# OpenPPL/ppq

Measured on AMD Instinct MI355X. Metric: calibration samples/sec (RuntimeCalibrationPass, KL 2048-bin, ResNet-50 INT8), higher is better.
Workload: dtype f32; 1 GPU; ResNet-50 topology (53 Conv + 1 Gemm, BN folded, seeded He init), RuntimeCalibrationPass kl 2048 bins, per-tensor INT8 activations, per-channel INT8 weights, 279 batches x 32 x 3x224x224 per GPU; samples=8928, batch=32, observed_tensors=72, rccl_ranks=1, async_observe=False, cache_params=False, channels_last=False, fuse_params=True, batch_observations=True, reuse_activations=False, replayed_batches=0, hip_graph=auto, graph_replays=0, miopen_find=False

## Files before the change

include/ppq_hip.h:

```cpp
#ifndef PPQ_HIP_H_
#define PPQ_HIP_H_

#include <stdint.h>

#ifdef __cplusplus
extern "C" {
#endif

typedef enum {
    PPQHIP_OK = 0,
    PPQHIP_ERR_INVALID_VALUE = -1,
    PPQHIP_ERR_UNSUPPORTED = -2,
    PPQHIP_ERR_HIP = -3
} ppqhip_status;

#define PPQHIP_ABI_VERSION 4

const char* ppqhip_last_error(void);
int ppqhip_version(void);
int ppqhip_device_arch(char* buf, int n);

int ppqhip_fq_linear_t(const float* x, const float* scale, const float* offset, float* out,
                       int64_t n, int clip_min, int clip_max, int rounding, void* stream);

// ... 85 lines not shown

int ppqhip_fq_float_c_bwd(const float* x, const float* scale, const float* offset,
                          const float* grad_y, float* grad_x, float* grad_s, int64_t n,
                          int64_t num_channel, int64_t elem_per_channel,
                          int exponent, int mantissa, float clip_min, float clip_max,
                          int rounding, void* stream);

int64_t ppqhip_hist_workspace_bytes(int64_t n, int64_t num_bins);
int ppqhip_hist_sym_t(const float* x, int64_t n, float hist_scale, int clip_outliers,
                      int32_t* hist, int64_t num_bins, void* workspace, void* stream);

int ppqhip_hist_asym_t(const float* x, int64_t n, float min_value, float max_value,
                       int clip_outliers, int32_t* hist, int64_t num_bins, void* workspace,
                       void* stream);

int ppqhip_hist_sym_c(const float* x, int64_t n, int64_t num_channel, int64_t elem_per_channel,
                      float hist_scale, int clip_outliers, int32_t* hist, int64_t num_bins,
                      void* stream);

int ppqhip_hist_sym_c_scales(const float* x, int64_t n, int64_t num_channel, int64_t elem_per_channel,
                             const float* hist_scales, int clip_outliers, int32_t* hist,
                             int64_t num_bins, void* stream);
int ppqhip_hist_asym_c_ranges(const float* x, int64_t n, int64_t num_channel, int64_t elem_per_channel,
                              const float* mins, const float* maxs, int clip_outliers, int32_t* hist,
                              int64_t num_bins, void* stream);

int64_t ppqhip_quantile_workspace_bytes(int64_t n);
int ppqhip_quantile_t(const float* x, int64_t n, float q, float* dest, uint32_t* hint, void* workspace,
                      void* stream);

typedef struct ppqhip_quantile_job {
    const float* x;
    float* dest;
    uint32_t* hint;
    int64_t n;
} ppqhip_quantile_job;
int64_t ppqhip_quantile_multi_workspace_bytes(int num_jobs, int64_t total_elems);
int ppqhip_quantile_t_multi(const ppqhip_quantile_job* jobs, int num_jobs, float q, void* workspace,
                            void* stream);
void ppqhip_quantile_debug_layout(int64_t* out);
void ppqhip_quantile_hot_layout(int64_t* out);

int ppqhip_isotone_t(const float* x, int64_t n, float* dest, void* workspace, void* stream);

int64_t ppqhip_minmax_workspace_bytes(int64_t n);
int ppqhip_minmax_t(const float* x, int64_t n, float* minmax, void* workspace, void* stream);

int ppqhip_minmax_c(const float* x, int64_t n, int64_t num_channel, int64_t elem_per_channel,
                    float* mins, float* maxs, void* stream);

typedef struct ppqhip_minmax_c_job {
    const float* x;
    float* mins;
    float* maxs;
    int64_t n, num_channel, elem_per_channel;
    int32_t fresh, reserved;
} ppqhip_minmax_c_job;
int ppqhip_minmax_c_multi(const ppqhip_minmax_c_job* jobs, int num_jobs, void* stream);

int ppqhip_channel_sum(const float* x, int64_t n, int64_t num_channel, int64_t elem_per_channel,
                       double* sums, void* stream);

int64_t ppqhip_hist_rows(void);
int ppqhip_hist_sym_t_rows(const float* x, int64_t n, float hist_scale, int clip_outliers,
                           int32_t* rows, int64_t num_bins, void* stream);
int ppqhip_hist_asym_t_rows(const float* x, int64_t n, float min_value, float max_value,
                            int clip_outliers, int32_t* rows, int64_t num_bins, void* stream);
typedef struct ppqhip_minmax_job {
    const float* x;
    float* slots;
    int64_t n;
} ppqhip_minmax_job;
int ppqhip_minmax_t_slots_multi(const ppqhip_minmax_job* jobs, int num_jobs, void* stream);

typedef struct ppqhip_hist_job {
    const float* x;
    int32_t* rows;
    int64_t n;
    float p0, p1;
} ppqhip_hist_job;
int ppqhip_hist_t_rows_multi(const ppqhip_hist_job* jobs, int num_jobs, int asymmetric,
                             int clip_outliers, int64_t num_bins, void* stream);
int ppqhip_hist_rows_finish(const int32_t* rows, int64_t num_bins, int32_t* hist, void* stream);
int ppqhip_check_bin_rule(const float* x, int64_t n, float min_value, float hist_scale, int asymmetric, uint64_t* out, void* stream);
int64_t ppqhip_minmax_slots(void);
int ppqhip_minmax_t_slots(const float* x, int64_t n, float* slots, void* stream);
int ppqhip_minmax_slots_finish(const float* slots, float* minmax, void* stream);

float ppqhip_mse_loss_host(const int64_t* hist, int64_t num_bins, int start, int step, int end);

int64_t ppqhip_mse_search_workspace_bytes(int64_t num_hist);
int ppqhip_mse_search(const int32_t* hist, int64_t num_hist, int64_t num_bins,
                      const double* hist_scale, const double* min_value,
                      int quant_min, int quant_max, int symmetrical, int32_t* best,
                      void* workspace, void* stream);

int64_t ppqhip_kl_num_candidates(int64_t num_bins, int num_of_bits);
int ppqhip_kl_losses(const int32_t* hist, int64_t num_hist, int64_t num_bins, int num_of_bits,
                     double* losses, void* stream);

int ppqhip_tensor_clip_t(const float* value, const float* reference, const float* limit,
                         float* out, int64_t n, void* stream);
int ppqhip_tensor_clip_c(const float* value, const float* reference, const float* limit,
                         float* out, int64_t n, int64_t num_channel, int64_t elem_per_channel,
                         void* stream);
int ppqhip_rounding_loss(const float* x, const float* scale, const float* offset, float* out,
                         int64_t n, int64_t num_channel, int64_t elem_per_channel,
                         int clip_min, int clip_max, int rounding, void* stream);
int ppqhip_rounding_loss_bwd(const float* x, const float* dy, const float* scale,
                             const float* offset, float* dx, int64_t n, int64_t num_channel,
                             int64_t elem_per_channel, int clip_min, int clip_max, int rounding,
                             void* stream);

int ppqhip_bias_act(float* y, const float* bias, int64_t n, int64_t num_channel, int64_t elem_per_channel,
                    int relu, void* stream);
int ppqhip_bias_add_act(float* a, const float* bias_a, float* b, const float* bias_b, float* out,
                        int64_t n, int64_t num_channel, int64_t elem_per_channel, int relu, void* stream);

#define PPQHIP_NOT_FUSED 1
int ppqhip_bias_act_stats(float* y, const float* bias, int64_t n, int64_t num_channel, int64_t elem_per_channel,
                          int relu, float* slots_y, void* stream);
int ppqhip_bias_add_act_stats(float* a, const float* bias_a, float* b, const float* bias_b, float* out,
                              int64_t n, int64_t num_channel, int64_t elem_per_channel, int relu,
                              float* slots_a, float* slots_b, float* slots_out, void* stream);

#define PPQHIP_ELIDE_A 1
#define PPQHIP_ELIDE_B 2
int ppqhip_bias_add_act_stats2(float* a, const float* bias_a, float* b, const float* bias_b, float* out,
                               int64_t n, int64_t num_channel, int64_t elem_per_channel, int relu,
                               float* slots_a, float* slots_b, float* slots_out, int elide, void* stream);

int ppqhip_bias_act_hist(float* y, const float* bias, int64_t n, int64_t num_channel, int64_t elem_per_channel,
                         int relu, int32_t* rows_y, float p0_y, float p1_y, int64_t num_bins, int asymmetric,
                         int clip_outliers, void* stream);
int ppqhip_bias_add_act_hist(float* a, const float* bias_a, float* b, const float* bias_b, float* out,
                             int64_t n, int64_t num_channel, int64_t elem_per_channel, int relu,
                             int32_t* rows_a, float p0_a, float p1_a, int32_t* rows_b, float p0_b, float p1_b,
                             int32_t* rows_out, float p0_out, float p1_out, int64_t num_bins, int asymmetric,
                             int clip_outliers, int elide, void* stream);

typedef struct ppqhip_adaround_job {
    const float* w;
    const float* v;
    const float* scale;
    const float* offset;
    float* out;
    const float* dy;
    int64_t n, num_channel, elem_per_channel;
    int32_t qmin, qmax;
} ppqhip_adaround_job;
int ppqhip_adaround_fwd_multi(const ppqhip_adaround_job* jobs, int num_jobs, void* stream);
int ppqhip_adaround_bwd_multi(const ppqhip_adaround_job* jobs, int num_jobs, const float* reg, void* stream);

typedef struct ppqhip_roundtune_job {
    const float* w;
    const float* r;
    const float* scale;
    const float* offset;
    float* out;
    int64_t n, num_channel, elem_per_channel;
    int32_t qmin, qmax;
} ppqhip_roundtune_job;
int ppqhip_roundtune_fwd_multi(const ppqhip_roundtune_job* jobs, int num_jobs, void* stream);

typedef struct ppqhip_fetch_rows_job {
    const float* x;
    const int32_t* index;
    float* out;
    int64_t rows, row_len, count;
} ppqhip_fetch_rows_job;
int ppqhip_fetch_rows_multi(const ppqhip_fetch_rows_job* jobs, int num_jobs, void* stream);
typedef struct ppqhip_measure_rows_job {
    const float* p;
    const float* r;
    const int32_t* index;
    double* sums;
    int64_t rows, row_len, count;
} ppqhip_measure_rows_job;
int ppqhip_measure_rows_multi(const ppqhip_measure_rows_job* jobs, int num_jobs, void* stream);
enum { PPQHIP_MEASURE_SNR = 0, PPQHIP_MEASURE_MSE = 1, PPQHIP_MEASURE_COSINE = 2 };
enum { PPQHIP_REDUCE_MEAN = 0, PPQHIP_REDUCE_MAX = 1 };
typedef struct ppqhip_measure_finish_job {
    const double* sums;
    double* acc;
    float* row_out;
    int64_t rows, count;
    int32_t method, reduce;
} ppqhip_measure_finish_job;
int ppqhip_measure_finish_multi(const ppqhip_measure_finish_job* jobs, int num_jobs, void* stream);

typedef struct ppqhip_equalize_segment {
    const float* base;
    int64_t extent;
    int64_t div, a, b;
    int64_t outer, stride, run;
    float multiplier;
    int32_t downstream;
} ppqhip_equalize_segment;
typedef struct ppqhip_equalize_scale_job {
    const ppqhip_equalize_segment* segments;
    float* scale;
    int32_t num_segments, num_channel;
    float value_threshold;
    int32_t reserved;
} ppqhip_equalize_scale_job;
int ppqhip_equalize_scale_multi(const ppqhip_equalize_scale_job* jobs, int num_jobs, void* stream);
typedef struct ppqhip_equalize_apply_job {
    float* x;
    const float* scale;
    int64_t n, run, inner, group_out;
    int64_t num_scale;
    int32_t divide, reserved;
} ppqhip_equalize_apply_job;
int ppqhip_equalize_apply_multi(const ppqhip_equalize_apply_job* jobs, int num_jobs, void* stream);

typedef struct ppqhip_split_plan_job {
    const ppqhip_equalize_segment* segments;
    int32_t* src_of;
    int32_t* count;
    int32_t num_segments, num_channel;
    float value_threshold;
    int32_t reserved;
// ... 119 lines not shown
```

ppq_amd/_lib.py:

```python
import ctypes
import os

_HERE = os.path.dirname(os.path.abspath(__file__))
LIB_PATH = os.path.join(_HERE, 'libppq_hip.so')

c_f32p = ctypes.c_void_p
c_i32p = ctypes.c_void_p
c_f64p = ctypes.c_void_p
c_i64 = ctypes.c_int64
c_int = ctypes.c_int
c_flt = ctypes.c_float
c_vp = ctypes.c_void_p

ABI_VERSION = 4


NOT_FUSED = 1


class ProfEntry(ctypes.Structure):
    _fields_ = [('name', ctypes.c_char * 48), ('launches', ctypes.c_int64),
                ('total_ms', ctypes.c_double), ('total_bytes', ctypes.c_double)]


PROTOTYPES = {
    'ppqhip_last_error': (ctypes.c_char_p, []),
    'ppqhip_version': (c_int, []),
    'ppqhip_device_arch': (c_int, [ctypes.c_char_p, c_int]),
    'ppqhip_fq_linear_t': (c_int, [c_f32p, c_f32p, c_f32p, c_f32p, c_i64, c_int, c_int, c_int, c_vp]),
    'ppqhip_fq_linear_c': (c_int, [c_f32p, c_f32p, c_f32p, c_f32p, c_i64, c_i64, c_i64, c_int, c_int, c_int, c_vp]),
    'ppqhip_to_int_t': (c_int, [c_f32p, c_f32p, c_f32p, c_vp, c_i64, c_int, c_int, c_int, c_int, c_vp]),
    'ppqhip_to_int_c': (c_int, [c_f32p, c_f32p, c_f32p, c_vp, c_i64, c_i64, c_i64, c_int, c_int, c_int, c_int, c_vp]),
    'ppqhip_fq_linear_t_bwd': (c_int, [c_f32p, c_f32p, c_f32p, c_f32p, c_f32p, c_f32p, c_i64, c_int, c_int, c_int,
                                       c_vp]),
    'ppqhip_fq_linear_c_bwd': (c_int, [c_f32p, c_f32p, c_f32p, c_f32p, c_f32p, c_f32p, c_i64, c_i64, c_i64, c_int,
                                       c_int, c_int, c_vp]),
    'ppqhip_fq_linear_c_bwd_multi': (c_int, [c_vp, c_int, c_int, c_vp]),
    'ppqhip_fq_linear_t_bwd_partials': (c_i64, [c_i64]),
    'ppqhip_fq_linear_t_bwd_main': (c_int, [c_f32p, c_f32p, c_f32p, c_f32p, c_f32p, c_f32p, c_i64, c_int, c_int, c_int, c_vp]),
    'ppqhip_lsq_finish_multi': (c_int, [c_vp, c_int, c_vp]),
    'ppqhip_bias_act': (c_int, [c_f32p, c_f32p, c_i64, c_i64, c_i64, c_int, c_vp]),
    'ppqhip_bias_add_act': (c_int, [c_f32p, c_f32p, c_f32p, c_f32p, c_f32p, c_i64, c_i64, c_i64, c_int, c_vp]),
    'ppqhip_bias_act_stats': (c_int, [c_f32p, c_f32p, c_i64, c_i64, c_i64, c_int, c_f32p, c_vp]),
    'ppqhip_bias_add_act_stats': (c_int, [c_f32p, c_f32p, c_f32p, c_f32p, c_f32p, c_i64, c_i64, c_i64, c_int, c_f32p, c_f32p,
                                          c_f32p, c_vp]),
    'ppqhip_bias_add_act_stats2': (c_int, [c_f32p, c_f32p, c_f32p, c_f32p, c_f32p, c_i64, c_i64, c_i64, c_int, c_f32p, c_f32p,
                                           c_f32p, c_int, c_vp]),
    'ppqhip_bias_act_hist': (c_int, [c_f32p, c_f32p, c_i64, c_i64, c_i64, c_int, c_i32p, c_flt, c_flt, c_i64, c_int, c_int, c_vp]),
    'ppqhip_bias_add_act_hist': (c_int, [c_f32p, c_f32p, c_f32p, c_f32p, c_f32p, c_i64, c_i64, c_i64, c_int,
                                         c_i32p, c_flt, c_flt, c_i32p, c_flt, c_flt, c_i32p, c_flt, c_flt, c_i64, c_int, c_int,
                                         c_int, c_vp]),
    'ppqhip_fq_float_t': (c_int, [c_f32p, c_f32p, c_f32p, c_f32p, c_i64, c_int, c_int, c_flt, c_flt, c_int, c_vp]),
    'ppqhip_fq_float_c': (c_int, [c_f32p, c_f32p, c_f32p, c_f32p, c_i64, c_i64, c_i64, c_int, c_int, c_flt, c_flt,
                                  c_int, c_vp]),
    'ppqhip_fq_float_c_bwd': (c_int, [c_f32p, c_f32p, c_f32p, c_f32p, c_f32p, c_f32p, c_i64, c_i64, c_i64, c_int,
                                      c_int, c_flt, c_flt, c_int, c_vp]),
    'ppqhip_hist_workspace_bytes': (c_i64, [c_i64, c_i64]),
    'ppqhip_hist_sym_t': (c_int, [c_f32p, c_i64, c_flt, c_int, c_i32p, c_i64, c_vp, c_vp]),
    'ppqhip_hist_asym_t': (c_int, [c_f32p, c_i64, c_flt, c_flt, c_int, c_i32p, c_i64, c_vp, c_vp]),
    'ppqhip_hist_sym_c': (c_int, [c_f32p, c_i64, c_i64, c_i64, c_flt, c_int, c_i32p, c_i64, c_vp]),
    'ppqhip_hist_sym_c_scales': (c_int, [c_f32p, c_i64, c_i64, c_i64, c_f32p, c_int, c_i32p, c_i64, c_vp]),
    'ppqhip_hist_asym_c_ranges': (c_int, [c_f32p, c_i64, c_i64, c_i64, c_f32p, c_f32p, c_int, c_i32p, c_i64, c_vp]),
    'ppqhip_quantile_workspace_bytes': (c_i64, [c_i64]),
    'ppqhip_quantile_t': (c_int, [c_f32p, c_i64, c_flt, c_f32p, c_vp, c_vp, c_vp]),
    'ppqhip_isotone_t': (c_int, [c_f32p, c_i64, c_f32p, c_vp, c_vp]),
    'ppqhip_minmax_workspace_bytes': (c_i64, [c_i64]),
    'ppqhip_minmax_t': (c_int, [c_f32p, c_i64, c_f32p, c_vp, c_vp]),
    'ppqhip_minmax_c': (c_int, [c_f32p, c_i64, c_i64, c_i64, c_f32p, c_f32p, c_vp]),
    'ppqhip_minmax_c_multi': (c_int, [c_vp, c_int, c_vp]),
    'ppqhip_fq_linear_multi_table_bytes': (c_i64, [c_int]),
    'ppqhip_fq_linear_multi': (c_int, [c_vp, c_int, c_int, c_vp, c_int, c_vp]),
    'ppqhip_float_scale_search_table_bytes': (c_i64, [c_int]),
    'ppqhip_float_scale_search': (c_int, [c_vp, c_int, c_vp, c_int, c_int, c_vp, c_vp, c_vp]),
    'ppqhip_fq_float_multi_table_bytes': (c_i64, [c_int]),
    'ppqhip_fq_float_multi': (c_int, [c_vp, c_int, c_int, c_vp, c_int, c_vp]),
    'ppqhip_quantile_multi_workspace_bytes': (c_i64, [c_int, c_i64]),
    'ppqhip_quantile_t_multi': (c_int, [c_vp, c_int, c_flt, c_vp, c_vp]),
    'ppqhip_quantile_debug_layout': (None, [c_vp]),
    'ppqhip_quantile_hot_layout': (None, [c_vp]),
    'ppqhip_minmax_t_slots_multi': (c_int, [c_vp, c_int, c_vp]),
    'ppqhip_hist_t_rows_multi': (c_int, [c_vp, c_int, c_int, c_int, c_i64, c_vp]),
    'ppqhip_channel_sum': (c_int, [c_f32p, c_i64, c_i64, c_i64, c_f64p, c_vp]),
    'ppqhip_hist_rows': (c_i64, []),
    'ppqhip_hist_sym_t_rows': (c_int, [c_f32p, c_i64, c_flt, c_int, c_i32p, c_i64, c_vp]),
    'ppqhip_hist_asym_t_rows': (c_int, [c_f32p, c_i64, c_flt, c_flt, c_int, c_i32p, c_i64, c_vp]),
    'ppqhip_hist_rows_finish': (c_int, [c_i32p, c_i64, c_i32p, c_vp]),
    'ppqhip_check_bin_rule': (c_int, [c_f32p, c_i64, c_flt, c_flt, c_int, c_vp, c_vp]),
    'ppqhip_minmax_slots': (c_i64, []),
    'ppqhip_minmax_t_slots': (c_int, [c_f32p, c_i64, c_f32p, c_vp]),
    'ppqhip_minmax_slots_finish': (c_int, [c_f32p, c_f32p, c_vp]),
    'ppqhip_mse_loss_host': (c_flt, [ctypes.POINTER(ctypes.c_int64), c_i64, c_int, c_int, c_int]),
    'ppqhip_mse_search_workspace_bytes': (c_i64, [c_i64]),
    'ppqhip_mse_search': (c_int, [c_i32p, c_i64, c_i64, c_f64p, c_f64p, c_int, c_int, c_int, c_i32p, c_vp, c_vp]),
    'ppqhip_kl_num_candidates': (c_i64, [c_i64, c_int]),
    'ppqhip_kl_losses': (c_int, [c_i32p, c_i64, c_i64, c_int, c_f64p, c_vp]),
    'ppqhip_tensor_clip_t': (c_int, [c_f32p, c_f32p, c_f32p, c_f32p, c_i64, c_vp]),
    'ppqhip_tensor_clip_c': (c_int, [c_f32p, c_f32p, c_f32p, c_f32p, c_i64, c_i64, c_i64, c_vp]),
    'ppqhip_rounding_loss': (c_int, [c_f32p, c_f32p, c_f32p, c_f32p, c_i64, c_i64, c_i64, c_int, c_int, c_int, c_vp]),
    'ppqhip_rounding_loss_bwd': (c_int, [c_f32p, c_f32p, c_f32p, c_f32p, c_f32p, c_i64, c_i64, c_i64, c_int, c_int,
                                         c_int, c_vp]),
    'ppqhip_adaround_fwd_multi': (c_int, [c_vp, c_int, c_vp]),
    'ppqhip_adaround_bwd_multi': (c_int, [c_vp, c_int, c_f32p, c_vp]),
    'ppqhip_roundtune_fwd_multi': (c_int, [c_vp, c_int, c_vp]),
    'ppqhip_equalize_scale_multi': (c_int, [c_vp, c_int, c_vp]),
    'ppqhip_equalize_apply_multi': (c_int, [c_vp, c_int, c_vp]),
    'ppqhip_split_plan_multi': (c_int, [c_vp, c_int, c_vp]),
    'ppqhip_split_apply_multi': (c_int, [c_vp, c_int, c_vp]),
    'ppqhip_ssd_scales_multi': (c_int, [c_vp, c_int, c_vp]),
    'ppqhip_ssd_apply_multi': (c_int, [c_vp, c_int, c_vp]),
    'ppqhip_fq_measure_rows_multi': (c_int, [c_vp, c_int, c_vp]),
    'ppqhip_fetch_rows_multi': (c_int, [c_vp, c_int, c_vp]),
    'ppqhip_measure_rows_multi': (c_int, [c_vp, c_int, c_vp]),
    'ppqhip_measure_finish_multi': (c_int, [c_vp, c_int, c_vp]),
    'ppqhip_stat_moments_multi': (c_int, [c_vp, c_int, c_vp]),
    'ppqhip_stat_shape_multi': (c_int, [c_vp, c_int, c_vp]),
    'ppqhip_mx_fq': (c_int, [c_f32p, c_f32p, c_vp, c_i64, c_i64, c_i64, c_int, c_vp]),
    'ppqhip_mx_fq_multi': (c_int, [c_vp, c_int, c_vp]),
    'ppqhip_mx_pack': (c_int, [c_f32p, c_vp, c_vp, c_i64, c_i64, c_i64, c_int, c_vp]),
    'ppqhip_mx_pack_multi': (c_int, [c_vp, c_int, c_vp]),
    'ppqhip_mx_unpack': (c_int, [c_vp, c_vp, c_f32p, c_i64, c_i64, c_i64, c_int, c_vp]),
    'ppqhip_mx_unpack_multi': (c_int, [c_vp, c_int, c_vp]),
    'ppqhip_mx_gemm': (c_int, [c_vp, c_vp, c_int, c_vp, c_vp, c_int, c_f32p, c_f32p, c_i64, c_i64, c_i64, c_vp]),
    'ppqhip_prof_enable': (c_int, [c_int]),
    'ppqhip_mx_conv2d': (c_int, [c_vp, c_vp, c_int, c_vp, c_vp, c_int, c_f32p, c_f32p] + [c_i64] * 13 + [c_vp]),
    'ppqhip_mx_gemm_fused': (c_int, [c_vp, c_vp, c_int, c_vp, c_vp, c_int, c_f32p, c_f32p, c_int, c_f32p, c_vp, c_vp, c_int, c_i64, c_i64, c_i64, c_vp]),
    'ppqhip_mx_conv2d_fused': (c_int, [c_vp, c_vp, c_int, c_vp, c_vp, c_int, c_f32p, c_f32p, c_int, c_f32p, c_vp, c_vp, c_int] + [c_i64] * 13 + [c_vp]),
    'ppqhip_prof_collect': (c_int, [ctypes.POINTER(ProfEntry), c_int]),
    'ppqhip_prof_event_overhead_us': (ctypes.c_double, [c_vp, c_int]),
}

if not os.path.exists(LIB_PATH):
    raise ImportError(
        f'{LIB_PATH} is missing: the HIP kernel library has not been built.  Run '
        '`python -c "import __graft_entry__ as g; g.build()"` or `make -C ppq_amd/csrc` (needs hipcc, '
        'targets gfx950).  ppq_amd has no CPU / PyTorch fallback by design.')

import torch

_torch_hip = os.path.join(os.path.dirname(torch.__file__), 'lib', 'libamdhip64.so')
if os.path.exists(_torch_hip):
    ctypes.CDLL(_torch_hip, mode=ctypes.RTLD_GLOBAL)

try:
    lib = ctypes.CDLL(LIB_PATH)
except OSError as e:
    raise ImportError(f'cannot load {LIB_PATH}: {e}') from e

for _name, (_res, _args) in PROTOTYPES.items():
    _fn = getattr(lib, _name)
    _fn.restype = _res
    _fn.argtypes = _args


if lib.ppqhip_version() != ABI_VERSION:
    raise ImportError(f'{LIB_PATH} has ABI version {lib.ppqhip_version()}, this package needs {ABI_VERSION}: rebuild it '
                      '(`make -C ppq_amd/csrc` or `python -c "import __graft_entry__ as g; g.build()"`)')


def last_error() -> str:
    msg = lib.ppqhip_last_error()
    return msg.decode('utf-8', 'replace') if msg else ''
```

ppq_amd/csrc/epilogue.hip:

```cpp
#include "channel_axis.hpp"
#include "common.hpp"
#include "hist_bin.hpp"
#include "minmax_fold.hpp"

namespace ppqhip {
namespace {

constexpr int kEpTileU = 2;
constexpr int kEpSmallU = 1;
constexpr long long kEpSmallElems = 1ll << 20;

struct EpArgs {
    float* a;
    const float* bias_a;
    float* b;
    const float* bias_b;
    float* out;
    uint32_t nvec;
    uint32_t tail;
    int ntail;
    FastDiv epc;
    FastDiv nc;
    uint32_t elide;
};

__device__ __forceinline__ float act(float v, bool relu) {
    return (relu && !__builtin_isnan(v)) ? __builtin_fmaxf(v, 0.f) : v;
}

__device__ __forceinline__ float4 add4(const float4& x, const float4& y) {
    return make_float4(x.x + y.x, x.y + y.y, x.z + y.z, x.w + y.w);
}

template <bool RELU>
__device__ __forceinline__ float4 act4(const float4& v) {
    return make_float4(act(v.x, RELU), act(v.y, RELU), act(v.z, RELU), act(v.w, RELU));
}

template <bool PLANE>
__device__ __forceinline__ float4 bias4(const float* __restrict__ bias, uint32_t v, const FastDiv& epc, const FastDiv& nc) {
    if (PLANE) {
        const float t = bias[channel_of(v, epc, nc)];
        return make_float4(t, t, t, t);
    }
    const uint32_t i = v * 4u;
    return make_float4(bias[channel_of(i, epc, nc)], bias[channel_of(i + 1, epc, nc)], bias[channel_of(i + 2, epc, nc)],
                       bias[channel_of(i + 3, epc, nc)]);
}

template <typename T>
struct EpStored { T a, b, out; };

constexpr uint32_t kElideA = 1u, kElideB = 2u;

template <bool RESID, bool BIAS_B, bool RELU>
__device__ __forceinline__ EpStored<float> epilogue_elem(const EpArgs& p, uint32_t i, const FastDiv& epc, uint32_t elide = 0) {
    EpStored<float> s{};
    const uint32_t c = channel_of(i, epc, p.nc);
    const float x = p.a[i] + p.bias_a[c];
    if (!RESID) { p.a[i] = s.a = act(x, RELU); return s; }
    s.a = x;
    if (!(elide & kElideA)) p.a[i] = x;
    float y = p.b[i];
    if (BIAS_B) {
        y = y + p.bias_b[c];
        s.b = y;
        if (!(elide & kElideB)) p.b[i] = y;
    }
    p.out[i] = s.out = act(x + y, RELU);
    return s;
}

template <bool RESID, bool BIAS_B, bool RELU>
__device__ __forceinline__ EpStored<float4> epilogue_vec(float4* a4, float4* b4, float4* o4, uint32_t vv, const float4& a,
                                                         const float4& ba, const float4& b, const float4& bb,
                                                         uint32_t elide = 0) {
    EpStored<float4> s{};
    const float4 x = add4(a, ba);
    if (!RESID) { a4[vv] = s.a = act4<RELU>(x); return s; }
    s.a = x;
    if (!(elide & kElideA)) a4[vv] = x;
    float4 y = b;
    if (BIAS_B) {
        y = add4(y, bb);
        s.b = y;
        if (!(elide & kElideB)) b4[vv] = y;
    }
    o4[vv] = s.out = act4<RELU>(add4(x, y));
    return s;
}

template <int U, bool RESID, bool BIAS_B, bool RELU, bool PLANE>
__global__ __launch_bounds__(kBlock) void epilogue_kernel(EpArgs p) {
    const uint32_t base = blockIdx.x * (kBlock * U) + threadIdx.x;
    float4* a4 = reinterpret_cast<float4*>(p.a);
    float4* b4 = reinterpret_cast<float4*>(p.b);
    float4* o4 = reinterpret_cast<float4*>(p.out);
    float4 a[U], ba[U], b[U]{}, bb[U]{};
#pragma unroll
    for (int k = 0; k < U; k++) {
        const uint32_t vv = min(base + k * kBlock, p.nvec - 1);
        a[k] = a4[vv];
        ba[k] = bias4<PLANE>(p.bias_a, vv, p.epc, p.nc);
        if (RESID) b[k] = b4[vv];
        if (BIAS_B) bb[k] = bias4<PLANE>(p.bias_b, vv, p.epc, p.nc);
    }
#pragma unroll
    for (int k = 0; k < U; k++) {
        const uint32_t vv = base + k * kBlock;
        if (vv >= p.nvec) continue;
        epilogue_vec<RESID, BIAS_B, RELU>(a4, b4, o4, vv, a[k], ba[k], b[k], bb[k]);
    }
    if (!PLANE && blockIdx.x == 0 && (int)threadIdx.x < p.ntail)
        epilogue_elem<RESID, BIAS_B, RELU>(p, p.tail + threadIdx.x, p.epc);
}

template <bool RESID, bool BIAS_B, bool RELU>
__global__ __launch_bounds__(kBlock) void epilogue_scalar_kernel(EpArgs p) {
    const uint32_t stride = gridDim.x * kBlock;
    for (uint32_t i = blockIdx.x * kBlock + threadIdx.x; i < (uint32_t)p.ntail; i += stride)
        epilogue_elem<RESID, BIAS_B, RELU>(p, i, p.epc);
}

bool fill_vector_geometry(EpArgs& p, int64_t n, int64_t C, int64_t epc) {
    const ChannelAxisMap g = pack_channel_axis(true, n, C, epc);
    p.nc = g.nc; p.epc = g.epc;
    p.nvec = g.nvec;
    p.tail = g.nvec * 4u;
    p.ntail = (int)(n & 3);
    return g.plane != 0;
}

template <bool RESID, bool BIAS_B, bool RELU>
void launch_epilogue(EpArgs p, int64_t n, int64_t C, int64_t epc, bool aligned, hipStream_t st) {
    if (!aligned || n < 4) {
        p.nvec = 0; p.tail = 0; p.ntail = (int)n;
        p.epc = make_fastdiv((uint32_t)epc); p.nc = make_fastdiv((uint32_t)C);
        hipLaunchKernelGGL((epilogue_scalar_kernel<RESID, BIAS_B, RELU>), dim3(stream_grid(n, kBlock)), dim3(kBlock), 0, st, p);
        return;
    }
    const bool plane = fill_vector_geometry(p, n, C, epc);
#define PPQ_LAUNCH_EP(U, PLANE)                                                                                          \
    hipLaunchKernelGGL((epilogue_kernel<U, RESID, BIAS_B, RELU, PLANE>), dim3((p.nvec + kBlock * U - 1) / (kBlock * U)),   \
                       dim3(kBlock), 0, st, p)
    if (n <= kEpSmallElems) {
        if (plane) PPQ_LAUNCH_EP(kEpSmallU, true); else PPQ_LAUNCH_EP(kEpSmallU, false);
    } else {
        if (plane) PPQ_LAUNCH_EP(kEpTileU, true); else PPQ_LAUNCH_EP(kEpTileU, false);
    }
#undef PPQ_LAUNCH_EP
}

constexpr int kEpStatBlock = 512;
constexpr int kEpStatWgPerCu = 2;

struct EpMinMaxSinks { float* slots[3]; };
template <bool RESID, bool BIAS_B>
struct EpMinMaxSet {
    using Args = EpMinMaxSinks;
    static constexpr int NS = RESID ? 3 : 1;
    bool live[NS];
    float mn[NS], mx[NS];
// ... 61 lines not shown
    __device__ __forceinline__ void begin() {
#pragma unroll
        for (int k = 0; k < NS; k++) {
#pragma unroll
            for (int r = 0; r < kRowRegs; r++) {
                const int b = (int)threadIdx.x + r * kEpStatBlock;
                old[k][r] = (early && live[k] && b <= acc[k].last) ? row[k][b] : 0;
            }
        }
        for (uint32_t i = threadIdx.x; i < lds_ints; i += kEpStatBlock) lds[i] = 0;
        asm volatile("s_waitcnt lgkmcnt(0)\n\ts_barrier" ::: "memory");
    }
    template <bool FULL>
    __device__ __forceinline__ void bin4(Binner<ASYM, CLIP, true>& a, const float4& v, bool in, bool elect) {
        int b[4];
        a.bins4(v, b);
        if (elect) a.elect(b[0], FULL || in);
        if (FULL && CLIP) a.commit4_exec(b);
        else {
            a.template commit<FULL>(b[0], in); a.template commit<FULL>(b[1], in);
            a.template commit<FULL>(b[2], in); a.template commit<FULL>(b[3], in);
        }
    }
    template <bool FULL>
    __device__ __forceinline__ void feed4(const EpStored<float4>& s, bool in, bool elect) {
        if (live[0]) bin4<FULL>(acc[0], s.a, in, elect);
        if (RESID) {
            if (BIAS_B && live[1]) bin4<FULL>(acc[1], s.b, in, elect);
            if (live[NS - 1]) bin4<FULL>(acc[NS - 1], s.out, in, elect);
        }
    }
    __device__ __forceinline__ void bin1(Binner<ASYM, CLIP, true>& a, float v, bool in) {
        const int b = a.bin1(v);
        a.elect(b, in);
        a.template commit<false>(b, in);
    }
    __device__ __forceinline__ void feed1(const EpStored<float>& s, bool in) {
        if (live[0]) bin1(acc[0], s.a, in);
        if (RESID) {
            if (BIAS_B && live[1]) bin1(acc[1], s.b, in);
            if (live[NS - 1]) bin1(acc[NS - 1], s.out, in);
        }
    }
    __device__ __forceinline__ void finish(const Args& sk, uint32_t g, int*) {
#pragma unroll
        for (int k = 0; k < NS; k++)
            if (live[k]) acc[k].flush_hot();
        asm volatile("s_waitcnt lgkmcnt(0)" ::: "memory");
        __syncthreads();
#pragma unroll
        for (int k = 0; k < NS; k++) {
            if (!live[k]) continue;
            const int* h = acc[k].h;
            if (early) {
#pragma unroll
                for (int r = 0; r < kRowRegs; r++) {
                    const int b = (int)threadIdx.x + r * kEpStatBlock;
                    if (b >= sk.bins) break;
                    const int c = h[b];
                    if (c) row[k][b] = old[k][r] + c;
                }
            } else {
                for (int b = threadIdx.x; b < sk.bins; b += kEpStatBlock) {
                    const int c = h[b];
                    if (c) row[k][b] += c;
                }
            }
        }
    }
};

template <int U, bool RESID, bool BIAS_B, bool RELU, bool PLANE, class SINKS>
__global__ __launch_bounds__(kEpStatBlock, (kEpStatBlock * kEpStatWgPerCu + 255) / 256)
void epilogue_stats_kernel(EpArgs p, typename SINKS::Args sk) {
    extern __shared__ int lds[];
    constexpr uint32_t kTile = (uint32_t)kEpStatBlock * U;
    const uint32_t G = gridDim.x, g = blockIdx.x;
    const uint32_t full = p.nvec / kTile, tiles = full + (p.nvec > full * kTile ? 1u : 0u);
    uint32_t t, t_end;
    even_split(tiles, G, g, t, t_end);
    float4* a4 = reinterpret_cast<float4*>(p.a);
    float4* b4 = reinterpret_cast<float4*>(p.b);
    float4* o4 = reinterpret_cast<float4*>(p.out);
    const uint32_t elide = p.elide;
    SINKS sinks;
    sinks.init(sk, lds);

    struct Tile { float4 a[U], ba[U], b[U], bb[U]; };
    auto fetch = [&](Tile& T, uint32_t tile) {
        const uint32_t base = tile * kTile + threadIdx.x;
#pragma unroll
        for (int u = 0; u < U; u++) {
            const uint32_t vv = base + u * kEpStatBlock;
            T.a[u] = a4[vv];
            T.ba[u] = bias4<PLANE>(p.bias_a, vv, p.epc, p.nc);
            if (RESID) T.b[u] = b4[vv];
            if (BIAS_B) T.bb[u] = bias4<PLANE>(p.bias_b, vv, p.epc, p.nc);
        }
    };
    auto consume = [&](const Tile& T, uint32_t tile) {
        const uint32_t base = tile * kTile + threadIdx.x;
        EpStored<float4> s[U];
#pragma unroll
        for (int u = 0; u < U; u++)
            s[u] = epilogue_vec<RESID, BIAS_B, RELU>(a4, b4, o4, base + u * kEpStatBlock, T.a[u], T.ba[u], T.b[u], T.bb[u], elide);
#pragma unroll
        for (int u = 0; u < U; u++) sinks.template feed4<true>(s[u], true, u == 0);
    };
    const uint32_t tf = min(t_end, full);
    Tile ta{}, tb{};
    if (t < tf) fetch(ta, t);
    sinks.begin();
    if (t < tf) {
        for (;;) {
            fetch(tb, min(t + 1, tf - 1));
            consume(ta, t);
            if (++t >= tf) break;
            fetch(ta, min(t + 1, tf - 1));
            consume(tb, t);
            if (++t >= tf) break;
        }
    }
    if (t < t_end) {
        const uint32_t base = t * kTile + threadIdx.x;
#pragma unroll
        for (int u = 0; u < U; u++) {
            const uint32_t vv = base + u * kEpStatBlock;
            const uint32_t vc = min(vv, p.nvec - 1);
            const float4 a = a4[vc], ba = bias4<PLANE>(p.bias_a, vc, p.epc, p.nc);
            float4 b{}, bb{};
            if (RESID) b = b4[vc];
            if (BIAS_B) bb = bias4<PLANE>(p.bias_b, vc, p.epc, p.nc);
            const bool in = vv < p.nvec;
            EpStored<float4> s{};
            if (in) s = epilogue_vec<RESID, BIAS_B, RELU>(a4, b4, o4, vv, a, ba, b, bb, elide);
            sinks.template feed4<false>(s, in, true);
        }
    }
    if (!PLANE && g == G - 1 && p.ntail > 0) {
        const bool in = (int)threadIdx.x < p.ntail;
        EpStored<float> s{};
        if (in) s = epilogue_elem<RESID, BIAS_B, RELU>(p, p.tail + threadIdx.x, p.epc, elide);
        sinks.feed1(s, in);
    }
    sinks.finish(sk, g, lds);
}

template <bool RESID, bool BIAS_B>
int launch_epilogue_stats(EpArgs p, int64_t n, int64_t C, int64_t epc, int relu, bool aligned, EpMinMaxSinks sk, const char* what,
                          hipStream_t st) {
    if ((!sk.slots[0] && !sk.slots[1] && !sk.slots[2]) || !aligned || n < 4) return PPQHIP_NOT_FUSED;
    const bool plane = fill_vector_geometry(p, n, C, epc);
    const bool small = n <= kEpSmallElems;
    const uint32_t tile = (uint32_t)kEpStatBlock * (small ? kEpSmallU : kEpTileU), tiles = (p.nvec + tile - 1) / tile;
    const uint32_t cap = (uint32_t)(num_cu() * kEpStatWgPerCu);
    const uint32_t grid = tiles < cap ? tiles : cap;
    using Set = EpMinMaxSet<RESID, BIAS_B>;
#define PPQ_LAUNCH_EPS(U, RELU, PLANE)                                                                                    \
    hipLaunchKernelGGL((epilogue_stats_kernel<U, RESID, BIAS_B, RELU, PLANE, Set>), dim3(grid), dim3(kEpStatBlock),         \
                       32 * sizeof(float), st, p, sk)
    switch ((small ? 0 : 4) | (relu ? 2 : 0) | (plane ? 1 : 0)) {
        case 0: PPQ_LAUNCH_EPS(kEpSmallU, false, false); break;
        case 1: PPQ_LAUNCH_EPS(kEpSmallU, false, true); break;
        case 2: PPQ_LAUNCH_EPS(kEpSmallU, true, false); break;
        case 3: PPQ_LAUNCH_EPS(kEpSmallU, true, true); break;
        case 4: PPQ_LAUNCH_EPS(kEpTileU, false, false); break;
        case 5: PPQ_LAUNCH_EPS(kEpTileU, false, true); break;
        case 6: PPQ_LAUNCH_EPS(kEpTileU, true, false); break;
        default: PPQ_LAUNCH_EPS(kEpTileU, true, true); break;
    }
#undef PPQ_LAUNCH_EPS
    return finish_launch(what);
}

constexpr uint32_t kEpHistLdsInts = 3 * 2048;
constexpr uint32_t kEpHistMinTiles = 2;
struct EpHistRule { int bins, asym, clip; };

template <bool RESID, bool BIAS_B>
int launch_epilogue_hist(EpArgs p, int64_t n, int64_t C, int64_t epc, int relu, bool aligned, EpHistSinks sk, EpHistRule r,
                         const char* what, hipStream_t st) {
    uint32_t ints = 0;
    for (int k = 0; k < 3; k++) {
        sk.lds_off[k] = ints;
        if (sk.rows[k]) ints += (uint32_t)r.bins;
    }
    sk.lds_ints = ints; sk.bins = r.bins;
    if (ints == 0 || ints > kEpHistLdsInts || !aligned || n <= kEpSmallElems || !relu) return PPQHIP_NOT_FUSED;
    const bool plane = fill_vector_geometry(p, n, C, epc);
    const uint32_t tile = (uint32_t)kEpStatBlock * kEpTileU, tiles = (p.nvec + tile - 1) / tile;
    const uint32_t cap = (uint32_t)(num_cu() * kEpStatWgPerCu);
    uint32_t grid = tiles / kEpHistMinTiles;
    if (grid > cap) grid = cap;
#define PPQ_LAUNCH_EPH(PLANE, ASYM, CLIP)                                                                                 \
    hipLaunchKernelGGL((epilogue_stats_kernel<kEpTileU, RESID, BIAS_B, true, PLANE, EpHistSet<RESID, BIAS_B, ASYM, CLIP>>),  \
                       dim3(grid), dim3(kEpStatBlock), ints * sizeof(int), st, p, sk)
    switch ((plane ? 4 : 0) | (r.asym ? 2 : 0) | (r.clip ? 1 : 0)) {
        case 0: PPQ_LAUNCH_EPH(false, false, false); break;
        case 1: PPQ_LAUNCH_EPH(false, false, true); break;
        case 2: PPQ_LAUNCH_EPH(false, true, false); break;
        case 3: PPQ_LAUNCH_EPH(false, true, true); break;
        case 4: PPQ_LAUNCH_EPH(true, false, false); break;
        case 5: PPQ_LAUNCH_EPH(true, false, true); break;
        case 6: PPQ_LAUNCH_EPH(true, true, false); break;
        default: PPQ_LAUNCH_EPH(true, true, true); break;
    }
#undef PPQ_LAUNCH_EPH
    return finish_launch(what);
}

void set_hist_rule(EpHistSinks& sk, int k, int32_t* rows, float p0, float p1, const EpHistRule& r) {
    sk.rows[k] = rows;
    if (r.asym) { sk.a0[k] = p0; sk.hs[k] = (p1 - p0) / (float)r.bins; }
    else { sk.a0[k] = 0.f; sk.hs[k] = p0; }
}

int validate_elide(const char* what, int elide, bool sink_a, bool sink_b, bool has_bias_b) {
    if (elide & ~(int)(kElideA | kElideB)) { set_error("%s: elide has unknown bits", what); return PPQHIP_ERR_INVALID_VALUE; }
    if (((elide & (int)kElideA) && !sink_a) || ((elide & (int)kElideB) && !(sink_b && has_bias_b))) {
        set_error("%s: a tensor that is not stored needs a sink", what); return PPQHIP_ERR_INVALID_VALUE;
    }
    return PPQHIP_OK;
}

}
}

using namespace ppqhip;

extern "C" {

int ppqhip_bias_act(float* y, const float* bias, int64_t n, int64_t num_channel, int64_t elem_per_channel, int relu,
                    void* stream) {
    if (int st = validate_channel_axis("bias_act", n, num_channel, elem_per_channel)) return st;
    if (!y || !bias) { set_error("bias_act: null pointer"); return PPQHIP_ERR_INVALID_VALUE; }
    hipStream_t s = (hipStream_t)stream;
    EpArgs p{};
    p.a = y; p.bias_a = bias;
    const bool aligned = aligned16(y);
    if (relu) launch_epilogue<false, false, true>(p, n, num_channel, elem_per_channel, aligned, s);
    else launch_epilogue<false, false, false>(p, n, num_channel, elem_per_channel, aligned, s);
    return finish_launch("bias_act");
}

int ppqhip_bias_add_act(float* a, const float* bias_a, float* b, const float* bias_b, float* out, int64_t n,
                        int64_t num_channel, int64_t elem_per_channel, int relu, void* stream) {
    if (int st = validate_channel_axis("bias_add_act", n, num_channel, elem_per_channel)) return st;
    if (!a || !bias_a || !b || !out) { set_error("bias_add_act: null pointer"); return PPQHIP_ERR_INVALID_VALUE; }
    hipStream_t s = (hipStream_t)stream;
    EpArgs p{};
    p.a = a; p.bias_a = bias_a; p.b = b; p.bias_b = bias_b; p.out = out;
    const bool aligned = aligned16(a) && aligned16(b) && aligned16(out);
    if (bias_b) {
        if (relu) launch_epilogue<true, true, true>(p, n, num_channel, elem_per_channel, aligned, s);
        else launch_epilogue<true, true, false>(p, n, num_channel, elem_per_channel, aligned, s);
    } else {
        if (relu) launch_epilogue<true, false, true>(p, n, num_channel, elem_per_channel, aligned, s);
        else launch_epilogue<true, false, false>(p, n, num_channel, elem_per_channel, aligned, s);
    }
    return finish_launch("bias_add_act");
}

int ppqhip_bias_act_stats(float* y, const float* bias, int64_t n, int64_t num_channel, int64_t elem_per_channel, int relu,
                          float* slots_y, void* stream) {
    if (int st = validate_channel_axis("bias_act_stats", n, num_channel, elem_per_channel)) return st;
    if (!y || !bias) { set_error("bias_act_stats: null pointer"); return PPQHIP_ERR_INVALID_VALUE; }
    EpArgs p{};
    p.a = y; p.bias_a = bias;
    return launch_epilogue_stats<false, false>(p, n, num_channel, elem_per_channel, relu, aligned16(y), EpMinMaxSinks{{slots_y, nullptr, nullptr}},
                                               "bias_act_stats", (hipStream_t)stream);
}

static int bias_add_act_stats_impl(const char* what, float* a, const float* bias_a, float* b, const float* bias_b, float* out,
                                   int64_t n, int64_t num_channel, int64_t elem_per_channel, int relu, float* slots_a,
                                   float* slots_b, float* slots_out, int elide, void* stream) {
    if (int st = validate_channel_axis(what, n, num_channel, elem_per_channel)) return st;
    if (!a || !bias_a || !b || !out) { set_error("%s: null pointer", what); return PPQHIP_ERR_INVALID_VALUE; }
    if (!bias_b && slots_b) { set_error("%s: without bias_b, b is only read: it has no sink", what); return PPQHIP_ERR_INVALID_VALUE; }
    if (int st = validate_elide(what, elide, slots_a != nullptr, slots_b != nullptr, bias_b != nullptr)) return st;
    EpArgs p{};
    p.a = a; p.bias_a = bias_a; p.b = b; p.bias_b = bias_b; p.out = out; p.elide = (uint32_t)elide;
    const bool aligned = aligned16(a) && aligned16(b) && aligned16(out);
    const EpMinMaxSinks sk{{slots_a, slots_b, slots_out}};
    hipStream_t s = (hipStream_t)stream;
    if (bias_b) return launch_epilogue_stats<true, true>(p, n, num_channel, elem_per_channel, relu, aligned, sk, what, s);
    return launch_epilogue_stats<true, false>(p, n, num_channel, elem_per_channel, relu, aligned, sk, what, s);
}

int ppqhip_bias_add_act_stats(float* a, const float* bias_a, float* b, const float* bias_b, float* out, int64_t n,
                              int64_t num_channel, int64_t elem_per_channel, int relu, float* slots_a, float* slots_b,
                              float* slots_out, void* stream) {
    return bias_add_act_stats_impl("bias_add_act_stats", a, bias_a, b, bias_b, out, n, num_channel, elem_per_channel, relu,
                                   slots_a, slots_b, slots_out, 0, stream);
}

int ppqhip_bias_add_act_stats2(float* a, const float* bias_a, float* b, const float* bias_b, float* out, int64_t n,
                               int64_t num_channel, int64_t elem_per_channel, int relu, float* slots_a, float* slots_b,
                               float* slots_out, int elide, void* stream) {
    return bias_add_act_stats_impl("bias_add_act_stats2", a, bias_a, b, bias_b, out, n, num_channel, elem_per_channel, relu,
                                   slots_a, slots_b, slots_out, elide, stream);
}

static int validate_hist_rule(const char* what, int64_t bins) {
    if (bins <= 0 || bins > 0x7fffffffLL) { set_error("%s: histogram is empty or too large", what); return PPQHIP_ERR_INVALID_VALUE; }
    return PPQHIP_OK;
}

int ppqhip_bias_act_hist(float* y, const float* bias, int64_t n, int64_t num_channel, int64_t elem_per_channel, int relu,
                         int32_t* rows_y, float p0_y, float p1_y, int64_t num_bins, int asymmetric, int clip_outliers,
                         void* stream) {
    if (int st = validate_channel_axis("bias_act_hist", n, num_channel, elem_per_channel)) return st;
    if (!y || !bias) { set_error("bias_act_hist: null pointer"); return PPQHIP_ERR_INVALID_VALUE; }
    if (int st = validate_hist_rule("bias_act_hist", num_bins)) return st;
    if (num_bins > (int64_t)kEpHistLdsInts) return PPQHIP_NOT_FUSED;
    const EpHistRule r{(int)num_bins, asymmetric ? 1 : 0, clip_outliers ? 1 : 0};
    EpHistSinks sk{};
    set_hist_rule(sk, 0, rows_y, p0_y, p1_y, r);
    EpArgs p{};
    p.a = y; p.bias_a = bias;
    return launch_epilogue_hist<false, false>(p, n, num_channel, elem_per_channel, relu, aligned16(y), sk, r, "bias_act_hist",
                                              (hipStream_t)stream);
}

int ppqhip_bias_add_act_hist(float* a, const float* bias_a, float* b, const float* bias_b, float* out, int64_t n,
                             int64_t num_channel, int64_t elem_per_channel, int relu, int32_t* rows_a, float p0_a, float p1_a,
                             int32_t* rows_b, float p0_b, float p1_b, int32_t* rows_out, float p0_out, float p1_out,
                             int64_t num_bins, int asymmetric, int clip_outliers, int elide, void* stream) {
    const char* what = "bias_add_act_hist";
    if (int st = validate_channel_axis(what, n, num_channel, elem_per_channel)) return st;
    if (!a || !bias_a || !b || !out) { set_error("%s: null pointer", what); return PPQHIP_ERR_INVALID_VALUE; }
    if (!bias_b && rows_b) { set_error("%s: without bias_b, b is only read: it has no sink", what); return PPQHIP_ERR_INVALID_VALUE; }
    if (int st = validate_hist_rule(what, num_bins)) return st;
    if (int st = validate_elide(what, elide, rows_a != nullptr, rows_b != nullptr, bias_b != nullptr)) return st;
    if ((rows_a && (rows_a == rows_b || rows_a == rows_out)) || (rows_b && rows_b == rows_out)) {
        set_error("%s: two sinks share one rows accumulator", what); return PPQHIP_ERR_INVALID_VALUE;
    }
    if (num_bins > (int64_t)kEpHistLdsInts) return PPQHIP_NOT_FUSED;
    const EpHistRule r{(int)num_bins, asymmetric ? 1 : 0, clip_outliers ? 1 : 0};
    EpHistSinks sk{};
    set_hist_rule(sk, 0, rows_a, p0_a, p1_a, r);
    set_hist_rule(sk, 1, rows_b, p0_b, p1_b, r);
    set_hist_rule(sk, 2, rows_out, p0_out, p1_out, r);
    EpArgs p{};
    p.a = a; p.bias_a = bias_a; p.b = b; p.bias_b = bias_b; p.out = out; p.elide = (uint32_t)elide;
    const bool aligned = aligned16(a) && aligned16(b) && aligned16(out);
    hipStream_t s = (hipStream_t)stream;
    if (bias_b) return launch_epilogue_hist<true, true>(p, n, num_channel, elem_per_channel, relu, aligned, sk, r, what, s);
    return launch_epilogue_hist<true, false>(p, n, num_channel, elem_per_channel, relu, aligned, sk, r, what, s);
}

}
```

ppq_amd/csrc/hist.hip:

```cpp
#include "common.hpp"
#include "hist_bin.hpp"

namespace ppqhip {

constexpr int kMaxLdsBins = 16384;
constexpr int kLdsBudgetInts = 2048;
constexpr int kHistBlock = 512;
constexpr int kHistWgPerCu = 2;
constexpr int kHistU = 2;
constexpr int kHistMinTiles = 2;
constexpr int kHistAtomicMaxWg = 128;
constexpr long long kHistNtElems = 48ll << 20;
constexpr int kHistRows = kNumCU * kHistWgPerCu;
constexpr uint32_t kTileVec = (uint32_t)kHistBlock * kHistU;
constexpr uint32_t kTileElems = kTileVec * 4;
static_assert(kHistBlock % 64 == 0 && kHistBlock >= 64 && kHistBlock <= 1024, "histogram workgroup: whole waves");

struct BinRule {
    float a;
    float hs;
    float rcp;
    int bins;
    int clip;
    int asym;
};
static BinRule make_rule(float a, float hs, int bins, int clip, int asym) {
    BinRule r; r.a = a; r.hs = hs; r.rcp = 1.0f / hs; r.bins = bins; r.clip = clip; r.asym = asym;
    return r;
}

constexpr int kReduceBins = 32, kReduceSlices = 32, kReduceBlock = kReduceBins * kReduceSlices;
__global__ __launch_bounds__(kReduceBlock) void hist_reduce_kernel(const int* __restrict__ partial, int count, int bins,
                                                                   int* __restrict__ hist) {
    __shared__ int lds[kReduceSlices][kReduceBins];
    const int lane_bin = threadIdx.x % kReduceBins, slice = threadIdx.x / kReduceBins;
    const int b = blockIdx.x * kReduceBins + lane_bin;
    int total = 0;
    if (b < bins) {
        int i = slice;
        for (; i + 15 * kReduceSlices < count; i += 16 * kReduceSlices) {
            int v[16];
#pragma unroll
            for (int k = 0; k < 16; k++) v[k] = partial[(size_t)(i + k * kReduceSlices) * bins + b];
#pragma unroll
            for (int k = 0; k < 16; k++) total += v[k];
        }
        for (; i < count; i += kReduceSlices) total += partial[(size_t)i * bins + b];
    }
    lds[slice][lane_bin] = total;
    __syncthreads();
    if (slice == 0 && b < bins) {
        int t = 0;
#pragma unroll
        for (int k = 0; k < kReduceSlices; k++) t += lds[k][lane_bin];
        if (t) hist[b] += t;
    }
}

constexpr int kMultiMax = 96;
enum FlushMode : int {
    FLUSH_ROWS_ADD = 0,
    FLUSH_ROWS_STORE = 1,
    FLUSH_ATOMIC = 2
};
struct HistJob {
    const float* x;
    int* rows;
    uint32_t n;
    float a, hs;
    uint32_t first_tile;
};
struct HistJobs {
    HistJob job[kMultiMax];
    uint32_t count;
    uint32_t total_tiles;
    int bins, copies, mode;
};
__host__ __device__ inline uint32_t job_tiles(uint32_t n, bool vec_ok) {
    if (!vec_ok) return (n + kTileElems - 1) / kTileElems;
    const uint32_t full = (n >> 2) / kTileVec;
    return full + (n > full * kTileElems ? 1u : 0u);
}

__device__ __forceinline__ void lds_hist_flush(int* lds, int bins, int copies, int* __restrict__ dst, int mode) {
    asm volatile("s_waitcnt lgkmcnt(0)" ::: "memory");
    __syncthreads();
    for (int b = threadIdx.x; b < bins; b += kHistBlock) {
        int s = 0;
        for (int c = 0; c < copies; c++) { s += lds[c * bins + b]; lds[c * bins + b] = 0; }
        if (mode == FLUSH_ROWS_STORE) dst[b] = s;
        else if (s) {
            if (mode == FLUSH_ROWS_ADD) dst[b] += s;
            else atomicAdd(&dst[b], s);
        }
    }
    __syncthreads();
}

template <bool ASYM, bool CLIP, bool HOT, bool NT>
__global__ __launch_bounds__(kHistBlock, (kHistBlock * kHistWgPerCu + 255) / 256)
void hist_persistent_kernel(const HistJobs jobs) {
    extern __shared__ int lds[];
    const uint32_t G = gridDim.x, g = blockIdx.x;
    uint32_t t, t_end;
    even_split(jobs.total_tiles, G, g, t, t_end);
    const int bins = jobs.bins, copies = jobs.copies;
    bool zeroed = false;
    auto zero_lds = [&]() {
        if (zeroed) return;
        for (int i = threadIdx.x; i < copies * bins; i += kHistBlock) lds[i] = 0;
        asm volatile("s_waitcnt lgkmcnt(0)\n\ts_barrier" ::: "memory");
        zeroed = true;
    };
    if (t >= t_end) {
        if (jobs.mode == FLUSH_ROWS_STORE) for (int b = threadIdx.x; b < bins; b += kHistBlock) jobs.job[0].rows[(size_t)g * bins + b] = 0;
        return;
    }
    uint32_t lo = 0, hi = jobs.count;
    while (hi - lo > 1) {
        const uint32_t mid = (lo + hi) >> 1;
        if (jobs.job[mid].first_tile <= t) lo = mid; else hi = mid;
    }
    Binner<ASYM, CLIP, HOT> acc;
    acc.init(lds + ((threadIdx.x >> 6) % copies) * bins, bins);

    for (uint32_t j = lo; t < t_end; j++) {
        const HistJob& job = jobs.job[j];
        const uint32_t j_end = (j + 1 < jobs.count) ? jobs.job[j + 1].first_tile : jobs.total_tiles;
        uint32_t k = t - job.first_tile;
        const uint32_t k1 = min(t_end, j_end) - job.first_tile;
        t = min(t_end, j_end);
        acc.set_rule(job.a, job.hs);
        const float* __restrict__ x = job.x;
        const uint32_t n = job.n;
        const bool vec_ok = (reinterpret_cast<uintptr_t>(x) & 15u) == 0;
        const uint32_t full = vec_ok ? (n >> 2) / kTileVec : 0u;
        const uint32_t kf = min(k1, full);
        if (k < kf) {
            const float4* xv = reinterpret_cast<const float4*>(x) + threadIdx.x;
// ... 534 lines not shown
    LaunchScope scope(K_HIST_SYM_T, 4.0 * (double)n, s);
    BinRule rule = make_rule(0.f, hist_scale, (int)num_bins, clip_outliers ? 1 : 0, 0);
    if (int st = launch_hist_t(x, n, rule, hist, workspace, s)) return st;
    return finish_launch("hist_sym_t");
}

int ppqhip_hist_asym_t(const float* x, int64_t n, float min_value, float max_value, int clip_outliers,
                       int32_t* hist, int64_t num_bins, void* workspace, void* stream) {
    if (int st = validate(n, num_bins, "hist_asym_t")) return st;
    hipStream_t s = (hipStream_t)stream;
    LaunchScope scope(K_HIST_ASYM_T, 4.0 * (double)n, s);
    const float hs = (max_value - min_value) / (float)num_bins;
    BinRule rule = make_rule(min_value, hs, (int)num_bins, clip_outliers ? 1 : 0, 1);
    if (int st = launch_hist_t(x, n, rule, hist, workspace, s)) return st;
    return finish_launch("hist_asym_t");
}

int64_t ppqhip_hist_rows(void) { return (int64_t)kHistRows; }

int ppqhip_hist_sym_t_rows(const float* x, int64_t n, float hist_scale, int clip_outliers, int32_t* rows,
                           int64_t num_bins, void* stream) {
    if (int st = validate(n, num_bins, "hist_sym_t_rows")) return st;
    if (num_bins > kMaxLdsBins) { set_error("hist_sym_t_rows: at most %d bins", kMaxLdsBins); return PPQHIP_ERR_UNSUPPORTED; }
    hipStream_t s = (hipStream_t)stream;
    LaunchScope scope(K_HIST_SYM_T, 4.0 * (double)n, s);
    BinRule rule = make_rule(0.f, hist_scale, (int)num_bins, clip_outliers ? 1 : 0, 0);
    if (int st = launch_hist_t(x, n, rule, nullptr, nullptr, s, rows)) return st;
    return finish_launch("hist_sym_t_rows");
}

int ppqhip_hist_asym_t_rows(const float* x, int64_t n, float min_value, float max_value, int clip_outliers,
                            int32_t* rows, int64_t num_bins, void* stream) {
    if (int st = validate(n, num_bins, "hist_asym_t_rows")) return st;
    if (num_bins > kMaxLdsBins) { set_error("hist_asym_t_rows: at most %d bins", kMaxLdsBins); return PPQHIP_ERR_UNSUPPORTED; }
    hipStream_t s = (hipStream_t)stream;
    LaunchScope scope(K_HIST_ASYM_T, 4.0 * (double)n, s);
    const float hs = (max_value - min_value) / (float)num_bins;
    BinRule rule = make_rule(min_value, hs, (int)num_bins, clip_outliers ? 1 : 0, 1);
    if (int st = launch_hist_t(x, n, rule, nullptr, nullptr, s, rows)) return st;
    return finish_launch("hist_asym_t_rows");
}

int ppqhip_hist_t_rows_multi(const ppqhip_hist_job* jobs, int num_jobs, int asymmetric, int clip_outliers,
                             int64_t num_bins, void* stream) {
    if (num_jobs <= 0) return PPQHIP_OK;
    if (jobs == nullptr) { set_error("hist_t_rows_multi: jobs is null"); return PPQHIP_ERR_INVALID_VALUE; }
    if (num_bins <= 0 || num_bins > kMaxLdsBins) {
        set_error("hist_t_rows_multi: 1..%d bins", kMaxLdsBins); return PPQHIP_ERR_UNSUPPORTED;
    }
    double bytes = 0.0;
    for (int k = 0; k < num_jobs; k++) {
        if (int st = validate(jobs[k].n, num_bins, "hist_t_rows_multi")) return st;
        if (jobs[k].x == nullptr || jobs[k].rows == nullptr) {
            set_error("hist_t_rows_multi: job %d has a null pointer", k); return PPQHIP_ERR_INVALID_VALUE;
        }
        bytes += 4.0 * (double)jobs[k].n;
    }
    hipStream_t s = (hipStream_t)stream;
    LaunchScope scope(asymmetric ? K_HIST_ASYM_T : K_HIST_SYM_T, bytes, s);
    if (int st = launch_hist_multi(jobs, num_jobs, (int)num_bins, clip_outliers ? 1 : 0, asymmetric ? 1 : 0, s)) return st;
    return finish_launch("hist_t_rows_multi");
}

int ppqhip_check_bin_rule(const float* x, int64_t n, float min_value, float hist_scale, int asymmetric, uint64_t* out, void* stream) {
    if (n <= 0 || n > 0x7fffffffLL || (n & 3) || !aligned16(x) || out == nullptr) {
        set_error("check_bin_rule: n must be a positive multiple of 4 below 2^31, x 16-B aligned, out non-null"); return PPQHIP_ERR_INVALID_VALUE;
    }
    hipStream_t s = (hipStream_t)stream;
    const uint32_t nvec = (uint32_t)(n >> 2);
    if (asymmetric) hipLaunchKernelGGL((check_bin_rule_kernel<true>), dim3(stream_grid(nvec, kBlock)), dim3(kBlock), 0, s, (const float4*)x, nvec,
                                       min_value, hist_scale, (unsigned long long*)out);
    else hipLaunchKernelGGL((check_bin_rule_kernel<false>), dim3(stream_grid(nvec, kBlock)), dim3(kBlock), 0, s, (const float4*)x, nvec,
                            0.f, hist_scale, (unsigned long long*)out);
    return finish_launch("check_bin_rule");
}

int ppqhip_hist_rows_finish(const int32_t* rows, int64_t num_bins, int32_t* hist, void* stream) {
    if (num_bins <= 0 || num_bins > kMaxLdsBins) { set_error("hist_rows_finish: bad bins"); return PPQHIP_ERR_INVALID_VALUE; }
    hipStream_t s = (hipStream_t)stream;
    launch_reduce((const int*)rows, (int)ppqhip_hist_rows(), (int)num_bins, hist, s);
    return finish_launch("hist_rows_finish");
}

static int hist_c_impl(const float* x, int64_t n, int64_t num_channel, int64_t elem_per_channel,
                       float hist_scale, const float* scales, const float* mins, const float* maxs, int clip_outliers,
                       int32_t* hist, int64_t num_bins, void* stream, const char* what) {
    if (int st = validate(n, num_bins, what)) return st;
    if (num_channel <= 0 || elem_per_channel <= 0 || n % (num_channel * elem_per_channel) != 0) {
        set_error("%s: Kernel Failure, Histogram shape is invalid.", what); return PPQHIP_ERR_INVALID_VALUE;
    }
    hipStream_t s = (hipStream_t)stream;
    const int asym = mins != nullptr;
    LaunchScope scope(K_HIST_SYM_C, 4.0 * (double)n, s);
    BinRule rule = make_rule(0.f, hist_scale, (int)num_bins, clip_outliers ? 1 : 0, asym);
    const FastDiv nc = make_fastdiv((uint32_t)num_channel);
    if (elem_per_channel % 4 == 0 && elem_per_channel >= 64 && aligned16(x) && num_bins <= kMaxLdsBins) {
        const uint32_t C = (uint32_t)num_channel, outer = (uint32_t)(n / (num_channel * elem_per_channel));
        const uint32_t want_wgs = (uint32_t)num_cu() * kHistCWgPerCu;
        uint32_t splits = C >= want_wgs ? 1u : (want_wgs + C - 1) / C;
        const uint64_t tiles_per_channel = ((uint64_t)outer * (uint64_t)(elem_per_channel / 4)) / kTileVec;
        if (splits > tiles_per_channel) splits = tiles_per_channel > 0 ? (uint32_t)tiles_per_channel : 1u;
        const int copies = pick_copies(rule.bins, kHistBlock);
        const int flush_mode = (splits == 1 && n > kHistSmallElems) ? FLUSH_ROWS_ADD : FLUSH_ATOMIC;
        const bool nt = n >= kHistNtElems;
#define PPQ_LAUNCH_HIST_CC(A, CL)                                                                                     \
        do {                                                                                                          \
            if (nt) hipLaunchKernelGGL((hist_c_channel_kernel<A, CL, true>), dim3(C * splits), dim3(kHistBlock), lds_bytes(rule.bins, copies), s, x, \
                           make_fastdiv((uint32_t)(elem_per_channel / 4)), C, outer, splits, rule, copies, hist, scales, mins, maxs, \
                           flush_mode);                                                                               \
            else hipLaunchKernelGGL((hist_c_channel_kernel<A, CL, false>), dim3(C * splits), dim3(kHistBlock), lds_bytes(rule.bins, copies), s, x, \
                           make_fastdiv((uint32_t)(elem_per_channel / 4)), C, outer, splits, rule, copies, hist, scales, mins, maxs, \
                           flush_mode);                                                                               \
        } while (0)
        switch ((asym ? 2 : 0) | (rule.clip ? 1 : 0)) {
            case 0: PPQ_LAUNCH_HIST_CC(false, false); break;
            case 1: PPQ_LAUNCH_HIST_CC(false, true); break;
            case 2: PPQ_LAUNCH_HIST_CC(true, false); break;
            default: PPQ_LAUNCH_HIST_CC(true, true); break;
        }
#undef PPQ_LAUNCH_HIST_CC
    } else if (n / num_channel >= 256 && num_bins <= kMaxLdsBins) {
        const uint32_t C = (uint32_t)num_channel, outer = (uint32_t)(n / (num_channel * elem_per_channel));
        const uint32_t want_wgs = (uint32_t)num_cu() * kHistCWgPerCu;
        uint32_t splits = C >= want_wgs ? 1u : (want_wgs + C - 1) / C;
        const uint64_t trips_per_channel = ((uint64_t)outer * (uint64_t)elem_per_channel) / (kHistBlock * 8);
        if (splits > trips_per_channel) splits = trips_per_channel > 0 ? (uint32_t)trips_per_channel : 1u;
        const int copies = pick_copies(rule.bins, kHistBlock);
#define PPQ_LAUNCH_HIST_CS(A, CL)                                                                                     \
        hipLaunchKernelGGL((hist_c_channel_scalar_kernel<A, CL>), dim3(C * splits), dim3(kHistBlock), lds_bytes(rule.bins, copies), s, \
                           x, make_fastdiv((uint32_t)elem_per_channel), C, outer, splits, rule, copies, hist, scales, mins, maxs)
        switch ((asym ? 2 : 0) | (rule.clip ? 1 : 0)) {
            case 0: PPQ_LAUNCH_HIST_CS(false, false); break;
            case 1: PPQ_LAUNCH_HIST_CS(false, true); break;
            case 2: PPQ_LAUNCH_HIST_CS(true, false); break;
            default: PPQ_LAUNCH_HIST_CS(true, true); break;
        }
#undef PPQ_LAUNCH_HIST_CS
    } else {
        hipLaunchKernelGGL(hist_c_global_kernel, dim3(stream_grid(n, kBlock * 4)), dim3(kBlock), 0, s, x, (uint32_t)n,
                           make_fastdiv((uint32_t)elem_per_channel), nc, rule, hist, scales, mins, maxs);
    }
    return finish_launch(what);
}

int ppqhip_hist_sym_c(const float* x, int64_t n, int64_t num_channel, int64_t elem_per_channel,
                      float hist_scale, int clip_outliers, int32_t* hist, int64_t num_bins, void* stream) {
    return hist_c_impl(x, n, num_channel, elem_per_channel, hist_scale, nullptr, nullptr, nullptr, clip_outliers, hist,
                       num_bins, stream, "hist_sym_c");
}

int ppqhip_hist_sym_c_scales(const float* x, int64_t n, int64_t num_channel, int64_t elem_per_channel,
                             const float* hist_scales, int clip_outliers, int32_t* hist, int64_t num_bins,
                             void* stream) {
    if (hist_scales == nullptr) { set_error("hist_sym_c_scales: hist_scales is null"); return PPQHIP_ERR_INVALID_VALUE; }
    return hist_c_impl(x, n, num_channel, elem_per_channel, 1.0f, hist_scales, nullptr, nullptr, clip_outliers, hist,
                       num_bins, stream, "hist_sym_c_scales");
}

int ppqhip_hist_asym_c_ranges(const float* x, int64_t n, int64_t num_channel, int64_t elem_per_channel,
                              const float* mins, const float* maxs, int clip_outliers, int32_t* hist,
                              int64_t num_bins, void* stream) {
    if (mins == nullptr || maxs == nullptr) { set_error("hist_asym_c_ranges: mins / maxs is null"); return PPQHIP_ERR_INVALID_VALUE; }
    return hist_c_impl(x, n, num_channel, elem_per_channel, 1.0f, nullptr, mins, maxs, clip_outliers, hist, num_bins,
                       stream, "hist_asym_c_ranges");
}

// ... 2 lines not shown
```

ppq_amd/csrc/reduce.hip:

```cpp
#include <cmath>
#include <cstdlib>
#include <vector>

#include "common.hpp"
#include "minmax_fold.hpp"

namespace ppqhip {

__device__ __forceinline__ void block_minmax_commit(float mn, float mx, float* gmin, float* gmax, float* lds) {
    mn = wave_min(mn);
    mx = wave_max(mx);
    const int wid = threadIdx.x >> 6, lane = threadIdx.x & 63, nw = blockDim.x >> 6;
    if (lane == 0) { lds[wid] = mn; lds[8 + wid] = mx; }
    __syncthreads();
    if (threadIdx.x == 0) {
        for (int w = 1; w < nw; w++) { mn = fminf(mn, lds[w]); mx = fmaxf(mx, lds[8 + w]); }
        if (mn <= mx) {
            atomic_min_f32(gmin, mn);
            atomic_max_f32(gmax, mx);
        }
    }
}

template <int U, bool NT>
__global__ __launch_bounds__(kBlock) void minmax_t_kernel(const float* __restrict__ x, uint32_t n, int vec_ok,
                                                          float* __restrict__ minmax, float* __restrict__ partial,
                                                          int accumulate) {
    __shared__ float lds[32];
    float mn = INFINITY, mx = -INFINITY;
    stream_elems<U, NT>(x, n, vec_ok != 0, [&](float a) { minmax_fold1(mn, mx, a); });
    if (partial == nullptr) { block_minmax_commit(mn, mx, &minmax[0], &minmax[1], lds); return; }
    minmax_block_fold(mn, mx, lds);
    if (threadIdx.x == 0) {
        if (accumulate) {
            mn = fminf(mn, partial[2 * blockIdx.x]);
            mx = fmaxf(mx, partial[2 * blockIdx.x + 1]);
        }
        partial[2 * blockIdx.x] = mn;
        partial[2 * blockIdx.x + 1] = mx;
    }
}

constexpr int kMinMaxMultiMax = 96;
constexpr int kMMBlock = 256, kMMU = 2;
constexpr int kMMWgPerCu = 8;
constexpr int kMMGrid = kNumCU * kMMWgPerCu;
constexpr uint32_t kMMTileVec = (uint32_t)kMMBlock * kMMU, kMMTileElems = kMMTileVec * 4;
static_assert(kMMGrid <= kNumCU * 8, "one slot per workgroup");
struct MinMaxJob {
    const float* x;
    float* slots;
    uint32_t n;
    uint32_t first_tile;
};
struct MinMaxJobs {
    MinMaxJob job[kMinMaxMultiMax];
    uint32_t count;
    uint32_t total_tiles;
};
__host__ __device__ inline uint32_t mm_job_tiles(uint32_t n, bool vec_ok) {
    if (!vec_ok) return (n + kMMTileElems - 1) / kMMTileElems;
    const uint32_t full = (n >> 2) / kMMTileVec;
    return full + (n > full * kMMTileElems ? 1u : 0u);
}

template <bool NT>
__global__ __launch_bounds__(kMMBlock) void minmax_persistent_kernel(const MinMaxJobs jobs) {
    __shared__ float lds[32];
    const uint32_t G = gridDim.x, g = blockIdx.x;
    uint32_t t, t_end;
    even_split(jobs.total_tiles, G, g, t, t_end);
    if (t >= t_end) return;
    uint32_t lo = 0, hi = jobs.count;
    while (hi - lo > 1) {
        const uint32_t mid = (lo + hi) >> 1;
        if (jobs.job[mid].first_tile <= t) lo = mid; else hi = mid;
    }
    for (uint32_t j = lo; t < t_end; j++) {
        const MinMaxJob& job = jobs.job[j];
        const uint32_t j_end = (j + 1 < jobs.count) ? jobs.job[j + 1].first_tile : jobs.total_tiles;
        uint32_t k = t - job.first_tile;
        const uint32_t k1 = min(t_end, j_end) - job.first_tile;
        t = min(t_end, j_end);
        const float* __restrict__ x = job.x;
        const uint32_t n = job.n;
        const bool vec_ok = (reinterpret_cast<uintptr_t>(x) & 15u) == 0;
        const uint32_t full = vec_ok ? (n >> 2) / kMMTileVec : 0u;
// ... 7 lines not shown
#pragma unroll
                for (int u = 0; u < kMMU; u++) buf[u] = load4<NT>(p + u * kMMBlock);
            };
            auto consume = [&](const float4 (&buf)[kMMU]) {
#pragma unroll
                for (int u = 0; u < kMMU; u++) minmax_fold4(mn, mx, buf[u]);
            };
            fetch(bufa, k);
            for (;;) {
                fetch(bufb, min(k + 1, kf - 1));
                consume(bufa);
                if (++k >= kf) break;
                fetch(bufa, min(k + 1, kf - 1));
                consume(bufb);
                if (++k >= kf) break;
            }
        }
        for (; k < k1; k++) {
            const uint32_t e0 = k * kMMTileElems + threadIdx.x;
#pragma unroll 4
            for (int r = 0; r < 4 * kMMU; r++) {
                const uint32_t i = e0 + r * kMMBlock;
                if (i < n) minmax_fold1(mn, mx, x[i]);
            }
        }
        minmax_block_fold(mn, mx, lds);
        if (threadIdx.x == 0) minmax_slot_fold(job.slots + 2 * g, mn, mx);
        __syncthreads();
    }
}

template <int K, bool PING = false, bool NT = false>
__global__ __launch_bounds__(kMMBlock) void minmax_small_kernel(const float* __restrict__ x, uint32_t n, float* __restrict__ slots) {
    __shared__ float lds[32];
    const uint32_t G = gridDim.x, g = blockIdx.x;
    float s_mn = INFINITY, s_mx = -INFINITY;
    if (threadIdx.x == 0) { s_mn = slots[2 * g]; s_mx = slots[2 * g + 1]; }
    const uint32_t nvec = n >> 2, full_rows = nvec / kMMBlock;
    uint32_t r0, r1;
    even_split(full_rows, G, g, r0, r1);
    const float4* xv = reinterpret_cast<const float4*>(x) + threadIdx.x;
    float mn = INFINITY, mx = -INFINITY;
    auto fetch = [&](float4 (&buf)[K], uint32_t r) {
#pragma unroll
        for (int k = 0; k < K; k++) buf[k] = load4<NT>(xv + (size_t)min(r + (uint32_t)k, r1 - 1) * kMMBlock);
    };
    auto fold = [&](const float4 (&buf)[K]) {
#pragma unroll
        for (int k = 0; k < K; k++) minmax_fold4(mn, mx, buf[k]);
    };
    if (PING) {
        if (r0 < r1) {
            float4 bufa[K], bufb[K];
            uint32_t r = r0;
            fetch(bufa, r);
            for (;;) {
                fetch(bufb, r + K);
                fold(bufa);
                r += K;
                if (r >= r1) break;
                fetch(bufa, r + K);
                fold(bufb);
                r += K;
                if (r >= r1) break;
            }
        }
    } else {
        for (uint32_t r = r0; r < r1; r += K) {
            float4 buf[K];
            fetch(buf, r);
            fold(buf);
        }
    }
    if (g == G - 1) {
        for (uint32_t i = full_rows * kMMBlock * 4 + threadIdx.x; i < n; i += kMMBlock) minmax_fold1(mn, mx, x[i]);
    }
    minmax_block_fold(mn, mx, lds);
    if (threadIdx.x == 0) {
        slots[2 * g] = fminf(mn, s_mn);
        slots[2 * g + 1] = fmaxf(mx, s_mx);
    }
}

__global__ __launch_bounds__(kBlock) void minmax_finish_kernel(const float* __restrict__ partial, uint32_t count,
                                                               float* __restrict__ minmax) {
    __shared__ float lds[32];
    float mn = INFINITY, mx = -INFINITY;
    for (uint32_t i = threadIdx.x; i < count; i += kBlock) {
        mn = fminf(mn, partial[2 * i]);
        mx = fmaxf(mx, partial[2 * i + 1]);
    }
    minmax_block_fold(mn, mx, lds);
    if (threadIdx.x == 0) minmax_slot_fold(minmax, mn, mx);
}

constexpr int kMMCU = 16;
constexpr int kMMCWavesPerCu = 16;
constexpr uint32_t kMMCChunk = 8192;
__global__ __launch_bounds__(kBlock) void minmax_c_wave_kernel(const float* __restrict__ x, uint32_t epc, int vec_ok, uint32_t C,
                                                               uint32_t outer, uint32_t K, uint32_t chunks, uint32_t items,
                                                               float* __restrict__ mins, float* __restrict__ maxs) {
    const uint32_t item = blockIdx.x * (kBlock / kWave) + (threadIdx.x >> 6);
    if (item >= items) return;
    const uint32_t lane = threadIdx.x & 63;
    const uint32_t rc = item / chunks, chunk = item - rc * chunks;
    const uint32_t g = rc / C, c = rc - g * C;
    const uint32_t n0 = g * K, n1 = min(n0 + K, outer);
    const uint32_t lo = chunk * kMMCChunk, hi = min(lo + kMMCChunk, epc);
    float mn = INFINITY, mx = -INFINITY;
    for (uint32_t n = n0; n < n1; n++) {
        const float* xr = x + ((size_t)n * C + c) * epc;
        if (vec_ok) {
            const float4* xv = reinterpret_cast<const float4*>(xr);
            const uint32_t v1 = hi >> 2;
            for (uint32_t v0 = (lo >> 2) + lane; v0 < v1; v0 += 64 * kMMCU) {
                float4 a[kMMCU];
#pragma unroll
                for (int u = 0; u < kMMCU; u++) a[u] = xv[min(v0 + 64 * u, v1 - 1)];
#pragma unroll
                for (int u = 0; u < kMMCU; u++) {
                    mn = fminf(fminf(mn, a[u].x), fminf(a[u].y, fminf(a[u].z, a[u].w)));
                    mx = fmaxf(fmaxf(mx, a[u].x), fmaxf(a[u].y, fmaxf(a[u].z, a[u].w)));
                }
            }
        } else {
            for (uint32_t j = lo + lane; j < hi; j += 64) { const float a = xr[j]; mn = fminf(mn, a); mx = fmaxf(mx, a); }
        }
    }
    mn = wave_min(mn);
    mx = wave_max(mx);
    if (lane == 0 && mn <= mx) { atomic_min_f32(&mins[c], mn); atomic_max_f32(&maxs[c], mx); }
}

__global__ __launch_bounds__(kBlock) void minmax_c_generic_kernel(const float* __restrict__ x, uint32_t n,
                                                                  FastDiv elem_per_channel, FastDiv num_channel,
                                                                  int use_lds, float* __restrict__ mins,
                                                                  float* __restrict__ maxs) {
    extern __shared__ float mm[];
    const uint32_t C = num_channel.d;
    if (use_lds) {
        for (uint32_t c = threadIdx.x; c < C; c += kBlock) { mm[c] = INFINITY; mm[C + c] = -INFINITY; }
        __syncthreads();
    }
    const uint32_t stride = gridDim.x * kBlock;
    for (uint32_t i = blockIdx.x * kBlock + threadIdx.x; i < n; i += stride) {
        const float a = x[i];
        if (a != a) continue;
        const uint32_t row = fdiv(i, elem_per_channel);
        const uint32_t c = row - fdiv(row, num_channel) * C;
        if (use_lds) { atomic_min_f32(&mm[c], a); atomic_max_f32(&mm[C + c], a); }
        else { atomic_min_f32(&mins[c], a); atomic_max_f32(&maxs[c], a); }
    }
    if (use_lds) {
        __syncthreads();
        for (uint32_t c = threadIdx.x; c < C; c += kBlock) {
            if (mm[c] <= mm[C + c]) { atomic_min_f32(&mins[c], mm[c]); atomic_max_f32(&maxs[c], mm[C + c]); }
        }
    }
}

__device__ __forceinline__ double wave_sum_f64(double v) {
#pragma unroll
    for (int m = 32; m > 0; m >>= 1) v += __shfl_xor(v, m, 64);
    return v;
}

__global__ __launch_bounds__(kBlock) void channel_sum_row_kernel(const float* __restrict__ x, uint32_t rows_per_channel,
                                                                 uint32_t C, uint32_t epc, int vec_ok,
                                                                 double* __restrict__ partial) {
    __shared__ double lds[kBlock / kWave];
    const uint32_t c = blockIdx.x, s = blockIdx.y, S = gridDim.y;
    double acc = 0.0;
    for (uint32_t n = s; n < rows_per_channel; n += S) {
        const float* xr = x + ((size_t)n * C + c) * epc;
        if (vec_ok) {
            const float4* xv = reinterpret_cast<const float4*>(xr);
// ... 234 lines not shown
int64_t ppqhip_minmax_slots(void) { return (int64_t)kNumCU * 8; }

static void launch_minmax_persistent(const MinMaxJobs& args, int64_t elems, hipStream_t s) {
    uint32_t grid = args.total_tiles / 2;
    if (grid < 1) grid = 1;
    const uint32_t mm_cap = (uint32_t)(num_cu() * kMMWgPerCu);
    if (grid > mm_cap) grid = mm_cap;
    if (elems >= (48ll << 20)) hipLaunchKernelGGL((minmax_persistent_kernel<true>), dim3(grid), dim3(kMMBlock), 0, s, args);
    else hipLaunchKernelGGL((minmax_persistent_kernel<false>), dim3(grid), dim3(kMMBlock), 0, s, args);
}

int ppqhip_minmax_t_slots(const float* x, int64_t n, float* slots, void* stream) {
    if (slots == nullptr) { set_error("minmax_t_slots: slots is null"); return PPQHIP_ERR_INVALID_VALUE; }
    if (int st = validate(n, "minmax_t_slots")) return st;
    hipStream_t s = (hipStream_t)stream;
    LaunchScope scope(K_MINMAX_T, 4.0 * (double)n, s);
    if (n <= (4ll << 20) && aligned16(x)) {
        const uint32_t full_rows = (uint32_t)((n >> 2) / kMMBlock);
        uint32_t grid = (full_rows + 1) / 2;
        const uint32_t cap = (uint32_t)(num_cu() * kMMWgPerCu);
        if (grid > cap) grid = cap;
        if (grid < 1) grid = 1;
        const uint32_t share = (full_rows + grid - 1) / grid;
        if (share <= 2) hipLaunchKernelGGL((minmax_small_kernel<2>), dim3(grid), dim3(kMMBlock), 0, s, x, (uint32_t)n, slots);
        else if (share <= 4) hipLaunchKernelGGL((minmax_small_kernel<4>), dim3(grid), dim3(kMMBlock), 0, s, x, (uint32_t)n, slots);
        else hipLaunchKernelGGL((minmax_small_kernel<8>), dim3(grid), dim3(kMMBlock), 0, s, x, (uint32_t)n, slots);
        return finish_launch("minmax_t_slots");
    }
    if (aligned16(x)) {
        const uint32_t full_rows = (uint32_t)((n >> 2) / kMMBlock);
        uint32_t grid = full_rows / 8;
        const uint32_t cap = (uint32_t)(num_cu() * kMMWgPerCu);
        if (grid > cap) grid = cap;
        if (grid < 1) grid = 1;
        if (n >= (48ll << 20)) hipLaunchKernelGGL((minmax_small_kernel<2, true, true>), dim3(grid), dim3(kMMBlock), 0, s, x, (uint32_t)n, slots);
        else hipLaunchKernelGGL((minmax_small_kernel<2, true, false>), dim3(grid), dim3(kMMBlock), 0, s, x, (uint32_t)n, slots);
        return finish_launch("minmax_t_slots");
    }
    MinMaxJobs args;
    args.count = 1;
    args.job[0].x = x; args.job[0].slots = slots; args.job[0].n = (uint32_t)n; args.job[0].first_tile = 0;
    args.total_tiles = mm_job_tiles((uint32_t)n, aligned16(x));
    launch_minmax_persistent(args, n, s);
    return finish_launch("minmax_t_slots");
}

int ppqhip_minmax_t_slots_multi(const ppqhip_minmax_job* jobs, int num_jobs, void* stream) {
    if (num_jobs <= 0) return PPQHIP_OK;
    if (jobs == nullptr) { set_error("minmax_t_slots_multi: jobs is null"); return PPQHIP_ERR_INVALID_VALUE; }
    double bytes = 0.0;
    for (int k = 0; k < num_jobs; k++) {
        if (int st = validate(jobs[k].n, "minmax_t_slots_multi")) return st;
        if (jobs[k].x == nullptr || jobs[k].slots == nullptr) {
            set_error("minmax_t_slots_multi: job %d has a null pointer", k); return PPQHIP_ERR_INVALID_VALUE;
        }
        bytes += 4.0 * (double)jobs[k].n;
    }
    hipStream_t s = (hipStream_t)stream;
    LaunchScope scope(K_MINMAX_T, bytes, s);
    for (int base = 0; base < num_jobs; base += kMinMaxMultiMax) {
        MinMaxJobs args;
        args.count = (uint32_t)((num_jobs - base) < kMinMaxMultiMax ? (num_jobs - base) : kMinMaxMultiMax);
        uint32_t tiles = 0;
        int64_t elems = 0;
        for (uint32_t k = 0; k < args.count; k++) {
            const ppqhip_minmax_job& src = jobs[base + k];
            args.job[k].x = src.x; args.job[k].slots = src.slots; args.job[k].n = (uint32_t)src.n;
            args.job[k].first_tile = tiles;
            tiles += mm_job_tiles((uint32_t)src.n, aligned16(src.x));
            elems += src.n;
        }
        args.total_tiles = tiles;
        launch_minmax_persistent(args, elems, s);
    }
    return finish_launch("minmax_t_slots_multi");
}

int ppqhip_minmax_slots_finish(const float* slots, float* minmax, void* stream) {
    hipStream_t s = (hipStream_t)stream;
    hipLaunchKernelGGL(minmax_finish_kernel, dim3(1), dim3(kBlock), 0, s, slots, (uint32_t)ppqhip_minmax_slots(), minmax);
    return finish_launch("minmax_slots_finish");
}

int ppqhip_minmax_c(const float* x, int64_t n, int64_t num_channel, int64_t elem_per_channel, float* mins,
                    float* maxs, void* stream) {
    if (int st = validate(n, "minmax_c")) return st;
    if (num_channel <= 0 || elem_per_channel <= 0 || n % (num_channel * elem_per_channel) != 0) {
        set_error("minmax_c: bad channel geometry"); return PPQHIP_ERR_INVALID_VALUE;
    }
    hipStream_t s = (hipStream_t)stream;
    LaunchScope scope(K_MINMAX_C, 4.0 * (double)n, s);
    const FastDiv nc = make_fastdiv((uint32_t)num_channel);
    if (elem_per_channel >= 64) {
        const int64_t rows = n / elem_per_channel;
        const int vec_ok = (aligned16(x) && elem_per_channel % 4 == 0) ? 1 : 0;
        const uint32_t C = (uint32_t)num_channel, outer = (uint32_t)(rows / num_channel);
        const uint32_t chunks = (uint32_t)((elem_per_channel + kMMCChunk - 1) / kMMCChunk);
        uint32_t K = 1;
        if (chunks == 1) {
            K = (uint32_t)(rows / (num_cu() * kMMCWavesPerCu));
            const uint32_t k_bytes = (uint32_t)(65536 / (elem_per_channel * 4));
            if (K > k_bytes) K = k_bytes;
            if (K > outer) K = outer;
            if (K < 1) K = 1;
        }
        const uint32_t groups = (outer + K - 1) / K;
        const uint32_t items = groups * C * chunks;
        hipLaunchKernelGGL(minmax_c_wave_kernel, dim3((items + kBlock / kWave - 1) / (kBlock / kWave)), dim3(kBlock), 0, s, x,
                           (uint32_t)elem_per_channel, vec_ok, C, outer, K, chunks, items, mins, maxs);
    } else {
        const int use_lds = num_channel <= 4096;
        const size_t lds = use_lds ? 2 * sizeof(float) * (size_t)num_channel : 0;
        hipLaunchKernelGGL(minmax_c_generic_kernel, dim3(stream_grid(n, kBlock * 16, num_cu() * 2)), dim3(kBlock), lds,
                           s, x, (uint32_t)n, make_fastdiv((uint32_t)elem_per_channel), nc, use_lds, mins, maxs);
    }
    return finish_launch("minmax_c");
}

int ppqhip_channel_sum(const float* x, int64_t n, int64_t num_channel, int64_t elem_per_channel, double* sums,
                       void* stream) {
    if (int st = validate(n, "channel_sum")) return st;
    if (num_channel <= 0 || elem_per_channel <= 0 || n % (num_channel * elem_per_channel) != 0) {
        set_error("channel_sum: bad channel geometry"); return PPQHIP_ERR_INVALID_VALUE;
    }
    hipStream_t s = (hipStream_t)stream;
    LaunchScope scope(K_CHANNEL_SUM, 4.0 * (double)n, s);
    const uint32_t C = (uint32_t)num_channel, epc = (uint32_t)elem_per_channel;
    const uint32_t outer = (uint32_t)(n / (num_channel * elem_per_channel));
    if (epc >= 64 && epc % 4 == 0 && aligned16(x) && C >= 2u * (uint32_t)num_cu()) {
        hipLaunchKernelGGL(channel_sum_single_kernel, dim3(C), dim3(kBlock), 0, s, x, outer, C, epc, sums);
    } else if (epc >= 64) {
        uint32_t S = (4 * (uint32_t)num_cu() + C - 1) / C;
        if (S > outer) S = outer;
        if (S < 1) S = 1;
        double* partial = (double*)scratch(s, sizeof(double) * (size_t)S * C);
        if (partial == nullptr) return PPQHIP_ERR_HIP;
        const int vec_ok = (aligned16(x) && epc % 4 == 0) ? 1 : 0;
        hipLaunchKernelGGL(channel_sum_row_kernel, dim3(C, S), dim3(kBlock), 0, s, x, outer, C, epc, vec_ok, partial);
        hipLaunchKernelGGL(channel_sum_finish_kernel, dim3((C + kBlock - 1) / kBlock), dim3(kBlock), 0, s, partial, S,
                           C, sums);
    } else {
        hipLaunchKernelGGL(channel_sum_generic_kernel, dim3((C + kBlock - 1) / kBlock), dim3(kBlock), 0, s, x, outer,
                           C, epc, sums);
    }
    return finish_launch("channel_sum");
}

int ppqhip_isotone_t(const float* x, int64_t n, float* dest, void* workspace, void* stream) {
    if (int st = validate(n, "isotone_t")) return st;
    if (workspace == nullptr) { set_error("isotone_t: workspace is null"); return PPQHIP_ERR_INVALID_VALUE; }
    hipStream_t s = (hipStream_t)stream;
    LaunchScope scope(K_ISOTONE, 4.0 * (double)n, s);
    Top2* partial = (Top2*)workspace;
    const int grid = stream_grid(n, kBlock * 8, kIsotoneBlocks);
    hipLaunchKernelGGL(isotone_kernel, dim3(grid), dim3(kBlock), 0, s, x, (uint32_t)n, (const Top2*)nullptr, 0u,
                       partial, (float*)nullptr, (uint32_t)n);
    hipLaunchKernelGGL(isotone_kernel, dim3(1), dim3(kBlock), 0, s, (const float*)nullptr, 0u, (const Top2*)partial,
                       (uint32_t)grid, (Top2*)nullptr, dest, (uint32_t)n);
    return finish_launch("isotone_t");
}

int ppqhip_minmax_c_multi(const ppqhip_minmax_c_job* jobs, int num_jobs, void* stream) {
    if (num_jobs <= 0) return PPQHIP_OK;
    if (jobs == nullptr) { set_error("minmax_c_multi: jobs is null"); return PPQHIP_ERR_INVALID_VALUE; }
    hipStream_t s = (hipStream_t)stream;
    double bytes = 0.0;
// ... 49 lines not shown
```

ppq_amd/ffi.py:

```python
import math
import threading
import weakref
from typing import List

import numpy as np
import torch

from . import _lib
from ._lib import lib

_KERNEL_FAILURE = 'Kernel Failure, '


_raw_stream = torch._C._cuda_getCurrentRawStream
_get_device = torch._C._cuda_getDevice


def _stream() -> int:
    return _raw_stream(_get_device())


def _check(t: torch.Tensor, dtype: torch.dtype, name: str) -> None:
    if not isinstance(t, torch.Tensor):
        raise TypeError(f'{name}: expected a torch.Tensor, got {type(t)}')
# ... 40 lines not shown
    return int(shape[channel_axis]), epc


class _DeviceOf:
    __slots__ = ('idx', 'prev')

    def __init__(self, t: torch.Tensor):
        self.idx = t.device.index
        self.prev = None

    def __enter__(self):
        if self.idx is not None and self.idx != _get_device():
            self.prev = _get_device()
            torch.cuda.set_device(self.idx)

    def __exit__(self, *a):
        if self.prev is not None:
            torch.cuda.set_device(self.prev)


_workspaces = {}
_MAX_WORKSPACES = 16


def _workspace(device: torch.device, nbytes: int) -> torch.Tensor:
    key = (device.index, _stream())
    ws = _workspaces.pop(key, None)
    if ws is None or ws.numel() < nbytes:
        ws = torch.empty(max(nbytes, 1 << 16), dtype=torch.uint8, device=device)
    _workspaces[key] = ws
    while len(_workspaces) > _MAX_WORKSPACES:
        _workspaces.pop(next(iter(_workspaces)))
    return ws


_MINMAX_JOB = np.dtype([('x', '<u8'), ('slots', '<u8'), ('n', '<i8')])
_FQ_JOB = np.dtype([('x', '<u8'), ('scale', '<u8'), ('offset', '<u8'), ('out', '<u8'), ('n', '<i8'),
                    ('num_channel', '<i8'), ('elem_per_channel', '<i8'), ('clip_min', '<i4'), ('clip_max', '<i4')])
_FQ_FLOAT_JOB = np.dtype([('x', '<u8'), ('scale', '<u8'), ('offset', '<u8'), ('out', '<u8'), ('n', '<i8'),
                          ('num_channel', '<i8'), ('elem_per_channel', '<i8'), ('exponent', '<i4'), ('mantissa', '<i4'),
                          ('clip_min', '<f4'), ('clip_max', '<f4')])
_FLOAT_SEARCH_JOB = np.dtype([('x', '<u8'), ('rows', '<i8'), ('row_len', '<i8'), ('exponent', '<i4'), ('mantissa', '<i4'),
                              ('clip_min', '<f4'), ('clip_max', '<f4')])
_LSQ_JOB = np.dtype([('x', '<u8'), ('scale', '<u8'), ('offset', '<u8'), ('grad_y', '<u8'), ('grad_x', '<u8'), ('grad_s', '<u8'),
                     ('n', '<i8'), ('num_channel', '<i8'), ('elem_per_channel', '<i8'), ('clip_min', '<i4'), ('clip_max', '<i4')])
_LSQ_FINISH_JOB = np.dtype([('partial', '<u8'), ('grad_s', '<u8'), ('n', '<i8'), ('clip_min', '<i4'), ('clip_max', '<i4')])
_MINMAX_C_JOB = np.dtype([('x', '<u8'), ('mins', '<u8'), ('maxs', '<u8'), ('n', '<i8'), ('num_channel', '<i8'),
                          ('elem_per_channel', '<i8'), ('fresh', '<i4'), ('reserved', '<i4')])
_QUANTILE_JOB = np.dtype([('x', '<u8'), ('dest', '<u8'), ('hint', '<u8'), ('n', '<i8')])

_owner_hints = weakref.WeakKeyDictionary()
_hint_owner = threading.local()


def quantile_hint(device: torch.device) -> torch.Tensor:
    return torch.zeros(8, dtype=torch.int32, device=device)


class quantile_hint_owner:
    __slots__ = ('owner', 'prev')

    def __init__(self, owner):
        self.owner, self.prev = owner, None

    def __enter__(self):
        self.prev = getattr(_hint_owner, 'current', None)
        _hint_owner.current = self.owner
        return self

    def __exit__(self, *a):
        _hint_owner.current = self.prev


def _owner_quantile_hint(device: torch.device, numel: int, q: float):
    owner = getattr(_hint_owner, 'current', None)
    if owner is None: return None
    try: per = _owner_hints.setdefault(owner, {})
    except TypeError: return None
    key = (device.index, int(numel), float(q))
    h = per.get(key)
    if h is None: h = per[key] = quantile_hint(device)
    return h


_HIST_JOB = np.dtype([('x', '<u8'), ('rows', '<u8'), ('n', '<i8'), ('p0', '<f4'), ('p1', '<f4')])


def _epilogue_geometry(ts, bias_list):
    t0 = ts[0]
    if not isinstance(t0, torch.Tensor) or t0.dtype is not _F32 or not t0.is_cuda or t0.dim() != 4 or t0.numel() == 0:
        return None
    shape, strides, dev = t0.shape, t0.stride(), t0.device
    for t in ts[1:]:
        if not isinstance(t, torch.Tensor) or t.dtype is not _F32 or t.device != dev or t.shape != shape or t.stride() != strides:
            return None
    C = int(shape[1])
    for bias in bias_list:
        if (not isinstance(bias, torch.Tensor) or bias.dtype is not _F32 or bias.device != dev or bias.dim() != 1
                or bias.numel() != C or not bias.is_contiguous()):
            return None
    if t0.is_contiguous(): return C, int(shape[2]) * int(shape[3])
    if t0.is_contiguous(memory_format=torch.channels_last): return C, 1
    return None


def bias_act_(y: torch.Tensor, bias: torch.Tensor, relu: bool) -> bool:
    geo = _epilogue_geometry([y], [bias])
    if geo is None: return False
    with _DeviceOf(y):
        _raise(lib.ppqhip_bias_act(y.data_ptr(), bias.data_ptr(), y.numel(), geo[0], geo[1], 1 if relu else 0, _stream()))
    return True


def bias_add_act(a: torch.Tensor, bias_a: torch.Tensor, b: torch.Tensor, bias_b, relu: bool):
    geo = _epilogue_geometry([a, b], [bias_a] if bias_b is None else [bias_a, bias_b])
    if geo is None or a.data_ptr() == b.data_ptr(): return None
    out = torch.empty_like(a)
    with _DeviceOf(a):
        _raise(lib.ppqhip_bias_add_act(a.data_ptr(), bias_a.data_ptr(), b.data_ptr(), 0 if bias_b is None else bias_b.data_ptr(),
                                       out.data_ptr(), a.numel(), geo[0], geo[1], 1 if relu else 0, _stream()))
    return out


def _sink_slots(job, dev) -> int:
    if job is None: return 0
    slots = job[1]
    if (job[0] != 'minmax' or slots.dtype is not _F32 or slots.device != dev or not slots.is_contiguous()
            or slots.numel() != 2 * lib.ppqhip_minmax_slots()): raise ValueError('no sink for this job')
    return slots.data_ptr()


def _fused_or_raise(status: int) -> bool:
    if status == _lib.NOT_FUSED: return False
    _raise(status)
    return True


def bias_act_stats_(y: torch.Tensor, bias: torch.Tensor, relu: bool, job) -> bool:
    geo = _epilogue_geometry([y], [bias])
    if geo is None or job is None: return False
    try: slots = _sink_slots(job, y.device)
    except ValueError: return False
    with _DeviceOf(y):
        return _fused_or_raise(lib.ppqhip_bias_act_stats(y.data_ptr(), bias.data_ptr(), y.numel(), geo[0], geo[1],
                                                         1 if relu else 0, slots, _stream()))


ELIDE_A, ELIDE_B = 1, 2


def bias_add_act_stats(a: torch.Tensor, bias_a: torch.Tensor, b: torch.Tensor, bias_b, relu: bool, job_a, job_b, job_out,
                       elide: int = 0):
    geo = _epilogue_geometry([a, b], [bias_a] if bias_b is None else [bias_a, bias_b])
    if geo is None or a.data_ptr() == b.data_ptr(): return None
    if bias_b is None and job_b is not None: return None
    try: slots = [_sink_slots(j, a.device) for j in (job_a, job_b, job_out)]
    except ValueError: return None
    if not any(slots): return None
    out = torch.empty_like(a)
    args = (a.data_ptr(), bias_a.data_ptr(), b.data_ptr(), 0 if bias_b is None else bias_b.data_ptr(), out.data_ptr(),
            a.numel(), geo[0], geo[1], 1 if relu else 0, slots[0], slots[1], slots[2])
    with _DeviceOf(a):
        if elide: ok = _fused_or_raise(lib.ppqhip_bias_add_act_stats2(*args, int(elide), _stream()))
        else: ok = _fused_or_raise(lib.ppqhip_bias_add_act_stats(*args, _stream()))
    return out if ok else None


def _sink_rows(job, dev) -> tuple:
    if job is None: return 0, 0.0, 0.0
    if job[0] != 'hist_rows': raise ValueError('no sink for this job')
    rows = job[1]
    if (rows.dtype is not torch.int32 or rows.device != dev or rows.dim() != 2 or not rows.is_contiguous()
            or rows.shape[0] != lib.ppqhip_hist_rows()): raise ValueError('no sink for this job')
    return rows.data_ptr(), float(job[3]), float(job[4])


def _hist_rule(jobs):
    rules = {(int(j[1].shape[1]), bool(j[2]), bool(j[5])) for j in jobs if j is not None}
    return next(iter(rules)) if len(rules) == 1 else None


def bias_act_hist_(y: torch.Tensor, bias: torch.Tensor, relu: bool, job) -> bool:
    geo = _epilogue_geometry([y], [bias])
    if geo is None or job is None: return False
    try: rows, p0, p1 = _sink_rows(job, y.device)
    except ValueError: return False
    bins, asym, clip = _hist_rule([job])
    with _DeviceOf(y):
        return _fused_or_raise(lib.ppqhip_bias_act_hist(y.data_ptr(), bias.data_ptr(), y.numel(), geo[0], geo[1],
                                                        1 if relu else 0, rows, p0, p1, bins, int(asym), int(clip), _stream()))


def bias_add_act_hist(a: torch.Tensor, bias_a: torch.Tensor, b: torch.Tensor, bias_b, relu: bool, job_a, job_b, job_out,
                      elide: int = 0):
    geo = _epilogue_geometry([a, b], [bias_a] if bias_b is None else [bias_a, bias_b])
    if geo is None or a.data_ptr() == b.data_ptr(): return None
    if bias_b is None and job_b is not None: return None
    try: sinks = [_sink_rows(j, a.device) for j in (job_a, job_b, job_out)]
    except ValueError: return None
    rule = _hist_rule([job_a, job_b, job_out])
    if rule is None: return None
    out = torch.empty_like(a)
    with _DeviceOf(a):
        ok = _fused_or_raise(lib.ppqhip_bias_add_act_hist(
            a.data_ptr(), bias_a.data_ptr(), b.data_ptr(), 0 if bias_b is None else bias_b.data_ptr(), out.data_ptr(),
            a.numel(), geo[0], geo[1], 1 if relu else 0, *sinks[0], *sinks[1], *sinks[2], rule[0], int(rule[1]), int(rule[2]),
            int(elide), _stream()))
    return out if ok else None


_ADAROUND_JOB = np.dtype([('w', '<u8'), ('v', '<u8'), ('scale', '<u8'), ('offset', '<u8'), ('out', '<u8'), ('dy', '<u8'),
                          ('n', '<i8'), ('num_channel', '<i8'), ('elem_per_channel', '<i8'), ('qmin', '<i4'), ('qmax', '<i4')])
_ROUNDTUNE_JOB = np.dtype([('w', '<u8'), ('r', '<u8'), ('scale', '<u8'), ('offset', '<u8'), ('out', '<u8'),
                           ('n', '<i8'), ('num_channel', '<i8'), ('elem_per_channel', '<i8'), ('qmin', '<i4'), ('qmax', '<i4')])


def _weight_map_table(label, dtype, items, outs, dys=None):
    n = len(items)
    if len(outs) != n or (dys is not None and len(dys) != n):
        raise RuntimeError(_KERNEL_FAILURE + f'{label}: argument lists differ in length')
    jobs = np.zeros(n, dtype=dtype)
    dev = items[0][0].device
    for k, (w, v, s, o, axis, qmin, qmax) in enumerate(items):
        ts = [('Value', w), ('Rounding', v), ('Scale', s), ('Offset', o), ('Out', outs[k])] + ([('Dy', dys[k])] if dys is not None else [])
        for name, t in ts:
            _f32(t, name)
            if t.device != dev: raise RuntimeError(_KERNEL_FAILURE + f'{label}: item {k}: {name} is on another device')
            if not t.is_contiguous(): raise RuntimeError(_KERNEL_FAILURE + f'{label}: item {k}: {name} is not contiguous')
        for name, t in ts[1:2] + ts[4:]:
            if t.shape != w.shape: raise RuntimeError(_KERNEL_FAILURE + f'{label}: item {k}: {name} is not shaped like the weight')
        C, epc = _geometry(w.shape, axis) if axis is not None else (1, w.numel())
        if s.numel() != C or o.numel() != C:
            raise RuntimeError(_KERNEL_FAILURE + f'{label}: item {k}: scale / offset need {C} elements')
        ptrs = [t.data_ptr() for _, t in ts[:5]]
        if 'dy' in dtype.names: ptrs.append(dys[k].data_ptr() if dys is not None else 0)
        jobs[k] = (*ptrs, w.numel(), C, epc, int(qmin), int(qmax))
    return jobs


def adaround_forward_multi(items, outs=None) -> List[torch.Tensor]:
    if not items: return []
    if outs is None: outs = [torch.empty_like(it[0]) for it in items]
    jobs = _weight_map_table('AdaRound', _ADAROUND_JOB, items, outs)
    with _DeviceOf(items[0][0]):
        _raise(lib.ppqhip_adaround_fwd_multi(jobs.ctypes.data, len(items), _stream()))
    return outs


def adaround_backward_multi(items, dys, reg: torch.Tensor, dvs=None) -> List[torch.Tensor]:
    if not items: return []
    _f32(reg, 'Reg')
    if reg.numel() != 3 or not reg.is_contiguous() or reg.device != items[0][0].device:
        raise RuntimeError(_KERNEL_FAILURE + 'AdaRound: reg must be a contiguous float32[3] on the weights\' device')
    if dvs is None: dvs = [torch.empty_like(it[0]) for it in items]
    jobs = _weight_map_table('AdaRound', _ADAROUND_JOB, items, dvs, dys)
    with _DeviceOf(items[0][0]):
        _raise(lib.ppqhip_adaround_bwd_multi(jobs.ctypes.data, len(items), reg.data_ptr(), _stream()))
    return dvs


def roundtune_forward_multi(items, outs=None) -> List[torch.Tensor]:
    if not items: return []
    if outs is None: outs = [torch.empty_like(it[0]) for it in items]
    jobs = _weight_map_table('RoundTuning', _ROUNDTUNE_JOB, items, outs)
    with _DeviceOf(items[0][0]):
        _raise(lib.ppqhip_roundtune_fwd_multi(jobs.ctypes.data, len(items), _stream()))
    return outs


_EQ_SEGMENT = np.dtype([('base', '<u8'), ('extent', '<i8'), ('div', '<i8'), ('a', '<i8'), ('b', '<i8'), ('outer', '<i8'),
                        ('stride', '<i8'), ('run', '<i8'), ('multiplier', '<f4'), ('downstream', '<i4')])
_EQ_SCALE_JOB = np.dtype([('segments', '<u8'), ('scale', '<u8'), ('num_segments', '<i4'), ('num_channel', '<i4'),
                          ('value_threshold', '<f4'), ('reserved', '<i4')])
_EQ_APPLY_JOB = np.dtype([('x', '<u8'), ('scale', '<u8'), ('n', '<i8'), ('run', '<i8'), ('inner', '<i8'), ('group_out', '<i8'),
                          ('num_scale', '<i8'), ('divide', '<i4'), ('reserved', '<i4')])


def _eq_tensor(t, what: str, k: int, dev):
    _f32(t, what)
    if t.device != dev: raise RuntimeError(_KERNEL_FAILURE + f'Equalization: item {k}: {what} is on another device')
    if not t.is_contiguous(): raise RuntimeError(_KERNEL_FAILURE + f'Equalization: item {k}: {what} is not contiguous')


def _segment_record(segment, k: int, dev, what: str = 'Value') -> tuple:
    t, div, a, b, outer, stride, run, mult, down = segment
    _eq_tensor(t, what, k, dev)
    return (t.data_ptr(), t.numel(), int(div), int(a), int(b), int(outer), int(stride), int(run), float(mult), 1 if down else 0)


class EqualizeTable:
    __slots__ = ('jobs', 'segments', 'keep', 'entry')
# ... 956 lines not shown
    def RoundingLoss_LC_B(value, dy, scale, offset, clip_min: int, clip_max: int, channel_axis: int,
                          rounding: int) -> torch.Tensor:
        _f32(value, 'Value'); _f32(scale, 'Scale'); _f32(offset, 'Offset'); _f32(dy, 'Gard')
        v = value.contiguous()
        C, epc = _geometry(v.shape, channel_axis)
        dx = torch.empty_like(v)
        with _DeviceOf(v):
            _raise(lib.ppqhip_rounding_loss_bwd(v.data_ptr(), dy.data_ptr(), scale.contiguous().data_ptr(),
                                                offset.contiguous().data_ptr(), dx.data_ptr(), v.numel(), C, epc,
                                                int(clip_min), int(clip_max), int(rounding), _stream()))
        return dx

    @ staticmethod
    def compute_mse_loss(hist: list, start: int, step: int, end: int) -> float:
        import ctypes
        arr = (ctypes.c_int64 * len(hist))(*[int(v) for v in hist])
        return float(lib.ppqhip_mse_loss_host(arr, len(hist), int(start), int(step), int(end)))

    @ staticmethod
    def MinMax_T(value, minmax) -> None:
        _f32(value, 'Value'); _f32(minmax, 'MinMax')
        v = _dense(value)
        with _DeviceOf(v):
            ws = _workspace(v.device, lib.ppqhip_minmax_workspace_bytes(v.numel()))
            _raise(lib.ppqhip_minmax_t(v.data_ptr(), v.numel(), minmax.data_ptr(), ws.data_ptr(), _stream()))

    @ staticmethod
    def MinMax_T_Slots(value, slots) -> None:
        _f32(value, 'Value'); _f32(slots, 'Slots')
        if slots.numel() != 2 * lib.ppqhip_minmax_slots() or not slots.is_contiguous():
            raise RuntimeError(_KERNEL_FAILURE + f'slots must be a contiguous [{lib.ppqhip_minmax_slots()}, 2] tensor')
        v = _dense(value)
        with _DeviceOf(v):
            _raise(lib.ppqhip_minmax_t_slots(v.data_ptr(), v.numel(), slots.data_ptr(), _stream()))

    @ staticmethod
    def MinMax_T_Slots_Multi(values, slots) -> None:
        if len(values) != len(slots): raise RuntimeError(_KERNEL_FAILURE + 'values / slots length mismatch')
        if not values: return
        S = 2 * lib.ppqhip_minmax_slots()
        vs = []
        for v, sl in zip(values, slots):
            _f32(v, 'Value'); _f32(sl, 'Slots')
            if sl.numel() != S or not sl.is_contiguous() or sl.device != values[0].device or v.device != values[0].device:
                raise RuntimeError(_KERNEL_FAILURE + 'slots must be contiguous [minmax_slots(), 2] tensors on the values\' device')
            vs.append(_dense(v))
        jobs = np.empty(len(vs), dtype=_MINMAX_JOB)
        jobs['x'] = [v.data_ptr() for v in vs]
        jobs['slots'] = [sl.data_ptr() for sl in slots]
        jobs['n'] = [v.numel() for v in vs]
        with _DeviceOf(vs[0]):
            _raise(lib.ppqhip_minmax_t_slots_multi(jobs.ctypes.data, len(vs), _stream()))

    @ staticmethod
    def Histogram_T_Rows_Multi(values, rows, p0, p1, asymmetric: bool, clip_outliers: bool) -> None:
        if not (len(values) == len(rows) == len(p0)) or (asymmetric and len(p1) != len(values)):
            raise RuntimeError(_KERNEL_FAILURE + 'values / rows / parameter length mismatch')
        if not values: return
        R, bins = lib.ppqhip_hist_rows(), rows[0].shape[-1]
        vs = []
        for v, r in zip(values, rows):
            _f32(v, 'Value'); _check(r, torch.int32, 'Rows(Expect to be INT32)')
            if (r.ndim != 2 or r.shape[0] != R or r.shape[1] != bins or not r.is_contiguous()
                    or r.device != values[0].device or v.device != values[0].device):
                raise RuntimeError(_KERNEL_FAILURE + f'rows must be contiguous [{R}, {bins}] tensors on the values\' device')
            vs.append(_dense(v))
        jobs = np.empty(len(vs), dtype=_HIST_JOB)
        jobs['x'] = [v.data_ptr() for v in vs]
        jobs['rows'] = [r.data_ptr() for r in rows]
        jobs['n'] = [v.numel() for v in vs]
        jobs['p0'] = np.asarray(p0, dtype=np.float32)
        jobs['p1'] = np.asarray(p1, dtype=np.float32) if asymmetric else 0.0
        with _DeviceOf(vs[0]):
            _raise(lib.ppqhip_hist_t_rows_multi(jobs.ctypes.data, len(vs), int(bool(asymmetric)),
                                                int(bool(clip_outliers)), bins, _stream()))

    @ staticmethod
    def MinMax_Slots_Finish(slots, minmax) -> None:
        _f32(slots, 'Slots'); _f32(minmax, 'MinMax')
        with _DeviceOf(slots):
            _raise(lib.ppqhip_minmax_slots_finish(slots.data_ptr(), minmax.data_ptr(), _stream()))

    @ staticmethod
    def Histogram_T_Rows(value, hist_scale: float, clip_outliers: bool, rows) -> None:
        _f32(value, 'Value'); _check(rows, torch.int32, 'Rows(Expect to be INT32)')
        R = lib.ppqhip_hist_rows()
        if rows.ndim != 2 or rows.shape[0] != R or not rows.is_contiguous():
            raise RuntimeError(_KERNEL_FAILURE + f'rows must be a contiguous [{R}, bins] tensor')
        v = _dense(value)
        with _DeviceOf(v):
            _raise(lib.ppqhip_hist_sym_t_rows(v.data_ptr(), v.numel(), float(hist_scale), int(bool(clip_outliers)),
                                              rows.data_ptr(), rows.shape[1], _stream()))

    @ staticmethod
    def Histogram_Asymmetric_T_Rows(min: float, max: float, value, clip_outliers: bool, rows) -> None:
        _f32(value, 'Value'); _check(rows, torch.int32, 'Rows(Expect to be INT32)')
        R = lib.ppqhip_hist_rows()
        if rows.ndim != 2 or rows.shape[0] != R or not rows.is_contiguous():
            raise RuntimeError(_KERNEL_FAILURE + f'rows must be a contiguous [{R}, bins] tensor')
        v = _dense(value)
        with _DeviceOf(v):
            _raise(lib.ppqhip_hist_asym_t_rows(v.data_ptr(), v.numel(), float(min), float(max),
                                               int(bool(clip_outliers)), rows.data_ptr(), rows.shape[1], _stream()))

    @ staticmethod
    def Histogram_Rows_Finish(rows, hist) -> None:
        _check(rows, torch.int32, 'Rows(Expect to be INT32)'); _HipExtension._check_hist(hist)
        with _DeviceOf(rows):
            _raise(lib.ppqhip_hist_rows_finish(rows.data_ptr(), rows.shape[1], hist.data_ptr(), _stream()))

    @ staticmethod
    def MinMax_C(value, channel_axis: int, mins, maxs) -> None:
        _f32(value, 'Value'); _f32(mins, 'Mins'); _f32(maxs, 'Maxs')
        v = _dense(value, channel_axis)
        C, epc = _geometry(v.shape, channel_axis)
        if mins.numel() != C or maxs.numel() != C:
            raise RuntimeError(_KERNEL_FAILURE + f'mins / maxs need {C} elements')
        with _DeviceOf(v):
            _raise(lib.ppqhip_minmax_c(v.data_ptr(), v.numel(), C, epc, mins.data_ptr(), maxs.data_ptr(), _stream()))

    @ staticmethod
    def MinMax_C_Multi(values, channel_axes, mins, maxs, fresh: bool = False):
        n = len(values)
        if n == 0: return
        if not (len(channel_axes) == len(mins) == len(maxs) == n):
            raise RuntimeError(_KERNEL_FAILURE + 'MinMax_C_Multi: argument lists differ in length')
        dev = values[0].device
        jobs = np.empty(n, dtype=_MINMAX_C_JOB)
        keep = []
        for k in range(n):
            _f32(values[k], 'Value'); _f32(mins[k], 'Mins'); _f32(maxs[k], 'Maxs')
            if values[k].device != dev: raise RuntimeError(_KERNEL_FAILURE + 'MinMax_C_Multi: one device per call')
            v = _dense(values[k], channel_axes[k])
            C, epc = _geometry(v.shape, channel_axes[k])
            if mins[k].numel() != C or maxs[k].numel() != C or not mins[k].is_contiguous() or not maxs[k].is_contiguous():
                raise RuntimeError(_KERNEL_FAILURE + f'MinMax_C_Multi: item {k} needs contiguous float32[{C}] mins / maxs')
            owns = bool(fresh[k] if isinstance(fresh, (list, tuple)) else fresh)
            if owns and not (v.numel() == C * epc and epc <= 8192):
                if isinstance(fresh, (list, tuple)):
                    raise RuntimeError(_KERNEL_FAILURE + f'MinMax_C_Multi: item {k} cannot be `fresh` (see minmax_c_fresh_ok)')
                owns = False
            keep.append(v)
            jobs[k] = (v.data_ptr(), mins[k].data_ptr(), maxs[k].data_ptr(), v.numel(), C, epc, 1 if owns else 0, 0)
        with _DeviceOf(values[0]):
            _raise(lib.ppqhip_minmax_c_multi(jobs.ctypes.data, n, _stream()))

    @ staticmethod
    def minmax_c_outer_is_one(value, channel_axis: int) -> bool:
        C, epc = _geometry(value.shape, channel_axis)
        return value.numel() == C * epc

    @ staticmethod
    def minmax_c_fresh_ok(value, channel_axis: int) -> bool:
        C, epc = _geometry(value.shape, channel_axis)
        return value.numel() == C * epc and epc <= 8192

    @ staticmethod
    def ChannelSum(value, channel_axis: int, sums) -> None:
        _f32(value, 'Value'); _check(sums, torch.float64, 'Sums(Expect to be FP64)')
        v = value.contiguous()
        C, epc = _geometry(v.shape, channel_axis)
        if sums.numel() != C: raise RuntimeError(_KERNEL_FAILURE + f'sums needs {C} elements')
        with _DeviceOf(v):
            _raise(lib.ppqhip_channel_sum(v.data_ptr(), v.numel(), C, epc, sums.data_ptr(), _stream()))

    @ staticmethod
# ... 313 lines not shown
                                                 rounding, channel_axis)

    @ staticmethod
    def MinMax_T(tensor, minmax):
        HIP_EXTENSION.MinMax_T(tensor, minmax)
        return minmax

    @ staticmethod
    def MinMax_C(tensor, channel_axis: int, mins, maxs):
        HIP_EXTENSION.MinMax_C(tensor, channel_axis, mins, maxs)
        return mins, maxs

    @ staticmethod
    def MinMax_C_Multi(tensors, channel_axes, mins, maxs, fresh: bool = False):
        return HIP_EXTENSION.MinMax_C_Multi(tensors, channel_axes, mins, maxs, fresh)

    @ staticmethod
    def minmax_c_fresh_ok(tensor, channel_axis: int) -> bool:
        return HIP_EXTENSION.minmax_c_fresh_ok(tensor, channel_axis)

    @ staticmethod
    def minmax_c_outer_is_one(tensor, channel_axis: int) -> bool:
        return HIP_EXTENSION.minmax_c_outer_is_one(tensor, channel_axis)

    @ staticmethod
    def ChannelSum(tensor, channel_axis: int, sums):
        HIP_EXTENSION.ChannelSum(tensor, channel_axis % tensor.ndim, sums)
        return sums

    @ staticmethod
    def ChannelMean(tensor, channel_axis: int) -> torch.Tensor:
        axis = channel_axis % tensor.ndim
        sums = torch.zeros(tensor.shape[axis], dtype=torch.float64, device=tensor.device)
        HIP_EXTENSION.ChannelSum(tensor, axis, sums)
        return (sums / (tensor.numel() // tensor.shape[axis])).to(torch.float32)

    @ staticmethod
    def minmax_slots() -> int: return int(lib.ppqhip_minmax_slots())

    @ staticmethod
    def hist_rows() -> int: return int(lib.ppqhip_hist_rows())

    @ staticmethod
    def MinMax_T_Slots(tensor, slots):
        HIP_EXTENSION.MinMax_T_Slots(tensor, slots)
        return slots

    @ staticmethod
    def MinMax_Slots_Finish(slots, minmax):
        HIP_EXTENSION.MinMax_Slots_Finish(slots, minmax)
        return minmax

    @ staticmethod
    def MinMax_T_Slots_Multi(tensors, slots):
        HIP_EXTENSION.MinMax_T_Slots_Multi(tensors, slots)
        return slots

    @ staticmethod
    def Histogram_T_Rows_Multi(tensors, rows, scales, clip_outliers: bool = True):
        HIP_EXTENSION.Histogram_T_Rows_Multi(tensors, rows, scales, None, False, clip_outliers)
        return rows

    @ staticmethod
    def Histogram_Asymmetric_T_Rows_Multi(min_values, max_values, tensors, rows, clip_outliers: bool = True):
        HIP_EXTENSION.Histogram_T_Rows_Multi(tensors, rows, min_values, max_values, True, clip_outliers)
        return rows

    @ staticmethod
    def Histogram_T_Rows(tensor, rows, scale: float, clip_outliers: bool = True):
        HIP_EXTENSION.Histogram_T_Rows(tensor, scale, clip_outliers, rows)
        return rows

    @ staticmethod
    def Histogram_Asymmetric_T_Rows(min_value: float, max_value: float, tensor, rows, clip_outliers: bool = True):
        HIP_EXTENSION.Histogram_Asymmetric_T_Rows(min_value, max_value, tensor, clip_outliers, rows)
        return rows

    @ staticmethod
    def Histogram_Rows_Finish(rows, histogram):
        HIP_EXTENSION.Histogram_Rows_Finish(rows, histogram)
        return histogram

    @ staticmethod
    def FloatScaleSearch(items, candidates, rounding: int = 0):
        return HIP_EXTENSION.FloatScaleSearch(items, candidates, rounding)

    @ staticmethod
    def KLLosses(histogram, num_of_bits: int = 8):
        return HIP_EXTENSION.KL_Losses(histogram, num_of_bits)

    @ staticmethod
    def MseSearch(histogram, hist_scale, min_value, quant_min: int, quant_max: int, symmetrical: bool):
        return HIP_EXTENSION.MSE_Search(histogram, hist_scale, min_value, quant_min, quant_max, symmetrical)

    @ staticmethod
    def MXQuantize(tensor, format, axis: int, block_size: int = MX_BLOCK, scale_codes=None):
        if block_size != MX_BLOCK: raise ValueError(f'MX block size is {MX_BLOCK}, got {block_size}')
        fmt = mx_format_id(format)
        _f32(tensor, 'Value')
        axis = _mx_axis(tensor.dim(), axis)
        v = _mx_dense(tensor, axis)
        outer, length, inner, codes_shape = _mx_geometry(v, axis)
        codes = None
        if scale_codes is not None:
            if not (isinstance(scale_codes, torch.Tensor) and scale_codes.dtype == torch.uint8 and list(scale_codes.shape) == codes_shape):
                raise RuntimeError(_KERNEL_FAILURE + f'scale_codes must be a uint8 tensor of shape {codes_shape}')
            if scale_codes.device != v.device: raise RuntimeError(_KERNEL_FAILURE + 'scale_codes is on another device')
            codes = scale_codes if scale_codes.stride() == _mx_codes_like(v, axis, codes_shape).stride() else _mx_codes_like(v, axis, codes_shape)
        out = torch.empty_like(v)
        with _DeviceOf(v):
            _raise(lib.ppqhip_mx_fq(v.data_ptr(), out.data_ptr(), codes.data_ptr() if codes is not None else 0, outer, length, inner,
                                    fmt, _stream()))
        if codes is not None and codes is not scale_codes: scale_codes.copy_(codes)
        return out

    @ staticmethod
    def MXPack(tensor, format, axis: int, block_size: int = MX_BLOCK):
        if block_size != MX_BLOCK: raise ValueError(f'MX block size is {MX_BLOCK}, got {block_size}')
        fmt = mx_format_id(format)
        _f32(tensor, 'Value')
        axis = _mx_axis(tensor.dim(), axis)
        v = _mx_dense(tensor, axis)
        outer, length, inner, _ = _mx_geometry(v, axis)
        eshape, sshape = mx_packed_shapes(v.shape, axis, fmt)
        elements = torch.empty(eshape, dtype=torch.uint8, device=v.device)
        scales = torch.empty(sshape, dtype=torch.uint8, device=v.device)
        with _DeviceOf(v):
            _raise(lib.ppqhip_mx_pack(v.data_ptr(), elements.data_ptr(), scales.data_ptr(), outer, length, inner, fmt, _stream()))
        return elements, scales

    @ staticmethod
    def MXUnpack(elements, scales, format, shape, axis: int):
        fmt = mx_format_id(format)
        shape = [int(d) for d in shape]
        axis = _mx_axis(len(shape), axis)
        _check(elements, torch.uint8, 'Elements(Expect to be UINT8)'); _check(scales, torch.uint8, 'Scales(Expect to be UINT8)')
        eshape, sshape = mx_packed_shapes(shape, axis, fmt)
        if list(elements.shape) != eshape or list(scales.shape) != sshape:
            raise RuntimeError(_KERNEL_FAILURE + f'elements / scales of shape {list(elements.shape)} / {list(scales.shape)}, expected {eshape} / {sshape}')
        if scales.device != elements.device: raise RuntimeError(_KERNEL_FAILURE + 'scales is on another device')
        elements, scales = elements.contiguous(), scales.contiguous()
        out = torch.empty(shape, dtype=torch.float32, device=elements.device)
        outer, length, inner, _ = _mx_geometry(out, axis)
        with _DeviceOf(out):
            _raise(lib.ppqhip_mx_unpack(elements.data_ptr(), scales.data_ptr(), out.data_ptr(), outer, length, inner, fmt, _stream()))
        return out

    @ staticmethod
    def MXMatmul(a_elements, a_scales, a_format, b_elements, b_scales, b_format, k: int, bias=None):
        a_elements, a_scales, fa, b_elements, b_scales, fb, k, bias, m, n = _mx_matmul_args(a_elements, a_scales, a_format, b_elements, b_scales, b_format, k, bias)
        out = torch.empty([m, n], dtype=torch.float32, device=a_elements.device)
        with _DeviceOf(out):
            _raise(lib.ppqhip_mx_gemm(a_elements.data_ptr(), a_scales.data_ptr(), fa, b_elements.data_ptr(), b_scales.data_ptr(), fb,
                                      bias.data_ptr() if bias is not None else 0, out.data_ptr(), m, n, k, _stream()))
        return out

    @ staticmethod
    def MXMatmulFused(a_elements, a_scales, a_format, b_elements, b_scales, b_format, k: int, bias=None, residual=None, relu: bool = False,
                      out_format=None, out_float: bool = True):
        a_elements, a_scales, fa, b_elements, b_scales, fb, k, bias, m, n = _mx_matmul_args(a_elements, a_scales, a_format, b_elements, b_scales, b_format, k, bias)
        fo, residual = _mx_fused_args(out_format, out_float, residual, [m, n], a_elements.device)
        dev = a_elements.device
        out = torch.empty([m, n], dtype=torch.float32, device=dev) if out_float else None
        elements = scales = None
        if out_format is not None:
            eshape, sshape = mx_packed_shapes([m, n], 1, fo)
# ... 45 lines not shown
```

ppq_amd/harness.py:

```python
from typing import Callable, Dict, List, Optional

import torch
import torch.nn.functional as F

from .core import LinearQuantizationConfig, QuantizationStates, TensorQuantizationConfig, is_initial
from .core import QuantizationProperty as P
from .qfunction import PPQuantFunction

PASSIVE_OPERATIONS = {'MaxPool', 'GlobalMaxPool', 'Reshape', 'Flatten', 'Identity', 'Dropout', 'Slice', 'Pad', 'Resize',
                      'Split', 'Transpose', 'Interp', 'Squeeze', 'Unsqueeze'}
COMPUTING_OP = {'Conv', 'Gemm', 'ConvTranspose', 'MatMul'}


class Variable:
    def __init__(self, name: str, value: torch.Tensor = None, is_parameter: bool = False):
        self.name = name
        self.value = value
        self.stored_value = None
        self.is_parameter = is_parameter
        self.dest_ops: List['Operation'] = []
        self.source_op: Optional['Operation'] = None

    def __hash__(self): return hash(self.name)
    def __eq__(self, o): return isinstance(o, Variable) and o.name == self.name
# ... 38 lines not shown
                var.stored_value = parked

    @ property
    def config_with_variable(self):
        return list(zip(self.config.input_quantization_config, self.inputs)) + \
            list(zip(self.config.output_quantization_config, self.outputs))

    def dequantize(self):
        if getattr(self, '_dequantized', False): return self
        for cfg, _ in self.config_with_variable:
            cfg.detail['Stored State'] = cfg.state
            cfg.state = QuantizationStates.FP32
        self._swap_parameters()
        self._dequantized = True
        return self

    def restore_quantize_state(self):
        if not getattr(self, '_dequantized', False): return self
        for cfg, _ in self.config_with_variable:
            if 'Stored State' in cfg.detail: cfg.state = cfg.detail.pop('Stored State')
        self._swap_parameters()
        self._dequantized = False
        return self

    def baking_parameters(self, quant_func: Callable):
        for config, var in self.config_with_variable:
            if var.is_parameter and QuantizationStates.is_activated(config.state):
                var.value = quant_func(var.value, config)
                config.state = (QuantizationStates.BAKED if config.state == QuantizationStates.ACTIVATED
                                else QuantizationStates.PASSIVE_BAKED)


class BaseGraph:
    def __init__(self, name: str):
        self.name = name
        self.operations: Dict[str, Operation] = {}
        self.variables: Dict[str, Variable] = {}
        self.inputs: Dict[str, Variable] = {}
        self.outputs: Dict[str, Variable] = {}

    def create_variable(self, name: str, value=None, is_parameter=False) -> Variable:
        v = Variable(name, value, is_parameter)
        self.variables[name] = v
        return v

    def create_operation(self, op_type: str, name: str, inputs: List[Variable], attributes: dict = None) -> Variable:
        out = self.create_variable(name + '_out')
        op = Operation(name, op_type, attributes, list(inputs), [out])
        out.source_op = op
        for v in inputs: v.dest_ops.append(op)
        self.operations[name] = op
        return out

    def topological_sort(self) -> List[Operation]:
        return list(self.operations.values())


def _forward(op: Operation, x: List[torch.Tensor]):
    t, a = op.type, op.attributes
    if t == 'Conv':
        return F.conv2d(x[0], x[1], x[2] if len(x) > 2 else None, stride=a.get('strides', 1),
                        padding=a.get('pads', 0), groups=a.get('group', 1))
    if t == 'Gemm': return F.linear(x[0], x[1], x[2] if len(x) > 2 else None)
    if t == 'MatMul': return torch.matmul(x[0], x[1])
    if t == 'Relu': return F.relu(x[0])
    if t == 'Gelu': return F.gelu(x[0])
    if t == 'Add': return x[0] + x[1]
    if t == 'MaxPool': return F.max_pool2d(x[0], a['kernel_shape'], a.get('strides', 1), a.get('pads', 0))
    if t == 'GlobalAveragePool': return F.adaptive_avg_pool2d(x[0], 1)
    if t == 'Flatten': return torch.flatten(x[0], 1)
    if t == 'LayerNormalization': return F.layer_norm(x[0], x[0].shape[-1:], x[1], x[2])
    if t == 'Softmax': return F.softmax(x[0], dim=a.get('axis', -1))
    if t == 'Mul': return x[0] * (x[1] if len(x) > 1 else a['value'])
    if t == 'Reshape': return x[0].reshape(a['shape'])
    if t == 'Transpose': return x[0].permute(a['perm'])
    if t == 'Concat': return torch.cat([v.expand(x[-1].shape[0], *v.shape[1:]) if v.shape[0] == 1 else v for v in x],
                                       dim=a.get('axis', 1))
    if t == 'Slice': return x[0].narrow(a['axis'], a['start'], a['length'])
    if t == 'Resize': return F.interpolate(x[0], scale_factor=a.get('scale', 2), mode=a.get('mode', 'nearest'))
    raise NotImplementedError(f'Graph op: {op.name}({op.type}) has no backend implementation')


class EpilogueGroup:
    __slots__ = ('kind', 'ops', 'convs', 'add', 'relu', 'keep')

    def __init__(self, kind, ops, convs, add, relu, keep=()):
        self.kind, self.ops, self.convs, self.add, self.relu, self.keep = kind, ops, convs, add, relu, frozenset(keep)

    def __repr__(self): return f'{self.kind}({", ".join(op.name for op in self.ops)})'


def _in_cfg(op, i):
    return op.config.input_quantization_config[i] if isinstance(op, QuantableOperation) else None


def _out_cfg(op, i):
    return op.config.output_quantization_config[i] if isinstance(op, QuantableOperation) else None


def plan_epilogues(operations: List[Operation], hooks: Dict[str, object] = None, keep=(), passes_through: Callable = None,
                   grad_enabled: bool = False) -> List[EpilogueGroup]:
    if grad_enabled: return []
    from .observer import CalibrationHook
    hooks = hooks or {}
    keep = set(keep)
    if passes_through is None:
        def passes_through(c): return not QuantizationStates.is_activated(c.state)

    def through(*cfgs): return all(c is None or passes_through(c) for c in cfgs)

    def hooks_ok(members, unwritten):
        for op in members:
            h = hooks.get(op.name)
            if h is None: continue
            if type(h) is not CalibrationHook: return False
            if any(c is not None and c in h._observer_table for c in unwritten): return False
        return True

    def conv_ok(op):
        return (op.type == 'Conv' and len(op.inputs) == 3 and op.inputs[2].is_parameter and len(op.outputs) == 1
                and op.outputs[0].name not in keep)

    def only_feeds(v, op): return len(v.dest_ops) == 1 and v.dest_ops[0] is op

    def relu_after(op, i):
        if i >= len(operations): return None
        r = operations[i]
        out = op.outputs[0]
        if r.type != 'Relu' or len(r.inputs) != 1 or r.inputs[0] is not out or not only_feeds(out, r) or out.name in keep:
            return None
        return r

    def try_p2(i):
        for n_conv in (2, 1):
            j = i + n_conv
            if j + 1 >= len(operations): continue
            add, convs = operations[j], operations[i:j]
            if add.type != 'Add' or len(add.inputs) != 2 or len(add.outputs) != 1 or not all(conv_ok(c) for c in convs): continue
            by_out = {c.outputs[0].name: c for c in convs}
            x0, x1 = add.inputs
            if x0.name not in by_out or x0 is x1: continue
            if n_conv == 2 and x1.name not in by_out: continue
            ordered = [by_out[x0.name]] + ([by_out[x1.name]] if n_conv == 2 else [])
            if not all(only_feeds(c.outputs[0], add) for c in convs): continue
            relu = relu_after(add, j + 1)
            if relu is None: continue
            unwritten = (_out_cfg(add, 0), _in_cfg(relu, 0))
            between = [_out_cfg(c, 0) for c in convs] + [_in_cfg(add, 0), _in_cfg(add, 1)]
            if not through(*unwritten, *between): return None
            members = list(operations[i:j + 2])
            if not hooks_ok(members, unwritten): return None
            return EpilogueGroup('P2', members, ordered, add, relu, keep)
        return None

    def try_p1(i):
        conv = operations[i]
        if not conv_ok(conv): return None
        relu = relu_after(conv, i + 1)
        if relu is None: return None
        unwritten = (_out_cfg(conv, 0), _in_cfg(relu, 0))
        if not through(*unwritten) or not hooks_ok([conv, relu], unwritten): return None
        return EpilogueGroup('P1', [conv, relu], [conv], None, relu, keep)

    groups, i = [], 0
    while i < len(operations):
        g = try_p2(i) if operations[i].type == 'Conv' else None
        if g is None and operations[i].type == 'Conv': g = try_p1(i)
        if g is None:
            i += 1
            continue
        groups.append(g)
        i += len(g.ops)
    return groups


def elidable_stores(grp: EpilogueGroup, hooks, jobs: Dict[str, tuple], recorder=None) -> set:
    if grp.kind != 'P2' or recorder is not None or not hooks: return set()
    add_hook = hooks.get(grp.add.name)
    out = set()
    for conv in grp.convs:
        v, hook = conv.outputs[0], hooks.get(conv.name)
        if len(v.dest_ops) != 1 or v.dest_ops[0] is not grp.add or v.name in grp.keep: continue
        if conv.name not in jobs or hook is None or not isinstance(conv, QuantableOperation): continue
        obs = [hook._observer_table.get(c) for c in conv.config.output_quantization_config]
        if len(obs) != 1 or obs[0] is None or not obs[0].reads_only_its_job(): continue
        if add_hook is not None and isinstance(grp.add, QuantableOperation) and any(
                c in add_hook._observer_table for x, c in zip(grp.add.inputs, grp.add.config.input_quantization_config) if x is v):
            continue
        out.add(conv.name)
    return out


class TorchExecutor:
    def __init__(self, graph: BaseGraph, device: str = 'cuda'):
        self._graph = graph
        self._device = device
        self._default_quant_fn = PPQuantFunction
        self.cache_parameter_quantization = False
        self._param_cache: Dict[str, tuple] = {}
        self.fuse_parameter_quantization = True
        self._plans: list = []
        self._plan_signature = None
        self._plan_cache: Dict[tuple, list] = {}
        self._fused: Dict[tuple, torch.Tensor] = {}
        self._delegates: Dict[object, Callable] = {}
        self._overrides: Dict[str, Callable] = {}
        self._takes_packed: set = set()
        self._group_overrides: Dict[str, tuple] = {}
        self.fuse_epilogues = True
        self._epilogue_cache: Dict[tuple, dict] = {}
        self.channels_last = False
        for v in graph.variables.values():
            if v.is_parameter and v.value is not None: v.value = v.value.to(device)

    def use_channels_last(self) -> 'TorchExecutor':
        self.channels_last = True
        for v in self._graph.variables.values():
            if v.is_parameter and isinstance(v.value, torch.Tensor) and v.value.dim() == 4:
                v.value = v.value.contiguous(memory_format=torch.channels_last)
        return self

    def _place(self, value: torch.Tensor) -> torch.Tensor:
        value = value.to(self._device)
        if self.channels_last and value.dim() == 4: value = value.contiguous(memory_format=torch.channels_last)
        return value

    def register_quantize_delegate(self, config, delegator: Callable) -> None:
        self._delegates[config] = delegator

    def remove_quantize_delegate(self, config) -> None:
        self._delegates.pop(config, None)

    def register_operation_override(self, op_name: str, fn: Callable, takes_packed: bool = False) -> None:
        if op_name not in self._graph.operations: raise KeyError(f'register_operation_override: the graph has no operation {op_name!r}')
        if not callable(fn): raise TypeError(f'register_operation_override: fn must be callable, got {type(fn)}')
        self._overrides[op_name] = fn
        if takes_packed: self._takes_packed.add(op_name)
        else: self._takes_packed.discard(op_name)

    def remove_operation_override(self, op_name: str) -> None:
        self._overrides.pop(op_name, None)
        self._takes_packed.discard(op_name)

    def register_group_override(self, op_names: List[str], fn: Callable) -> None:
        if not op_names: raise ValueError('register_group_override: no operations')
        for name in op_names:
            if name not in self._graph.operations: raise KeyError(f'register_group_override: the graph has no operation {name!r}')
        if not callable(fn): raise TypeError(f'register_group_override: fn must be callable, got {type(fn)}')
        self._group_overrides[op_names[0]] = (tuple(op_names), fn)

    def remove_group_override(self, first_name: str) -> None:
        self._group_overrides.pop(first_name, None)

    def _group_plan(self, operations: List[Operation], hooks, output_names, all_float: bool) -> Dict[str, tuple]:
        if not self._group_overrides: return {}
        hooks = hooks or {}
        keep = set(self._graph.outputs) | set(output_names or ())
        at = {op.name: i for i, op in enumerate(operations)}
        plan = {}
        for first, (names, fn) in self._group_overrides.items():
            if any(n not in at or n in hooks for n in names): continue
            if any(at[a] >= at[b] for a, b in zip(names, names[1:])): continue
            ops = [operations[at[n]] for n in names]
            if any(v.name in keep for m in ops[:-1] for v in m.outputs): continue
            need = set()
            for v in ops[-1].outputs:
                handed = [d.name in self._takes_packed and d.name in self._overrides and d.name not in hooks and d.name in at
                          and d.inputs[0] is v and sum(1 for x in d.inputs if x is v) == 1 for d in v.dest_ops]
                if all_float or v.name in keep or not handed or not all(handed): need.add(v.name)
            plan[first] = (ops, fn, need)
        return plan

# ... 71 lines not shown
                    qin = [self._quantize_parameter(v, c) if v.is_parameter else self.quantize_function(x, c)
                           for v, x, c in zip(op.inputs, raw_in, op.config.input_quantization_config)]
                else: qin = raw_in
                outs = _forward(op, qin)
            outs = list(outs) if isinstance(outs, (list, tuple)) else [outs]
            if isinstance(op, QuantableOperation):
                outs = [self.quantize_function(y, c) for y, c in zip(outs, op.config.output_quantization_config)]
            for v, y in zip(op.outputs, outs):
                v.value = y
                if v.name in output_names: results[output_names.index(v.name)] = y
        for v in g.variables.values():
            if not v.is_parameter: v.value = None
        return results

    def _fused_parameters(self, operations=None) -> None:
        self._fused = {}
        if not self.fuse_parameter_quantization or self._default_quant_fn is not PPQuantFunction: return
        from .ffi import FloatingQuantizePlan, LinearQuantizePlan
        todo, sig = [], []
        for op in (self._graph.operations.values() if operations is None else operations):
            if not isinstance(op, QuantableOperation): continue
            for v, c in zip(op.inputs, op.config.input_quantization_config):
                if not (v.is_parameter and isinstance(v.value, torch.Tensor) and v.value.is_cuda): continue
                if not QuantizationStates.is_activated(c.state) or c in self._delegates: continue
                pol = c.policy
                floating = pol.has_property(P.FLOATING)
                if not (pol.has_property(P.LINEAR) or floating) or pol.has_property(P.DYNAMIC): continue
                if v.value.dtype != torch.float32 or v.value.requires_grad or v.value.numel() == 0: continue
                if not (isinstance(c.scale, torch.Tensor) and isinstance(c.offset, torch.Tensor)): continue
                axis = c.channel_axis if pol.has_property(P.PER_CHANNEL) else None
                if not LinearQuantizePlan.accepts(v.value, c.scale, c.offset, axis): continue
                rnd = int(getattr(c.rounding, 'value', c.rounding))
                todo.append((v, c, axis, rnd, floating))
                sig.append((v.name, id(c), v.value.data_ptr(), c.scale.data_ptr(), c.offset.data_ptr(), tuple(v.value.shape), c.scale.numel(),
                            axis, c.quant_min, c.quant_max, rnd, floating,
                            (c.exponent_bits, c.mantissa_bits) if floating else None))
        if not todo:
            self._plans, self._plan_signature = [], None
            return
        cached = self._plan_cache.get(tuple(sig))
        if cached is not None:
            self._plan_cache[tuple(sig)] = self._plan_cache.pop(tuple(sig))
            self._plans, self._plan_signature = cached, sig
        if sig != self._plan_signature:
            groups: Dict[tuple, list] = {}
            for item in todo: groups.setdefault((item[3], item[4]), []).append(item)
            self._plans = []
            for (rnd, floating), items in groups.items():
                if floating:
                    plan = FloatingQuantizePlan([(v.value, c.scale, c.offset, axis, c.exponent_bits, c.mantissa_bits,
                                                  c.quant_min, c.quant_max) for v, c, axis, _, _ in items], rounding=rnd)
                else:
                    plan = LinearQuantizePlan([(v.value, c.scale, c.offset, axis, c.quant_min, c.quant_max)
                                               for v, c, axis, _, _ in items], rounding=rnd)
                self._plans.append((plan, [(v.name, id(c)) for v, c, _, _, _ in items]))
            self._plan_signature = sig
            if len(self._plan_cache) >= 8: self._plan_cache.pop(next(iter(self._plan_cache)))
            self._plan_cache[tuple(sig)] = self._plans
        for plan, keys in self._plans:
            for key, out in zip(keys, plan.run()): self._fused[key] = out

    def _epilogue_plan(self, operations: List[Operation], hooks, output_names, grouped=()) -> Dict[str, EpilogueGroup]:
        if not self.fuse_epilogues or torch.is_grad_enabled() or self._default_quant_fn is not PPQuantFunction: return {}
        states = tuple(c.state for op in operations if isinstance(op, QuantableOperation)
                       for c in (*op.config.input_quantization_config, *op.config.output_quantization_config))
        sig = (tuple(op.name for op in operations), tuple((k, id(h)) for k, h in hooks.items()) if hooks else (),
               tuple(output_names or ()), tuple(id(c) for c in self._delegates), states, tuple(sorted(self._overrides)), tuple(sorted(grouped)))
        plan = self._epilogue_cache.get(sig)
        if plan is None:
            delegates = self._delegates

            def passes_through(c): return not QuantizationStates.is_activated(c.state) and c not in delegates
            groups = plan_epilogues(operations, hooks, set(self._graph.outputs) | set(output_names or ()), passes_through)
            if self._overrides:
                groups = [g for g in groups if not any(m.name in self._overrides and not (hooks and m.name in hooks) for m in g.ops)]
            if grouped:
                groups = [g for g in groups if not any(m.name in grouped for m in g.ops)]
            plan = {g.ops[0].name: g for g in groups}
            if len(self._epilogue_cache) >= 8: self._epilogue_cache.pop(next(iter(self._epilogue_cache)))
            self._epilogue_cache[sig] = plan
        return plan

    def _run_epilogue(self, grp: EpilogueGroup, raw_of: Callable, hooks) -> Optional[Dict[str, torch.Tensor]]:
        from .ffi import (ELIDE_A, ELIDE_B, bias_act_, bias_act_hist_, bias_act_stats_, bias_add_act, bias_add_act_hist,
                          bias_add_act_stats)
        for conv in grp.convs:
            x, w = raw_of(conv.inputs[0]), conv.inputs[1].value
            if not (isinstance(x, torch.Tensor) and x.is_cuda and x.dtype == torch.float32 and x.dim() == 4
                    and isinstance(w, torch.Tensor) and w.dim() == 4): return None
            fmt = torch.channels_last if self.channels_last else torch.contiguous_format
            if not (x.is_contiguous(memory_format=fmt) and w.is_contiguous(memory_format=fmt)): return None
        if grp.add is not None:
            b_var = grp.add.inputs[1]
            if b_var.source_op not in grp.convs:
                b = raw_of(b_var)
                if not (isinstance(b, torch.Tensor) and b.is_cuda and b.dtype == torch.float32): return None
        hooks = hooks or {}
        ys, biases, qins = {}, {}, {}
        for conv in grp.ops[:len(grp.convs)]:
            raw_in = [raw_of(v) for v in conv.inputs]
            qin, in_cfgs = raw_in, None
            if isinstance(conv, QuantableOperation):
                in_cfgs = list(conv.config.input_quantization_config)
                qin = [self._quantize_parameter(v, c) if v.is_parameter else self.quantize_function(x, c)
                       for v, x, c in zip(conv.inputs, raw_in, in_cfgs)]
            hook = hooks.get(conv.name)
            if hook is not None: qin = hook.pre_forward_hook(inputs=raw_in, quant_inputs=qin, quant_configs=in_cfgs)
            a = conv.attributes
            ys[conv.name] = F.conv2d(qin[0], qin[1], None, stride=a.get('strides', 1), padding=a.get('pads', 0),
                                     groups=a.get('group', 1))
            biases[conv.name] = qin[2]
            qins[conv.name] = qin
        if grp.kind == 'P1':
            conv = grp.convs[0]
            y = ys[conv.name]
            stored = {grp.relu.name: y}
            fed = self._epilogue_sinks(grp, hooks, stored, y)
            if fed is not None:
                job = fed[0].get(grp.relu.name)
                launch = bias_act_hist_ if job is not None and job[0] == 'hist_rows' else bias_act_stats_
                if not launch(y, biases[conv.name], True, job): fed = None
            if fed is None and not bias_act_(y, biases[conv.name], relu=True):
                y.add_(biases[conv.name].view(1, -1, 1, 1)).relu_()
            tail, elided = {conv.name: y, grp.relu.name: y}, set()
        else:
            conv_a = grp.convs[0]
            a = ys[conv_a.name]
            conv_b = grp.convs[1] if len(grp.convs) > 1 else None
            b = ys[conv_b.name] if conv_b is not None else raw_of(grp.add.inputs[1])
            bias_b = biases[conv_b.name] if conv_b is not None else None
            stored = {conv_a.name: a, grp.relu.name: None}
            if conv_b is not None: stored[conv_b.name] = b
            fed, out, elided = self._epilogue_sinks(grp, hooks, stored, a), None, set()
            if fed is not None:
                jobs = fed[0]
                elided = elidable_stores(grp, hooks, jobs, fed[1].recorder)
                mask = (ELIDE_A if conv_a.name in elided else 0) | (ELIDE_B if conv_b is not None and conv_b.name in elided else 0)
                launch = bias_add_act_hist if next(iter(jobs.values()))[0] == 'hist_rows' else bias_add_act_stats
                out = launch(a, biases[conv_a.name], b, bias_b, True, jobs.get(conv_a.name),
                             jobs.get(conv_b.name) if conv_b is not None else None, jobs.get(grp.relu.name), mask)
                if out is None: fed, elided = None, set()
                else: stored[grp.relu.name] = out
            if out is None: out = bias_add_act(a, biases[conv_a.name], b, bias_b, relu=True)
            if out is None:
                a.add_(biases[conv_a.name].view(1, -1, 1, 1))
                if conv_b is not None: b.add_(biases[conv_b.name].view(1, -1, 1, 1))
                out = F.relu(a + b)
            tail = {conv_a.name: a, grp.add.name: out, grp.relu.name: out}
            if conv_b is not None: tail[conv_b.name] = b
        if fed is not None:
            for name, job in fed[0].items(): fed[1].prepay(stored[name], job[1])
        values: Dict[str, torch.Tensor] = {}
        for op in grp.ops:
            hook = hooks.get(op.name)
            quantable = isinstance(op, QuantableOperation)
            if op.type != 'Conv':
                raw_in = [values[v.name] if v.name in values else raw_of(v) for v in op.inputs]
                qin, in_cfgs = raw_in, None
                if quantable:
                    in_cfgs = list(op.config.input_quantization_config)
                    qin = [self.quantize_function(x, c) for x, c in zip(raw_in, in_cfgs)]
                if hook is not None: hook.pre_forward_hook(inputs=raw_in, quant_inputs=qin, quant_configs=in_cfgs)
            outs = fp_outs = [tail[op.name]]
            out_cfgs = None
            if quantable:
                out_cfgs = list(op.config.output_quantization_config)
                outs = [self.quantize_function(y, c) for y, c in zip(outs, out_cfgs)]
            if hook is not None:
                outs = hook.post_forward_hook(outputs=fp_outs, quant_outputs=outs, quant_configs=out_cfgs)
            for v, y in zip(op.outputs, outs): values[v.name] = y
        for name in elided:
            for v in next(m for m in grp.ops if m.name == name).outputs: values[v.name] = None
        return values

    @ staticmethod
    def _epilogue_sinks(grp: EpilogueGroup, hooks, stored: Dict[str, torch.Tensor], like: torch.Tensor):
        jobs, queue = {}, None
        for op in grp.ops:
            hook = hooks.get(op.name)
            if hook is None or not isinstance(op, QuantableOperation): continue
            for cfg in op.config.output_quantization_config:
                ob = hook._observer_table.get(cfg)
                if ob is None: continue
                if op.name not in stored or op.name in jobs or hook.stream is not None or ob.queue is None: return None
                if queue is not None and ob.queue is not queue: return None
                job = ob.stat_job(like)
                if job is None: return None
                jobs[op.name], queue = job, ob.queue
        if len({job[0] for job in jobs.values()}) > 1: return None
        return (jobs, queue) if jobs else None

    def _quantize_parameter(self, var: Variable, config) -> torch.Tensor:
        hit = self._fused.get((var.name, id(config)))
        if hit is not None: return hit
        """A parameter and its scale do not change between calibration forwards, so its fake-quantised
        value is computed once and kept resident (the reference recomputes it every forward until
        ParameterBakingPass; same values, ppq/executor/torch.py:516-518).  The cache entry is keyed on
        the identity + version of value, scale and offset and on the config state."""
        if not self.cache_parameter_quantization or not QuantizationStates.is_activated(config.state):
            return self.quantize_function(var.value, config)
        key = (var.value.data_ptr(), var.value._version, id(config.scale), config.scale._version,
               id(config.offset), config.offset._version, int(getattr(config.state, 'value', config.state)))
        hit = self._param_cache.get(var.name)
        if hit is not None and hit[0] == key: return hit[1]
        q = self.quantize_function(var.value, config)
        self._param_cache[var.name] = (key, q)
        return q

    @ torch.no_grad()
    def forward_cached(self, inputs, output_names: List[str], cache: Dict[str, torch.Tensor]) -> List[torch.Tensor]:
        g = self._graph
        if isinstance(inputs, torch.Tensor): inputs = {next(iter(g.inputs)): inputs}
        elif isinstance(inputs, (list, tuple)): inputs = {k: v for k, v in zip(g.inputs, inputs)}
        for name, value in inputs.items():
            if name not in cache: cache[name] = self._place(value)
        need, stack = set(), [g.variables[n] for n in output_names]
        while stack:
            v = stack.pop()
            if v.name in cache or v.is_parameter: continue
            op = v.source_op
            if op is None: raise ValueError(f'forward_cached: graph input {v.name} was not fed')
            if op.name in need: continue
            need.add(op.name)
            stack.extend(op.inputs)
        ops = [op for op in g.topological_sort() if op.name in need]
        if ops: self._fused_parameters(ops)
        groups, packed = self._group_plan(ops, None, output_names, True), {}
        plan, fused_done = (self._epilogue_plan(ops, None, output_names, [m.name for e in groups.values() for m in e[0]]) if ops else {}), set()
        for op in ops:
            if op.name in fused_done: continue
            if op.name in groups:
                vals = self._run_group(groups[op.name], lambda v: v.value if v.is_parameter else cache[v.name], packed)
                members = groups[op.name][0]
                for m in members: fused_done.add(m.name)
                for v in members[-1].outputs: cache[v.name] = vals[v.name]
                continue
            grp = plan.get(op.name)
            vals = (self._run_epilogue(grp, lambda v: v.value if v.is_parameter else cache[v.name], None)
                    if grp is not None else None)
            if vals is not None:
                hidden = grp.relu.inputs[0].name
                for m in grp.ops:
                    fused_done.add(m.name)
                    for v in m.outputs:
                        if v.name != hidden: cache[v.name] = vals[v.name]
                continue
            raw_in = [v.value if v.is_parameter else cache[v.name] for v in op.inputs]
            override = self._overrides.get(op.name)
            if override is not None: outs = override(op, raw_in)
            else:
                if isinstance(op, QuantableOperation):
                    qin = [self._quantize_parameter(v, c) if v.is_parameter else self.quantize_function(x, c)
                           for v, x, c in zip(op.inputs, raw_in, op.config.input_quantization_config)]
                else: qin = raw_in
                outs = _forward(op, qin)
            outs = list(outs) if isinstance(outs, (list, tuple)) else [outs]
            if isinstance(op, QuantableOperation):
                outs = [self.quantize_function(y, c) for y, c in zip(outs, op.config.output_quantization_config)]
            for v, y in zip(op.outputs, outs): cache[v.name] = y
        return [cache[n] for n in output_names]

    @ torch.no_grad()
    def forward(self, inputs, output_names: List[str] = None, hooks: Dict[str, object] = None) -> List[torch.Tensor]:
        g = self._graph
        if isinstance(inputs, torch.Tensor): inputs = {next(iter(g.inputs)): inputs}
        elif isinstance(inputs, (list, tuple)): inputs = {k: v for k, v in zip(g.inputs, inputs)}
        for name, value in inputs.items(): g.variables[name].value = self._place(value)
        stop_early = output_names is not None and not hooks
        if output_names is None: output_names = list(g.outputs)
        results = [None] * len(output_names)
        visited = set()
        self._fused_parameters()
        ops = g.topological_sort()
        groups, packed = self._group_plan(ops, hooks, output_names, False), {}
        plan, fused_done = self._epilogue_plan(ops, hooks, output_names, [m.name for e in groups.values() for m in e[0]]), set()

        def finish(op, outs):
            for v, y in zip(op.outputs, outs):
                v.value = y
                if v.name in output_names: results[output_names.index(v.name)] = y
            visited.add(op.name)
            for v in op.inputs:
                if not v.is_parameter and all(d.name in visited for d in v.dest_ops): v.value = None

        for op in ops:
            if op.name in fused_done: continue
            if op.name in groups:
                vals = self._run_group(groups[op.name], lambda v: v.value, packed)
                for m in groups[op.name][0]:
                    fused_done.add(m.name)
                    finish(m, [vals[v.name] for v in m.outputs])
                if stop_early and all(r is not None for r in results): break
                continue
            grp = plan.get(op.name)
            vals = self._run_epilogue(grp, lambda v: v.value, hooks) if grp is not None else None
            if vals is not None:
                for m in grp.ops:
                    fused_done.add(m.name)
                    finish(m, [vals[v.name] for v in m.outputs])
                if stop_early and all(r is not None for r in results): break
                continue
            hook = hooks.get(op.name) if hooks else None
            raw_in = [v.value for v in op.inputs]
            qin = raw_in
            quantable = isinstance(op, QuantableOperation)
            override = self._overrides.get(op.name) if hook is None else None
            if override is not None: outs = override(op, self._override_inputs(op, raw_in, packed))
            else:
                if quantable:
                    in_cfgs = list(op.config.input_quantization_config)
                    qin = [self._quantize_parameter(v, c) if v.is_parameter else self.quantize_function(x, c)
                           for v, x, c in zip(op.inputs, raw_in, in_cfgs)]
                if hook is not None:
                    qin = hook.pre_forward_hook(inputs=raw_in, quant_inputs=qin, quant_configs=in_cfgs)
                outs = _forward(op, qin)
            outs = list(outs) if isinstance(outs, (list, tuple)) else [outs]
            fp_outs = outs
            if quantable:
                out_cfgs = list(op.config.output_quantization_config)
                outs = [self.quantize_function(y, c) for y, c in zip(outs, out_cfgs)]
            if hook is not None:
                outs = hook.post_forward_hook(outputs=fp_outs, quant_outputs=outs, quant_configs=out_cfgs)
            finish(op, outs)
            if stop_early and all(r is not None for r in results): break
        for v in g.variables.values():
            if not v.is_parameter: v.value = None
        return results

# ... 287 lines not shown
```

ppq_amd/observer.py:

```python
from typing import Dict, List, Optional, Sequence, Tuple

import weakref

import numpy as np
import torch

from .core import (OBSERVER_FLOATING_MSE_FETCHES, OBSERVER_ISOTONE_OBSERVER_AXIS, OBSERVER_KL_HIST_BINS, OBSERVER_KL_HIST_BINS_MANUL_OVERRIDE,
                   OBSERVER_MIN_SCALE, OBSERVER_MIN_SCALE_MANUL_OVERRIDE, OBSERVER_MSE_HIST_BINS,
                   OBSERVER_PERCENTILE, OBSERVER_PERCENTILE_MANUL_OVERRIDE, is_initial, set_activated)
from .core import QuantizationProperty as P
from .core import RoundingPolicy
from .ffi import CUDA, quantile_hint
from .round import ppq_numerical_round, ppq_round_to_power_of_2


def minmax_to_scale_offset(min_val: float, max_val: float, config,
                           scale_threshold: float = OBSERVER_MIN_SCALE) -> Tuple[float, float]:
    if OBSERVER_MIN_SCALE_MANUL_OVERRIDE in config.detail:
        scale_threshold = config.detail[OBSERVER_MIN_SCALE_MANUL_OVERRIDE]
    scale, offset = 1, 0
    if min_val > 0: min_val = 0
    if max_val < 0: max_val = 0
    if config.policy.has_property(P.ASYMMETRICAL):
        range = float(max_val - min_val)
# ... 216 lines not shown
    def pending_range(self) -> Optional[torch.Tensor]:
        return None

    def take_range(self, host: np.ndarray) -> None:
        """Receive the host copy of ``pending_range()`` (fetched for all observers at once)."""

    def reducible(self) -> List[Tuple[torch.Tensor, str]]:
        return []

    def gatherable(self) -> List[torch.Tensor]:
        return []

    def take_gathered(self, merged: List[torch.Tensor]) -> None:
        pass


_RANGE_SEEDS: Dict[object, tuple] = {}


def _range_seed(device) -> tuple:
    hit = _RANGE_SEEDS.get(device)
    if hit is None:
        one = torch.tensor([float('inf'), float('-inf')], dtype=torch.float32, device=device)
        hit = _RANGE_SEEDS[device] = (one, one.repeat(CUDA.minmax_slots(), 1).contiguous())
    return hit


class TorchMinMaxObserver(BaseTensorObserver):
    def __init__(self, watch_on, quant_cfg):
        super().__init__(watch_on, quant_cfg)
        self._range: Optional[torch.Tensor] = None
        self._slots: Optional[torch.Tensor] = None
        self._slots_dirty = False
        self._queued_c = False
        self._host_range: Optional[np.ndarray] = None
        self._observed = False

    @ torch.no_grad()
    def observe(self, value: torch.Tensor):
        assert isinstance(value, torch.Tensor), 'TorchMinMaxObserver can only deal with torch Tensor values'
        assert value.numel() > 0, (f'You are observing an empty tensor({getattr(self._watch_on, "name", "")}).')
        if not is_initial(self._quant_cfg): return
        cfg = self._quant_cfg
        if cfg.policy.has_property(P.PER_TENSOR):
            _, slots = TorchMinMaxObserver.stat_job(self, value)
            if self.queue is not None and value.is_cuda: self.queue.add_minmax(value, slots)
            else: CUDA.MinMax_T_Slots(value, slots)
            self._slots_dirty = True
        elif cfg.policy.has_property(P.PER_CHANNEL):
            queued = (self.queue is not None and value.is_cuda and CUDA.minmax_c_outer_is_one(value, cfg.channel_axis))
            fresh = False
            if self._range is None:
                C = value.shape[cfg.channel_axis]
                self._range = torch.empty((2, C), dtype=torch.float32, device=value.device)
                fresh = queued and CUDA.minmax_c_fresh_ok(value, cfg.channel_axis)
                if not fresh: self._range[0].fill_(float('inf')); self._range[1].fill_(float('-inf'))
            if queued:
                self.queue.add_minmax_c(value, cfg.channel_axis, self._range[0], self._range[1], fresh)
                self._queued_c = True
            else: CUDA.MinMax_C(value, cfg.channel_axis, self._range[0], self._range[1])
        else:
            raise TypeError('Min-max Observer only work with per-tensor or per-channel quantize policy.')
        self._observed = True
        self._host_range = None

    def stat_job(self, value: torch.Tensor) -> Optional[tuple]:
        cfg = self._quant_cfg
        if not is_initial(cfg) or not cfg.policy.has_property(P.PER_TENSOR): return None
        if self._range is None:
            seed = _range_seed(value.device)
            self._range = seed[0].clone()
            self._slots = seed[1].clone()
        return ('minmax', self._slots)

    def _fold(self) -> None:
        if self._queued_c:
            self._drain()
            self._queued_c = False
        if self._slots_dirty:
            self._drain()
            CUDA.MinMax_Slots_Finish(self._slots, self._range)
            self._slots_dirty = False

    def pending_range(self):
        if not (is_initial(self._quant_cfg) and self._observed): return None
        self._fold()
        return self._range

    def take_range(self, host: np.ndarray) -> None:
        self._host_range = host

    def reducible(self):
        if self._range is None: return []
        self._fold()
        if self._range.ndim == 1: return [(self._range[0:1], 'min'), (self._range[1:2], 'max')]
        return [(self._range[0], 'min'), (self._range[1], 'max')]

    def _range_on_host(self) -> np.ndarray:
        if not self._observed:
            raise ValueError('Can not render quantization config yet, Observer data collator is empty. '
                             'Invoke observe() function before render config.')
        if self._host_range is None: _prefetch_siblings(self)
        if self._host_range is None:
            self._fold()
            self._host_range = self._range.cpu().numpy()
        return self._host_range

    def render_quantization_config(self):
        if not is_initial(self._quant_cfg): return
        cfg = self._quant_cfg
        r = self._range_on_host()
        device = self._range.device
        if cfg.policy.has_property(P.PER_TENSOR):
            scale, offset = minmax_to_scale_offset(min_val=float(r[0]), max_val=float(r[1]), config=cfg)
            _set_per_tensor(cfg, scale, offset, device)
        elif cfg.policy.has_property(P.PER_CHANNEL):
            scales, offsets = minmax_to_scale_offset_channels(np.ascontiguousarray(r[0]), np.ascontiguousarray(r[1]), cfg)
            if _DEFERRED_SETS is not None:
                _DEFERRED_SETS.append((cfg, scales, offsets, device))
                return
            cfg.scale = torch.tensor(scales, dtype=torch.float32, device=device)
            cfg.offset = torch.tensor(offsets, dtype=torch.float32, device=device)
            set_activated(cfg)
        else:
            raise TypeError('Min-max Observer only work with per-tensor or per-channel quantize policy.')


class TorchHistObserver(TorchMinMaxObserver):
    def __init__(self, watch_on, quant_cfg, hist_bins: int = OBSERVER_KL_HIST_BINS):
        self._phase = 'Detecting Minmax'
        self._hist = None
        self._rows = None
        self._rows_dirty = False
        self._hist_scale = None
        self._min = None
        self._max = None
        self._losses: Optional[np.ndarray] = None
        if OBSERVER_KL_HIST_BINS_MANUL_OVERRIDE in quant_cfg.detail:
            hist_bins = quant_cfg.detail[OBSERVER_KL_HIST_BINS_MANUL_OVERRIDE]
        self._hist_bins = hist_bins
        super().__init__(watch_on, quant_cfg)

    def observe(self, value: torch.Tensor):
        if not is_initial(self._quant_cfg): return
        assert value.numel() > 0, (f'You are observing an empty tensor({getattr(self._watch_on, "name", "")}).')
        if self._phase == 'Detecting Minmax':
            if self.queue is not None and self.queue.recorder is not None and value.is_cuda:
                self.queue.recorder.append((self, value))
            return super().observe(value)
        elif self._phase == 'Collating Hist':
            self._losses = None
            if getattr(self, '_best', None) is not None: self._best = None
            self._hist_buffers(value)
            if self._quant_cfg.policy.has_property(P.ASYMMETRICAL):
                if self._rows is not None:
                    if self.queue is not None: self.queue.add_hist(value, self._rows, True, self._min, self._max)
                    else: CUDA.Histogram_Asymmetric_T_Rows(self._min, self._max, tensor=value, rows=self._rows)
                    self._rows_dirty = True
                else:
                    CUDA.Histogram_Asymmetric_T(self._min, self._max, tensor=value, histogram=self._hist)
            elif self._quant_cfg.policy.has_property(P.SYMMETRICAL):
                if self._rows is not None:
                    if self.queue is not None: self.queue.add_hist(value, self._rows, False, self._hist_scale)
                    else: CUDA.Histogram_T_Rows(tensor=value, rows=self._rows, scale=self._hist_scale)
                    self._rows_dirty = True
                else:
                    CUDA.Histogram_T(tensor=value, histogram=self._hist, scale=self._hist_scale)
            else:
                raise TypeError('Quantization Property is invalid, expect either ASYMMETRICAL or SYMMETRICAL config here.')

    def _hist_buffers(self, value: torch.Tensor) -> None:
        if self._hist is None:
            self._hist = torch.zeros(size=(self._hist_bins,), dtype=torch.int32, device=value.device)
            if self._hist_bins <= 16384:
                self._rows = torch.zeros(size=(CUDA.hist_rows(), self._hist_bins), dtype=torch.int32,
                                         device=value.device)

    def stat_job(self, value: torch.Tensor) -> Optional[tuple]:
        if self._phase == 'Detecting Minmax': return super().stat_job(value)
        cfg = self._quant_cfg
        if (self._phase != 'Collating Hist' or not is_initial(cfg) or self.queue is None
                or not cfg.policy.has_property(P.PER_TENSOR)): return None
        self._hist_buffers(value)
        if self._rows is None: return None
        if cfg.policy.has_property(P.ASYMMETRICAL): return ('hist_rows', self._rows, True, self._min, self._max, True)
        if cfg.policy.has_property(P.SYMMETRICAL): return ('hist_rows', self._rows, False, self._hist_scale, 0.0, True)
        return None

    def pending_range(self):
        return super().pending_range() if self._phase == 'Detecting Minmax' else None

    def _fold_hist(self) -> None:
        if self._rows_dirty:
            self._drain()
            CUDA.Histogram_Rows_Finish(self._rows, self._hist)
            self._rows_dirty = False
            if self._rows.is_cuda: self._rows.record_stream(torch.cuda.current_stream(self._rows.device))
            self._rows = None

    def histogram(self) -> Optional[torch.Tensor]:
        self._fold_hist()
        return self._hist

    def reducible(self):
        if self._phase == 'Detecting Minmax': return super().reducible()
        return [(self.histogram(), 'sum')] if self._hist is not None else []

    search_kind = 'kl'

    def search_key(self):
        return ('kl', self._hist_bins, self._quant_cfg.num_of_bits)

    def take_losses(self, losses: np.ndarray) -> None:
        self._losses = losses

    def hist_to_scale_offset(self, histogram: torch.Tensor, hist_bins: int, hist_scale: float, config,
                             scale_threshold: float = OBSERVER_MIN_SCALE) -> Tuple[float, int]:
        if config.policy.has_property(P.ASYMMETRICAL):
            raise PermissionError('KL observer is not designed for ASYMMETRICAL quantization')
        if OBSERVER_MIN_SCALE_MANUL_OVERRIDE in config.detail:
            scale_threshold = config.detail[OBSERVER_MIN_SCALE_MANUL_OVERRIDE]
        quant_bins = 2 ** (config.num_of_bits - 1)
        if self._losses is None: _prefetch_siblings(self)
        if self._losses is None:
            self._losses = CUDA.KLLosses(histogram, config.num_of_bits).cpu().numpy()[0]
        losses = [{'kl': float(kl), 'bin_range': (j + 1) * quant_bins} for j, kl in enumerate(self._losses)]
        best_bin_range = sorted(losses, key=lambda x: x['kl'])[0]['bin_range']
        scale, offset = (best_bin_range / self._hist_bins) * hist_scale * (self._hist_bins / quant_bins), 0
        scale = max(scale, scale_threshold)
        if config.policy.has_property(P.POWER_OF_2):
            scale = ppq_round_to_power_of_2(scale, policy=RoundingPolicy.ROUND_HALF_UP)
        return scale, offset

    def render_quantization_config(self):
        if not is_initial(self._quant_cfg): return
        if not self._quant_cfg.policy.has_property(P.PER_TENSOR):
            raise ValueError('Hist observer can only apply with per-tensor quantization config.')
        if self._phase == 'Detecting Minmax':
            r = self._range_on_host()
            min_val, max_val = float(r[0]), float(r[1])
            if self._quant_cfg.policy.has_property(P.SYMMETRICAL):
                hist_range = float(max(abs(max_val), abs(min_val)))
            else:
                hist_range = max_val - min_val
            self._min = min_val
            self._max = max_val
            self._hist_scale = hist_range / self._hist_bins
            self._phase = 'Collating Hist'
        elif self._phase == 'Collating Hist':
            if self._hist is None:
                raise ValueError('Can not render quantization config yet, histogram is empty. '
                                 'Invoke observe() function before render config.')
            scale, offset = self.hist_to_scale_offset(histogram=self.histogram(), hist_bins=self._hist_bins,
                                                      hist_scale=self._hist_scale, config=self._quant_cfg)
            _set_per_tensor(self._quant_cfg, scale, offset, self._hist.device)


class ChannelwiseKLObserver(TorchHistObserver):
    def __init__(self, watch_on, quant_cfg, hist_bins: int = OBSERVER_KL_HIST_BINS):
        super().__init__(watch_on, quant_cfg, hist_bins)
        if not quant_cfg.policy.has_property(P.PER_CHANNEL) or not quant_cfg.policy.has_property(P.SYMMETRICAL):
            raise TypeError('ChannelwiseKLObserver needs a symmetrical per-channel config.')
        self._scales_dev: Optional[torch.Tensor] = None

    def observe(self, value: torch.Tensor):
        if not is_initial(self._quant_cfg): return
        assert value.numel() > 0, (f'You are observing an empty tensor({getattr(self._watch_on, "name", "")}).')
        if self._phase == 'Detecting Minmax':
            return TorchMinMaxObserver.observe(self, value)
        C = value.shape[self._quant_cfg.channel_axis]
# ... 447 lines not shown
        self.stream = stream

    def _observe_all(self, values: list, quant_configs: list) -> None:
        todo = [(v, self._observer_table[c]) for v, c in zip(values, quant_configs) if c in self._observer_table]
        if not todo: return
        if self.stream is None or not todo[0][0].is_cuda:
            for v, ob in todo: ob.observe(v)
            return
        self.stream.wait_stream(torch.cuda.current_stream(todo[0][0].device))
        with torch.cuda.stream(self.stream):
            capturing = torch.cuda.is_current_stream_capturing()
            for v, ob in todo:
                ob.observe(v)
                if not capturing: v.record_stream(self.stream)

    def pre_forward_hook(self, inputs: list, quant_inputs: list, quant_configs: list) -> list:
        self._observe_all(inputs, quant_configs)
        return quant_inputs

    def post_forward_hook(self, outputs: list, quant_outputs: list, quant_configs: list) -> list:
        self._observe_all(outputs, quant_configs)
        return quant_outputs

    def render_quantization_config(self):
        if self.stream is not None: torch.cuda.current_stream().wait_stream(self.stream)
        for _, observer in self._observer_table.items():
            observer.render_quantization_config()
            observer.report()

    def __str__(self) -> str:
        return ''.join([observer.__str__() + '\n' for _, observer in self._observer_table.items()])


class OperationObserver:
    def __init__(self, operation, monitor_parameter: bool = True, monitor_outputs: bool = True,
                 monitor_inputs: bool = True) -> None:
        if not hasattr(operation, 'config'):
            raise TypeError(f'Only QuantableOP instance can apply an Observer, while {type(operation)} was given.')
        self._operation = operation
        self._hook = self.build_hook(monitor_parameter=monitor_parameter, monitor_outputs=monitor_outputs,
                                     monitor_inputs=monitor_inputs)

    def render_quantization_config(self):
        self.hook.render_quantization_config()

    def build_hook(self, monitor_parameter: bool, monitor_outputs: bool, monitor_inputs: bool) -> CalibrationHook:
        observer_table = {}
        for var, config in zip(self._operation.inputs, self._operation.config.input_quantization_config):
            if is_initial(config):
                if var in self._operation.parameters and monitor_parameter:
                    observer_table[config] = TensorObserverFactroy.build_observer(var, config)
                elif monitor_inputs:
                    observer_table[config] = TensorObserverFactroy.build_observer(var, config)
        if monitor_outputs:
            for var, config in zip(self._operation.outputs, self._operation.config.output_quantization_config):
                if is_initial(config):
                    observer_table[config] = TensorObserverFactroy.build_observer(var, config)
        return CalibrationHook(operation=self._operation, observer_table=observer_table)

    @ property
    def hook(self) -> CalibrationHook:
        return self._hook

    def observers(self) -> List[BaseTensorObserver]:
        return list(self._hook._observer_table.values())

    def report(self) -> str:
        return str(self._hook)


def render_observers(observers: Sequence[BaseTensorObserver]) -> None:
    observers = [ob for ob in observers if is_initial(ob._quant_cfg)]
    _prefetch(observers)
    global _DEFERRED_SETS
    _DEFERRED_SETS = pending = []
    try:
        for ob in observers:
            ob.render_quantization_config()
    finally:
        _DEFERRED_SETS = None
        _flush_deferred_sets(pending)


def _prefetch(observers: Sequence[BaseTensorObserver]) -> None:
    pend = [(ob, ob.pending_range()) for ob in observers if getattr(ob, '_host_range', None) is None]
    pend = [(ob, r) for ob, r in pend if r is not None]
    if pend:
        flat = torch.cat([r.reshape(-1) for _, r in pend]).cpu().numpy()
        pos = 0
        for ob, r in pend:
            n = r.numel()
            ob.take_range(flat[pos: pos + n].reshape(tuple(r.shape)))
            pos += n
    groups: Dict[tuple, List[TorchHistObserver]] = {}
    for ob in observers:
        if isinstance(ob, TorchHistObserver) and ob._phase == 'Collating Hist' and ob._hist is not None:
            if ob._losses is not None or getattr(ob, '_best', None) is not None: continue
            if ob._quant_cfg.policy.has_property(P.PER_TENSOR):
                groups.setdefault(ob.search_key(), []).append(ob)
    for key, obs in groups.items():
        hists = torch.stack([ob.histogram() for ob in obs])
        if key[0] == 'kl':
            if any(ob._quant_cfg.policy.has_property(P.ASYMMETRICAL) for ob in obs): continue
            losses = CUDA.KLLosses(hists, key[2]).cpu().numpy()
            for ob, l in zip(obs, losses): ob.take_losses(l)
        else:
            dev = hists.device
            hs = torch.tensor([ob._hist_scale for ob in obs], dtype=torch.float64, device=dev)
            mn = torch.tensor([ob._min for ob in obs], dtype=torch.float64, device=dev)
            best = CUDA.MseSearch(hists, hs, mn, key[2], key[3], key[4]).cpu().numpy()
            for ob, b in zip(obs, best): ob.take_best(b)
    fobs = [ob for ob in observers if isinstance(ob, DirectMSEObserver) and ob._collector]
    if fobs:
        by_round: Dict[int, list] = {}
        for ob in fobs:
            if getattr(ob, '_sse', None) is None:
                by_round.setdefault(int(getattr(ob._quant_cfg.rounding, 'value', ob._quant_cfg.rounding)), []).append(ob)
        for r, obs in by_round.items():
            items = [ob.search_item() for ob in obs]
            sse = CUDA.FloatScaleSearch(items, DirectMSEObserver.SCALE_CANDIDATES, r)
            pos = 0
            for ob, it in zip(obs, items):
                rows = it[0].shape[0]
                ob.take_squared_errors(sse[pos: pos + rows], it[0].shape[1]); pos += rows
        means = [(ob._sse.reshape(-1, len(DirectMSEObserver.SCALE_CANDIDATES)) / ob._count.reshape(-1, 1)) for ob in fobs]
        best = torch.argmin(torch.cat(means), dim=-1).cpu().tolist()
        pos = 0
        for ob, m in zip(fobs, means):
            ob.take_best(best[pos: pos + m.shape[0]]); pos += m.shape[0]
```

Baseline: 3800 samples/s.

## Fuse bias-ReLU epilogue with stem maxpool and batch observer finish kernels

Adds an epilogue kernel that applies bias and ReLU to each plane, stages it in LDS, feeds minmax or histogram sinks, and computes the 3x3 stride-2 maxpool from LDS. When only the pool reads the ReLU output, the full-resolution store can be skipped. Separately, it batches minmax-slot and histogram-row finish reductions across observers into single multi-job launches. The aim is to cut memory traffic for the stem pool and launch overhead at render time. The trade-offs are a large LDS footprint (up to 64KB), which can lower occupancy, and a hardcoded pool geometry that the kernel assumes.

```diff
diff --git a/include/ppq_hip.h b/include/ppq_hip.h
--- a/include/ppq_hip.h
+++ b/include/ppq_hip.h
@@ -191,10 +191,20 @@
 int ppqhip_hist_t_rows_multi(const ppqhip_hist_job* jobs, int num_jobs, int asymmetric,
                              int clip_outliers, int64_t num_bins, void* stream);
 int ppqhip_hist_rows_finish(const int32_t* rows, int64_t num_bins, int32_t* hist, void* stream);
+typedef struct ppqhip_hist_finish_job {
+    const int32_t* rows;
+    int32_t* hist;
+} ppqhip_hist_finish_job;
+int ppqhip_hist_rows_finish_multi(const ppqhip_hist_finish_job* jobs, int num_jobs, int64_t num_bins, void* stream);
 int ppqhip_check_bin_rule(const float* x, int64_t n, float min_value, float hist_scale, int asymmetric, uint64_t* out, void* stream);
 int64_t ppqhip_minmax_slots(void);
 int ppqhip_minmax_t_slots(const float* x, int64_t n, float* slots, void* stream);
 int ppqhip_minmax_slots_finish(const float* slots, float* minmax, void* stream);
+typedef struct ppqhip_minmax_finish_job {
+    const float* slots;
+    float* minmax;
+} ppqhip_minmax_finish_job;
+int ppqhip_minmax_slots_finish_multi(const ppqhip_minmax_finish_job* jobs, int num_jobs, void* stream);
 
 float ppqhip_mse_loss_host(const int64_t* hist, int64_t num_bins, int start, int step, int end);
 
@@ -247,6 +257,14 @@
                              int32_t* rows_a, float p0_a, float p1_a, int32_t* rows_b, float p0_b, float p1_b,
                              int32_t* rows_out, float p0_out, float p1_out, int64_t num_bins, int asymmetric,
                              int clip_outliers, int elide, void* stream);
+
+int ppqhip_bias_act_pool(float* y, const float* bias, float* pooled, int64_t N, int64_t C, int64_t H, int64_t W,
+                         int relu, int elide_y, void* stream);
+int ppqhip_bias_act_pool_stats(float* y, const float* bias, float* pooled, int64_t N, int64_t C, int64_t H, int64_t W,
+                               int relu, float* slots_y, int elide_y, void* stream);
+int ppqhip_bias_act_pool_hist(float* y, const float* bias, float* pooled, int64_t N, int64_t C, int64_t H, int64_t W,
+                              int relu, int32_t* rows_y, float p0_y, float p1_y, int64_t num_bins, int asymmetric,
+                              int clip_outliers, int elide_y, void* stream);
 
 typedef struct ppqhip_adaround_job {
     const float* w;
diff --git a/ppq_amd/_lib.py b/ppq_amd/_lib.py
--- a/ppq_amd/_lib.py
+++ b/ppq_amd/_lib.py
@@ -50,6 +50,10 @@
     'ppqhip_bias_add_act_hist': (c_int, [c_f32p, c_f32p, c_f32p, c_f32p, c_f32p, c_i64, c_i64, c_i64, c_int,
                                          c_i32p, c_flt, c_flt, c_i32p, c_flt, c_flt, c_i32p, c_flt, c_flt, c_i64, c_int, c_int,
                                          c_int, c_vp]),
+    'ppqhip_bias_act_pool': (c_int, [c_f32p, c_f32p, c_f32p, c_i64, c_i64, c_i64, c_i64, c_int, c_int, c_vp]),
+    'ppqhip_bias_act_pool_stats': (c_int, [c_f32p, c_f32p, c_f32p, c_i64, c_i64, c_i64, c_i64, c_int, c_f32p, c_int, c_vp]),
+    'ppqhip_bias_act_pool_hist': (c_int, [c_f32p, c_f32p, c_f32p, c_i64, c_i64, c_i64, c_i64, c_int, c_i32p, c_flt, c_flt,
+                                          c_i64, c_int, c_int, c_int, c_vp]),
     'ppqhip_fq_float_t': (c_int, [c_f32p, c_f32p, c_f32p, c_f32p, c_i64, c_int, c_int, c_flt, c_flt, c_int, c_vp]),
     'ppqhip_fq_float_c': (c_int, [c_f32p, c_f32p, c_f32p, c_f32p, c_i64, c_i64, c_i64, c_int, c_int, c_flt, c_flt,
                                   c_int, c_vp]),
@@ -85,10 +89,12 @@
     'ppqhip_hist_sym_t_rows': (c_int, [c_f32p, c_i64, c_flt, c_int, c_i32p, c_i64, c_vp]),
     'ppqhip_hist_asym_t_rows': (c_int, [c_f32p, c_i64, c_flt, c_flt, c_int, c_i32p, c_i64, c_vp]),
     'ppqhip_hist_rows_finish': (c_int, [c_i32p, c_i64, c_i32p, c_vp]),
+    'ppqhip_hist_rows_finish_multi': (c_int, [c_vp, c_int, c_i64, c_vp]),
     'ppqhip_check_bin_rule': (c_int, [c_f32p, c_i64, c_flt, c_flt, c_int, c_vp, c_vp]),
     'ppqhip_minmax_slots': (c_i64, []),
     'ppqhip_minmax_t_slots': (c_int, [c_f32p, c_i64, c_f32p, c_vp]),
     'ppqhip_minmax_slots_finish': (c_int, [c_f32p, c_f32p, c_vp]),
+    'ppqhip_minmax_slots_finish_multi': (c_int, [c_vp, c_int, c_vp]),
     'ppqhip_mse_loss_host': (c_flt, [ctypes.POINTER(ctypes.c_int64), c_i64, c_int, c_int, c_int]),
     'ppqhip_mse_search_workspace_bytes': (c_i64, [c_i64]),
     'ppqhip_mse_search': (c_int, [c_i32p, c_i64, c_i64, c_f64p, c_f64p, c_int, c_int, c_int, c_i32p, c_vp, c_vp]),
diff --git a/ppq_amd/csrc/epilogue.hip b/ppq_amd/csrc/epilogue.hip
--- a/ppq_amd/csrc/epilogue.hip
+++ b/ppq_amd/csrc/epilogue.hip
@@ -2,6 +2,8 @@
 #include "common.hpp"
 #include "hist_bin.hpp"
 #include "minmax_fold.hpp"
+
+#include <type_traits>
 
 namespace ppqhip {
 namespace {
@@ -77,7 +79,11 @@
                                                          uint32_t elide = 0) {
     EpStored<float4> s{};
     const float4 x = add4(a, ba);
-    if (!RESID) { a4[vv] = s.a = act4<RELU>(x); return s; }
+    if (!RESID) {
+        s.a = act4<RELU>(x);
+        if (!(elide & kElideA)) a4[vv] = s.a;
+        return s;
+    }
     s.a = x;
     if (!(elide & kElideA)) a4[vv] = x;
     float4 y = b;
@@ -305,7 +311,7 @@
     float4* a4 = reinterpret_cast<float4*>(p.a);
     float4* b4 = reinterpret_cast<float4*>(p.b);
     float4* o4 = reinterpret_cast<float4*>(p.out);
-    const uint32_t elide = p.elide;
+    const uint32_t elide = RESID ? p.elide : 0u;
     SINKS sinks;
     sinks.init(sk, lds);
 
@@ -432,6 +438,152 @@
     return finish_launch(what);
 }
 
+struct EpPoolArgs {
+    float* y;
+    const float* bias;
+    float* pooled;
+    uint32_t planes;
+    FastDiv nc;
+    uint32_t nv;
+    uint32_t tiles;
+    int H, W;
+    uint32_t HoWo;
+    FastDiv wo;
+    uint32_t plane_off;
+    uint32_t elide;
+};
+
+constexpr uint32_t kEpPoolLdsBytes = 64u << 10;
+
+struct EpNoSinks {
+    struct Args { int unused; };
+    __device__ __forceinline__ void init(const Args&, int*) {}
+    __device__ __forceinline__ void begin() {}
+    template <bool FULL>
+    __device__ __forceinline__ void feed4(const EpStored<float4>&, bool, bool) {}
+    __device__ __forceinline__ void finish(const Args&, uint32_t, int*) {}
+};
+
+__device__ __forceinline__ void lds_barrier() { asm volatile("s_waitcnt lgkmcnt(0)\n\ts_barrier" ::: "memory"); }
+
+template <int U, bool RELU, class SINKS>
+__global__ __launch_bounds__(kEpStatBlock, (kEpStatBlock * kEpStatWgPerCu + 255) / 256)
+void epilogue_pool_kernel(EpPoolArgs p, typename SINKS::Args sk) {
+    extern __shared__ int lds[];
+    constexpr uint32_t kTile = (uint32_t)kEpStatBlock * U;
+    float* plane = reinterpret_cast<float*>(lds + p.plane_off);
+    float4* plane4 = reinterpret_cast<float4*>(plane);
+    uint32_t pl, pl_end;
+    even_split(p.planes, gridDim.x, blockIdx.x, pl, pl_end);
+    const uint32_t elide = p.elide;
+    SINKS sinks;
+    sinks.init(sk, lds);
+
+    struct Tile { float4 a[U]; float bias; };
+    auto fetch = [&](Tile& T, uint32_t q, uint32_t tile) {
+        const float4* src = reinterpret_cast<const float4*>(p.y) + (size_t)q * p.nv;
+        const uint32_t base = tile * kTile + threadIdx.x;
+#pragma unroll
+        for (int u = 0; u < U; u++) T.a[u] = src[min(base + u * kEpStatBlock, p.nv - 1)];
+        T.bias = p.bias[q - fdiv(q, p.nc) * p.nc.d];
+    };
+    auto consume = [&](const Tile& T, uint32_t q, uint32_t tile, auto full) {
+        constexpr bool FULL = decltype(full)::value;
+        float4* dst = reinterpret_cast<float4*>(p.y) + (size_t)q * p.nv;
+        const uint32_t base = tile * kTile + threadIdx.x;
+        const float4 ba = make_float4(T.bias, T.bias, T.bias, T.bias);
+        EpStored<float4> s[U];
+        bool in[U];
+#pragma unroll
+        for (int u = 0; u < U; u++) {
+            const uint32_t vv = base + u * kEpStatBlock;
+            in[u] = FULL || vv < p.nv;
+            s[u] = EpStored<float4>{};
+            if (in[u]) {
+                s[u] = epilogue_vec<false, false, RELU>(dst, nullptr, nullptr, vv, T.a[u], ba, float4{}, float4{}, elide);
+                plane4[vv] = s[u].a;
+            }
+        }
+#pragma unroll
+        for (int u = 0; u < U; u++) sinks.template feed4<FULL>(s[u], in[u], u == 0);
+    };
+    auto pool = [&](uint32_t q) {
+        lds_barrier();
+        float* out = p.pooled + (size_t)q * p.HoWo;
+        for (uint32_t o = threadIdx.x; o < p.HoWo; o += kEpStatBlock) {
+            const uint32_t oh = fdiv(o, p.wo), ow = o - oh * p.wo.d;
+            const int h0 = 2 * (int)oh - 1, w0 = 2 * (int)ow - 1;
+            float m = -INFINITY;
+#pragma unroll
+            for (int dh = 0; dh < 3; dh++) {
+                const int h = h0 + dh;
+                const float* row = plane + (uint32_t)min(max(h, 0), p.H - 1) * (uint32_t)p.W;
+#pragma unroll
+                for (int dw = 0; dw < 3; dw++) {
+                    const int w = w0 + dw;
+                    const float v = row[min(max(w, 0), p.W - 1)];
+                    const bool inside = (unsigned)h < (unsigned)p.H && (unsigned)w < (unsigned)p.W;
+                    if (inside && (v > m || __builtin_isnan(v))) m = v;
+                }
+            }
+            out[o] = m;
+        }
+        lds_barrier();
+    };
+
+    uint32_t t = 0;
+    auto step = [&](const Tile& cur, Tile& nxt) -> bool {
+        uint32_t nt = t + 1, npl = pl;
+        if (nt == p.tiles) { nt = 0; npl++; }
+        const bool last = npl >= pl_end;
+        fetch(nxt, last ? pl : npl, last ? t : nt);
+        if ((t + 1) * kTile <= p.nv) consume(cur, pl, t, std::true_type{});
+        else consume(cur, pl, t, std::false_type{});
+        if (nt == 0) pool(pl);
+        pl = npl; t = nt;
+        return !last;
+    };
+    Tile ta{}, tb{};
+    fetch(ta, pl, 0);
+    sinks.begin();
+    while (step(ta, tb) && step(tb, ta)) {}
+    sinks.finish(sk, blockIdx.x, lds);
+}
+
+bool fill_pool_geometry(EpPoolArgs& p, int64_t N, int64_t C, int64_t H, int64_t W, uint32_t sink_ints, uint32_t& grid,
+                        size_t& lds_bytes) {
+    const int64_t hw = H * W;
+    if (hw % 4 != 0 || !aligned16(p.y) || !aligned16(p.pooled)) return false;
+    p.plane_off = (sink_ints + 3u) & ~3u;
+    lds_bytes = ((size_t)p.plane_off + (size_t)hw) * sizeof(int);
+    if (lds_bytes > kEpPoolLdsBytes) return false;
+    const int64_t Ho = (H - 1) / 2 + 1, Wo = (W - 1) / 2 + 1;
+    constexpr uint32_t tile = (uint32_t)kEpStatBlock * kEpTileU;
+    p.planes = (uint32_t)(N * C); p.nc = make_fastdiv((uint32_t)C);
+    p.nv = (uint32_t)(hw / 4);
+    p.tiles = (p.nv + tile - 1) / tile;
+    p.H = (int)H; p.W = (int)W;
+    p.HoWo = (uint32_t)(Ho * Wo);
+    p.wo = make_fastdiv((uint32_t)Wo);
+    const uint32_t cap = (uint32_t)(num_cu() * kEpStatWgPerCu);
+    grid = p.planes < cap ? p.planes : cap;
+    return true;
+}
+
+int validate_pool(const char* what, const float* y, const float* bias, const float* pooled, int64_t N, int64_t C, int64_t H,
+                  int64_t W) {
+    constexpr int64_t kMax = 0x7fffffffLL;
+    if (N <= 0 || C <= 0 || H <= 0 || W <= 0 || N > kMax || C > kMax || H > kMax || W > kMax) {
+        set_error("%s: [%lld, %lld, %lld, %lld] is empty or too large", what, (long long)N, (long long)C, (long long)H, (long long)W);
+        return PPQHIP_ERR_INVALID_VALUE;
+    }
+    if (N * C > kMax || H * W > kMax || (N * C) * (H * W) > kMax) {
+        set_error("%s: more than 2^31 - 1 elements", what); return PPQHIP_ERR_INVALID_VALUE;
+    }
+    if (!y || !bias || !pooled) { set_error("%s: null pointer", what); return PPQHIP_ERR_INVALID_VALUE; }
+    return PPQHIP_OK;
+}
+
 void set_hist_rule(EpHistSinks& sk, int k, int32_t* rows, float p0, float p1, const EpHistRule& r) {
     sk.rows[k] = rows;
     if (r.asym) { sk.a0[k] = p0; sk.hs[k] = (p1 - p0) / (float)r.bins; }
@@ -572,4 +724,66 @@
     return launch_epilogue_hist<true, false>(p, n, num_channel, elem_per_channel, relu, aligned, sk, r, what, s);
 }
 
-}
+int ppqhip_bias_act_pool(float* y, const float* bias, float* pooled, int64_t N, int64_t C, int64_t H, int64_t W, int relu,
+                         int elide_y, void* stream) {
+    if (int st = validate_pool("bias_act_pool", y, bias, pooled, N, C, H, W)) return st;
+    EpPoolArgs p{};
+    p.y = y; p.bias = bias; p.pooled = pooled; p.elide = elide_y ? kElideA : 0u;
+    uint32_t grid; size_t lds_bytes;
+    if (!fill_pool_geometry(p, N, C, H, W, 0, grid, lds_bytes)) return PPQHIP_NOT_FUSED;
+    const EpNoSinks::Args sk{};
+    hipStream_t s = (hipStream_t)stream;
+    if (relu) hipLaunchKernelGGL((epilogue_pool_kernel<kEpTileU, true, EpNoSinks>), dim3(grid), dim3(kEpStatBlock), lds_bytes, s, p, sk);
+    else hipLaunchKernelGGL((epilogue_pool_kernel<kEpTileU, false, EpNoSinks>), dim3(grid), dim3(kEpStatBlock), lds_bytes, s, p, sk);
+    return finish_launch("bias_act_pool");
+}
+
+int ppqhip_bias_act_pool_stats(float* y, const float* bias, float* pooled, int64_t N, int64_t C, int64_t H, int64_t W,
+                               int relu, float* slots_y, int elide_y, void* stream) {
+    const char* what = "bias_act_pool_stats";
+    if (int st = validate_pool(what, y, bias, pooled, N, C, H, W)) return st;
+    if (int st = validate_elide(what, elide_y ? (int)kElideA : 0, slots_y != nullptr, false, false)) return st;
+    if (!slots_y) return PPQHIP_NOT_FUSED;
+    EpPoolArgs p{};
+    p.y = y; p.bias = bias; p.pooled = pooled; p.elide = elide_y ? kElideA : 0u;
+    uint32_t grid; size_t lds_bytes;
+    if (!fill_pool_geometry(p, N, C, H, W, 32, grid, lds_bytes)) return PPQHIP_NOT_FUSED;
+    const EpMinMaxSinks sk{{slots_y, nullptr, nullptr}};
+    using Set = EpMinMaxSet<false, false>;
+    hipStream_t s = (hipStream_t)stream;
+    if (relu) hipLaunchKernelGGL((epilogue_pool_kernel<kEpTileU, true, Set>), dim3(grid), dim3(kEpStatBlock), lds_bytes, s, p, sk);
+    else hipLaunchKernelGGL((epilogue_pool_kernel<kEpTileU, false, Set>), dim3(grid), dim3(kEpStatBlock), lds_bytes, s, p, sk);
+    return finish_launch(what);
+}
+
+int ppqhip_bias_act_pool_hist(float* y, const float* bias, float* pooled, int64_t N, int64_t C, int64_t H, int64_t W,
+                              int relu, int32_t* rows_y, float p0_y, float p1_y, int64_t num_bins, int asymmetric,
+                              int clip_outliers, int elide_y, void* stream) {
+    const char* what = "bias_act_pool_hist";
+    if (int st = validate_pool(what, y, bias, pooled, N, C, H, W)) return st;
+    if (int st = validate_hist_rule(what, num_bins)) return st;
+    if (int st = validate_elide(what, elide_y ? (int)kElideA : 0, rows_y != nullptr, false, false)) return st;
+    if (!rows_y || num_bins > (int64_t)kEpHistLdsInts || !relu) return PPQHIP_NOT_FUSED;
+    const EpHistRule r{(int)num_bins, asymmetric ? 1 : 0, clip_outliers ? 1 : 0};
+    EpHistSinks sk{};
+    set_hist_rule(sk, 0, rows_y, p0_y, p1_y, r);
+    sk.lds_ints = (uint32_t)r.bins; sk.bins = r.bins;
+    EpPoolArgs p{};
+    p.y = y; p.bias = bias; p.pooled = pooled; p.elide = elide_y ? kElideA : 0u;
+    uint32_t grid; size_t lds_bytes;
+    if (!fill_pool_geometry(p, N, C, H, W, sk.lds_ints, grid, lds_bytes)) return PPQHIP_NOT_FUSED;
+    hipStream_t s = (hipStream_t)stream;
+#define PPQ_LAUNCH_EPP(ASYM, CLIP)                                                                                        \
+    hipLaunchKernelGGL((epilogue_pool_kernel<kEpTileU, true, EpHistSet<false, false, ASYM, CLIP>>), dim3(grid),             \
+                       dim3(kEpStatBlock), lds_bytes, s, p, sk)
+    switch ((r.asym ? 2 : 0) | (r.clip ? 1 : 0)) {
+        case 0: PPQ_LAUNCH_EPP(false, false); break;
+        case 1: PPQ_LAUNCH_EPP(false, true); break;
+        case 2: PPQ_LAUNCH_EPP(true, false); break;
+        default: PPQ_LAUNCH_EPP(true, true); break;
+    }
+#undef PPQ_LAUNCH_EPP
+    return finish_launch(what);
+}
+
+}
diff --git a/ppq_amd/csrc/hist.hip b/ppq_amd/csrc/hist.hip
--- a/ppq_amd/csrc/hist.hip
+++ b/ppq_amd/csrc/hist.hip
@@ -1,5 +1,6 @@
 #include "common.hpp"
 #include "hist_bin.hpp"
+#include "job_table.hpp"
 
 namespace ppqhip {
 
@@ -30,9 +31,8 @@
 }
 
 constexpr int kReduceBins = 32, kReduceSlices = 32, kReduceBlock = kReduceBins * kReduceSlices;
-__global__ __launch_bounds__(kReduceBlock) void hist_reduce_kernel(const int* __restrict__ partial, int count, int bins,
-                                                                   int* __restrict__ hist) {
-    __shared__ int lds[kReduceSlices][kReduceBins];
+__device__ __forceinline__ void hist_reduce(const int* __restrict__ partial, int count, int bins, int* __restrict__ hist,
+                                            int (*lds)[kReduceBins]) {
     const int lane_bin = threadIdx.x % kReduceBins, slice = threadIdx.x / kReduceBins;
     const int b = blockIdx.x * kReduceBins + lane_bin;
     int total = 0;
@@ -55,6 +55,22 @@
         for (int k = 0; k < kReduceSlices; k++) t += lds[k][lane_bin];
         if (t) hist[b] += t;
     }
+}
+
+__global__ __launch_bounds__(kReduceBlock) void hist_reduce_kernel(const int* __restrict__ partial, int count, int bins,
+                                                                   int* __restrict__ hist) {
+    __shared__ int lds[kReduceSlices][kReduceBins];
+    hist_reduce(partial, count, bins, hist, lds);
+}
+
+constexpr int kReduceMultiMax = 96;
+struct HistFinishArgs {
+    ppqhip_hist_finish_job jobs[kReduceMultiMax];
+};
+__global__ __launch_bounds__(kReduceBlock) void hist_reduce_multi_kernel(const HistFinishArgs args, int count, int bins) {
+    __shared__ int lds[kReduceSlices][kReduceBins];
+    const ppqhip_hist_finish_job& j = args.jobs[blockIdx.y];
+    hist_reduce(j.rows, count, bins, j.hist, lds);
 }
 
 constexpr int kMultiMax = 96;
@@ -755,6 +771,27 @@
     return finish_launch("hist_rows_finish");
 }
 
+int ppqhip_hist_rows_finish_multi(const ppqhip_hist_finish_job* jobs, int num_jobs, int64_t num_bins, void* stream) {
+    if (num_jobs <= 0) return PPQHIP_OK;
+    if (int st = check_job_table("hist_rows_finish_multi", jobs, num_jobs)) return st;
+    if (num_bins <= 0 || num_bins > kMaxLdsBins) { set_error("hist_rows_finish_multi: bad bins"); return PPQHIP_ERR_INVALID_VALUE; }
+    for (int k = 0; k < num_jobs; k++) {
+        if (!jobs[k].rows || !jobs[k].hist) {
+            set_error("hist_rows_finish_multi: job %d has a null pointer", k); return PPQHIP_ERR_INVALID_VALUE;
+        }
+    }
+    hipStream_t s = (hipStream_t)stream;
+    const int bins = (int)num_bins;
+    for (int base = 0; base < num_jobs; base += kReduceMultiMax) {
+        HistFinishArgs args;
+        const int count = num_jobs - base < kReduceMultiMax ? num_jobs - base : kReduceMultiMax;
+        for (int k = 0; k < kReduceMultiMax; k++) args.jobs[k] = jobs[base + (k < count ? k : 0)];
+        hipLaunchKernelGGL(hist_reduce_multi_kernel, dim3((bins + kReduceBins - 1) / kReduceBins, count), dim3(kReduceBlock), 0, s,
+                           args, (int)ppqhip_hist_rows(), bins);
+    }
+    return finish_launch("hist_rows_finish_multi");
+}
+
 static int hist_c_impl(const float* x, int64_t n, int64_t num_channel, int64_t elem_per_channel,
                        float hist_scale, const float* scales, const float* mins, const float* maxs, int clip_outliers,
                        int32_t* hist, int64_t num_bins, void* stream, const char* what) {
diff --git a/ppq_amd/csrc/reduce.hip b/ppq_amd/csrc/reduce.hip
--- a/ppq_amd/csrc/reduce.hip
+++ b/ppq_amd/csrc/reduce.hip
@@ -3,6 +3,7 @@
 #include <vector>
 
 #include "common.hpp"
+#include "job_table.hpp"
 #include "minmax_fold.hpp"
 
 namespace ppqhip {
@@ -176,9 +177,8 @@
     }
 }
 
-__global__ __launch_bounds__(kBlock) void minmax_finish_kernel(const float* __restrict__ partial, uint32_t count,
-                                                               float* __restrict__ minmax) {
-    __shared__ float lds[32];
+__device__ __forceinline__ void minmax_finish(const float* __restrict__ partial, uint32_t count, float* __restrict__ minmax,
+                                              float* lds) {
     float mn = INFINITY, mx = -INFINITY;
     for (uint32_t i = threadIdx.x; i < count; i += kBlock) {
         mn = fminf(mn, partial[2 * i]);
@@ -186,6 +186,22 @@
     }
     minmax_block_fold(mn, mx, lds);
     if (threadIdx.x == 0) minmax_slot_fold(minmax, mn, mx);
+}
+
+__global__ __launch_bounds__(kBlock) void minmax_finish_kernel(const float* __restrict__ partial, uint32_t count,
+                                                               float* __restrict__ minmax) {
+    __shared__ float lds[32];
+    minmax_finish(partial, count, minmax, lds);
+}
+
+constexpr int kFinishMultiMax = 96;
+struct MinMaxFinishArgs {
+    ppqhip_minmax_finish_job jobs[kFinishMultiMax];
+};
+__global__ __launch_bounds__(kBlock) void minmax_finish_multi_kernel(const MinMaxFinishArgs args, uint32_t count) {
+    __shared__ float lds[32];
+    const ppqhip_minmax_finish_job& j = args.jobs[blockIdx.x];
+    minmax_finish(j.slots, count, j.minmax, lds);
 }
 
 constexpr int kMMCU = 16;
@@ -586,6 +602,24 @@
     return finish_launch("minmax_slots_finish");
 }
 
+int ppqhip_minmax_slots_finish_multi(const ppqhip_minmax_finish_job* jobs, int num_jobs, void* stream) {
+    if (num_jobs <= 0) return PPQHIP_OK;
+    if (int st = check_job_table("minmax_slots_finish_multi", jobs, num_jobs)) return st;
+    for (int k = 0; k < num_jobs; k++) {
+        if (!jobs[k].slots || !jobs[k].minmax) {
+            set_error("minmax_slots_finish_multi: job %d has a null pointer", k); return PPQHIP_ERR_INVALID_VALUE;
+        }
+    }
+    hipStream_t s = (hipStream_t)stream;
+    for (int base = 0; base < num_jobs; base += kFinishMultiMax) {
+        MinMaxFinishArgs args;
+        const int count = num_jobs - base < kFinishMultiMax ? num_jobs - base : kFinishMultiMax;
+        for (int k = 0; k < kFinishMultiMax; k++) args.jobs[k] = jobs[base + (k < count ? k : 0)];
+        hipLaunchKernelGGL(minmax_finish_multi_kernel, dim3(count), dim3(kBlock), 0, s, args, (uint32_t)ppqhip_minmax_slots());
+    }
+    return finish_launch("minmax_slots_finish_multi");
+}
+
 int ppqhip_minmax_c(const float* x, int64_t n, int64_t num_channel, int64_t elem_per_channel, float* mins,
                     float* maxs, void* stream) {
     if (int st = validate(n, "minmax_c")) return st;
diff --git a/ppq_amd/ffi.py b/ppq_amd/ffi.py
--- a/ppq_amd/ffi.py
+++ b/ppq_amd/ffi.py
@@ -146,6 +146,8 @@
     if h is None: h = per[key] = quantile_hint(device)
     return h
 
+
+_FOLD_JOB = np.dtype([('src', '<u8'), ('dst', '<u8')])
 
 _HIST_JOB = np.dtype([('x', '<u8'), ('rows', '<u8'), ('n', '<i8'), ('p0', '<f4'), ('p1', '<f4')])
 
@@ -271,6 +273,27 @@
             a.numel(), geo[0], geo[1], 1 if relu else 0, *sinks[0], *sinks[1], *sinks[2], rule[0], int(rule[1]), int(rule[2]),
             int(elide), _stream()))
     return out if ok else None
+
+
+def bias_act_pool_(y: torch.Tensor, bias: torch.Tensor, relu: bool, job=None, elide: bool = False):
+    geo = _epilogue_geometry([y], [bias])
+    if geo is None or not y.is_contiguous(): return None
+    N, C, H, W = (int(d) for d in y.shape)
+    pooled = torch.empty((N, C, (H - 1) // 2 + 1, (W - 1) // 2 + 1), dtype=_F32, device=y.device)
+    head = (y.data_ptr(), bias.data_ptr(), pooled.data_ptr(), N, C, H, W, 1 if relu else 0)
+    try:
+        with _DeviceOf(y):
+            if job is None:
+                ok = _fused_or_raise(lib.ppqhip_bias_act_pool(*head, int(bool(elide)), _stream()))
+            elif job[0] == 'hist_rows':
+                rows, p0, p1 = _sink_rows(job, y.device)
+                bins, asym, clip = _hist_rule([job])
+                ok = _fused_or_raise(lib.ppqhip_bias_act_pool_hist(*head, rows, p0, p1, bins, int(asym), int(clip),
+                                                                   int(bool(elide)), _stream()))
+            else:
+                ok = _fused_or_raise(lib.ppqhip_bias_act_pool_stats(*head, _sink_slots(job, y.device), int(bool(elide)), _stream()))
+    except ValueError: return None
+    return pooled if ok else None
 
 
 _ADAROUND_JOB = np.dtype([('w', '<u8'), ('v', '<u8'), ('scale', '<u8'), ('offset', '<u8'), ('out', '<u8'), ('dy', '<u8'),
@@ -1393,6 +1416,38 @@
             _raise(lib.ppqhip_minmax_slots_finish(slots.data_ptr(), minmax.data_ptr(), _stream()))
 
     @ staticmethod
+    def MinMax_Slots_Finish_Multi(slots, minmax) -> None:
+        if len(slots) != len(minmax): raise RuntimeError(_KERNEL_FAILURE + 'MinMax_Slots_Finish_Multi: argument lists differ in length')
+        if not slots: return
+        S, dev = 2 * lib.ppqhip_minmax_slots(), slots[0].device
+        for sl, mm in zip(slots, minmax):
+            _f32(sl, 'Slots'); _f32(mm, 'MinMax')
+            if (sl.numel() != S or not sl.is_contiguous() or mm.numel() != 2 or not mm.is_contiguous()
+                    or sl.device != dev or mm.device != dev):
+                raise RuntimeError(_KERNEL_FAILURE + 'MinMax_Slots_Finish_Multi: contiguous [minmax_slots(), 2] / [2] tensors on one device')
+        jobs = np.empty(len(slots), dtype=_FOLD_JOB)
+        jobs['src'] = [sl.data_ptr() for sl in slots]
+        jobs['dst'] = [mm.data_ptr() for mm in minmax]
+        with _DeviceOf(slots[0]):
+            _raise(lib.ppqhip_minmax_slots_finish_multi(jobs.ctypes.data, len(slots), _stream()))
+
+    @ staticmethod
+    def Histogram_Rows_Finish_Multi(rows, hists) -> None:
+        if len(rows) != len(hists): raise RuntimeError(_KERNEL_FAILURE + 'Histogram_Rows_Finish_Multi: argument lists differ in length')
+        if not rows: return
+        R, bins, dev = lib.ppqhip_hist_rows(), rows[0].shape[-1], rows[0].device
+        for r, h in zip(rows, hists):
+            _check(r, torch.int32, 'Rows(Expect to be INT32)'); _HipExtension._check_hist(h)
+            if (r.ndim != 2 or r.shape[0] != R or r.shape[1] != bins or not r.is_contiguous() or h.numel() != bins
+                    or not h.is_contiguous() or r.device != dev or h.device != dev):
+                raise RuntimeError(_KERNEL_FAILURE + f'Histogram_Rows_Finish_Multi: contiguous [{R}, {bins}] / [{bins}] tensors on one device')
+        jobs = np.empty(len(rows), dtype=_FOLD_JOB)
+        jobs['src'] = [r.data_ptr() for r in rows]
+        jobs['dst'] = [h.data_ptr() for h in hists]
+        with _DeviceOf(rows[0]):
+            _raise(lib.ppqhip_hist_rows_finish_multi(jobs.ctypes.data, len(rows), bins, _stream()))
+
+    @ staticmethod
     def Histogram_T_Rows(value, hist_scale: float, clip_outliers: bool, rows) -> None:
         _f32(value, 'Value'); _check(rows, torch.int32, 'Rows(Expect to be INT32)')
         R = lib.ppqhip_hist_rows()
@@ -1872,6 +1927,16 @@
         return histogram
 
     @ staticmethod
+    def MinMax_Slots_Finish_Multi(slots, minmax):
+        HIP_EXTENSION.MinMax_Slots_Finish_Multi(slots, minmax)
+        return minmax
+
+    @ staticmethod
+    def Histogram_Rows_Finish_Multi(rows, histograms):
+        HIP_EXTENSION.Histogram_Rows_Finish_Multi(rows, histograms)
+        return histograms
+
+    @ staticmethod
     def FloatScaleSearch(items, candidates, rounding: int = 0):
         return HIP_EXTENSION.FloatScaleSearch(items, candidates, rounding)
 
diff --git a/ppq_amd/harness.py b/ppq_amd/harness.py
--- a/ppq_amd/harness.py
+++ b/ppq_amd/harness.py
@@ -144,10 +144,11 @@
 
 
 class EpilogueGroup:
-    __slots__ = ('kind', 'ops', 'convs', 'add', 'relu', 'keep')
-
-    def __init__(self, kind, ops, convs, add, relu, keep=()):
+    __slots__ = ('kind', 'ops', 'convs', 'add', 'relu', 'keep', 'pool')
+
+    def __init__(self, kind, ops, convs, add, relu, keep=(), pool=None):
         self.kind, self.ops, self.convs, self.add, self.relu, self.keep = kind, ops, convs, add, relu, frozenset(keep)
+        self.pool = pool
 
     def __repr__(self): return f'{self.kind}({", ".join(op.name for op in self.ops)})'
 
@@ -192,6 +193,20 @@
         if r.type != 'Relu' or len(r.inputs) != 1 or r.inputs[0] is not out or not only_feeds(out, r) or out.name in keep:
             return None
         return r
+
+    def pool_after(relu, i):
+        if i >= len(operations): return None
+        mp, out = operations[i], relu.outputs[0]
+        if (mp.type != 'MaxPool' or len(mp.inputs) != 1 or mp.inputs[0] is not out or not only_feeds(out, mp)
+                or len(mp.outputs) != 1 or mp.outputs[0].name in keep): return None
+        a = mp.attributes
+
+        def is_all(value, k): return value == k or (isinstance(value, (list, tuple)) and len(value) > 0 and all(x == k for x in value))
+        if not (is_all(a.get('kernel_shape'), 3) and is_all(a.get('strides', 1), 2) and is_all(a.get('pads', 0), 1)
+                and is_all(a.get('dilations', 1), 1) and not a.get('ceil_mode', 0)): return None
+        cfgs = (_in_cfg(mp, 0), _out_cfg(mp, 0))
+        if not through(*cfgs, _out_cfg(relu, 0)) or not hooks_ok([mp], cfgs): return None
+        return mp
 
     def try_p2(i):
         for n_conv in (2, 1):
@@ -222,6 +237,8 @@
         if relu is None: return None
         unwritten = (_out_cfg(conv, 0), _in_cfg(relu, 0))
         if not through(*unwritten) or not hooks_ok([conv, relu], unwritten): return None
+        pool = pool_after(relu, i + 2)
+        if pool is not None: return EpilogueGroup('P1', [conv, relu, pool], [conv], None, relu, keep, pool)
         return EpilogueGroup('P1', [conv, relu], [conv], None, relu, keep)
 
     groups, i = [], 0
@@ -237,19 +254,22 @@
 
 
 def elidable_stores(grp: EpilogueGroup, hooks, jobs: Dict[str, tuple], recorder=None) -> set:
-    if grp.kind != 'P2' or recorder is not None or not hooks: return set()
-    add_hook = hooks.get(grp.add.name)
+    if recorder is not None or not hooks: return set()
+    if grp.kind == 'P2': producers, reader = grp.convs, grp.add
+    elif grp.pool is not None: producers, reader = [grp.relu], grp.pool
+    else: return set()
+    reader_hook = hooks.get(reader.name)
     out = set()
-    for conv in grp.convs:
-        v, hook = conv.outputs[0], hooks.get(conv.name)
-        if len(v.dest_ops) != 1 or v.dest_ops[0] is not grp.add or v.name in grp.keep: continue
-        if conv.name not in jobs or hook is None or not isinstance(conv, QuantableOperation): continue
-        obs = [hook._observer_table.get(c) for c in conv.config.output_quantization_config]
+    for op in producers:
+        v, hook = op.outputs[0], hooks.get(op.name)
+        if len(v.dest_ops) != 1 or v.dest_ops[0] is not reader or v.name in grp.keep: continue
+        if op.name not in jobs or hook is None or not isinstance(op, QuantableOperation): continue
+        obs = [hook._observer_table.get(c) for c in op.config.output_quantization_config]
         if len(obs) != 1 or obs[0] is None or not obs[0].reads_only_its_job(): continue
-        if add_hook is not None and isinstance(grp.add, QuantableOperation) and any(
-                c in add_hook._observer_table for x, c in zip(grp.add.inputs, grp.add.config.input_quantization_config) if x is v):
+        if reader_hook is not None and isinstance(reader, QuantableOperation) and any(
+                c in reader_hook._observer_table for x, c in zip(reader.inputs, reader.config.input_quantization_config) if x is v):
             continue
-        out.add(conv.name)
+        out.add(op.name)
     return out
 
 
@@ -487,8 +507,8 @@
         return plan
 
     def _run_epilogue(self, grp: EpilogueGroup, raw_of: Callable, hooks) -> Optional[Dict[str, torch.Tensor]]:
-        from .ffi import (ELIDE_A, ELIDE_B, bias_act_, bias_act_hist_, bias_act_stats_, bias_add_act, bias_add_act_hist,
-                          bias_add_act_stats)
+        from .ffi import (ELIDE_A, ELIDE_B, bias_act_, bias_act_hist_, bias_act_pool_, bias_act_stats_, bias_add_act,
+                          bias_add_act_hist, bias_add_act_stats)
         for conv in grp.convs:
             x, w = raw_of(conv.inputs[0]), conv.inputs[1].value
             if not (isinstance(x, torch.Tensor) and x.is_cuda and x.dtype == torch.float32 and x.dim() == 4
@@ -521,13 +541,27 @@
             y = ys[conv.name]
             stored = {grp.relu.name: y}
             fed = self._epilogue_sinks(grp, hooks, stored, y)
-            if fed is not None:
-                job = fed[0].get(grp.relu.name)
-                launch = bias_act_hist_ if job is not None and job[0] == 'hist_rows' else bias_act_stats_
-                if not launch(y, biases[conv.name], True, job): fed = None
-            if fed is None and not bias_act_(y, biases[conv.name], relu=True):
-                y.add_(biases[conv.name].view(1, -1, 1, 1)).relu_()
-            tail, elided = {conv.name: y, grp.relu.name: y}, set()
+            pooled, elided = None, set()
+            if grp.pool is not None and not self.channels_last:
+                job = fed[0].get(grp.relu.name) if fed is not None else None
+                if job is not None: elided = elidable_stores(grp, hooks, fed[0], fed[1].recorder)
+                elif not hooks:
+                    v = grp.relu.outputs[0]
+                    if len(v.dest_ops) == 1 and v.dest_ops[0] is grp.pool and v.name not in grp.keep: elided = {grp.relu.name}
+                if job is not None or not hooks:
+                    pooled = bias_act_pool_(y, biases[conv.name], True, job, bool(elided))
+                if pooled is None: elided = set()
+            if pooled is None:
+                if fed is not None:
+                    job = fed[0].get(grp.relu.name)
+                    launch = bias_act_hist_ if job is not None and job[0] == 'hist_rows' else bias_act_stats_
+                    if not launch(y, biases[conv.name], True, job): fed = None
+                if fed is None and not bias_act_(y, biases[conv.name], relu=True):
+                    y.add_(biases[conv.name].view(1, -1, 1, 1)).relu_()
+            tail = {conv.name: y, grp.relu.name: y}
+            if grp.pool is not None:
+                a = grp.pool.attributes
+                tail[grp.pool.name] = pooled if pooled is not None else F.max_pool2d(y, a['kernel_shape'], a.get('strides', 1), a.get('pads', 0))
         else:
             conv_a = grp.convs[0]
             a = ys[conv_a.name]
@@ -648,7 +682,7 @@
                 for m in grp.ops:
                     fused_done.add(m.name)
                     for v in m.outputs:
-                        if v.name != hidden: cache[v.name] = vals[v.name]
+                        if v.name != hidden and vals[v.name] is not None: cache[v.name] = vals[v.name]
                 continue
             raw_in = [v.value if v.is_parameter else cache[v.name] for v in op.inputs]
             override = self._overrides.get(op.name)
diff --git a/ppq_amd/observer.py b/ppq_amd/observer.py
--- a/ppq_amd/observer.py
+++ b/ppq_amd/observer.py
@@ -322,6 +322,10 @@
             CUDA.MinMax_Slots_Finish(self._slots, self._range)
             self._slots_dirty = False
 
+    def fold_job(self) -> Optional[tuple]:
+        if not (is_initial(self._quant_cfg) and self._observed and self._slots_dirty): return None
+        return self._slots, self._range
+
     def pending_range(self):
         if not (is_initial(self._quant_cfg) and self._observed): return None
         self._fold()
@@ -426,6 +430,9 @@
         if cfg.policy.has_property(P.ASYMMETRICAL): return ('hist_rows', self._rows, True, self._min, self._max, True)
         if cfg.policy.has_property(P.SYMMETRICAL): return ('hist_rows', self._rows, False, self._hist_scale, 0.0, True)
         return None
+
+    def fold_job(self):
+        return super().fold_job() if self._phase == 'Detecting Minmax' else None
 
     def pending_range(self):
         return super().pending_range() if self._phase == 'Detecting Minmax' else None
@@ -1039,7 +1046,38 @@
         _flush_deferred_sets(pending)
 
 
+def _fold_ranges(observers: Sequence[BaseTensorObserver]) -> None:
+    by_device: Dict[object, list] = {}
+    for ob in observers:
+        job = ob.fold_job() if isinstance(ob, TorchMinMaxObserver) else None
+        if job is not None: by_device.setdefault(job[0].device, []).append((ob, job))
+    for items in by_device.values():
+        if len(items) < 2: continue
+        for ob, _ in items: ob._drain()
+        CUDA.MinMax_Slots_Finish_Multi([j[0] for _, j in items], [j[1] for _, j in items])
+        for ob, _ in items: ob._slots_dirty = False
+
+
+def _stacked_histograms(obs: Sequence['TorchHistObserver']) -> torch.Tensor:
+    dirty = [k for k, ob in enumerate(obs) if ob._rows_dirty and ob._rows is not None and type(ob).histogram is TorchHistObserver.histogram]
+    dev = obs[0]._hist.device
+    if len(dirty) < 2 or any(ob._hist.device != dev for ob in obs): return torch.stack([ob.histogram() for ob in obs])
+    buf = torch.zeros((len(obs), obs[0]._hist.numel()), dtype=torch.int32, device=dev)
+    for k in dirty: obs[k]._drain()
+    CUDA.Histogram_Rows_Finish_Multi([obs[k]._rows for k in dirty], [buf[k] for k in dirty])
+    for k in dirty:
+        ob = obs[k]
+        ob._hist, ob._rows_dirty = buf[k], False
+        if ob._rows.is_cuda: ob._rows.record_stream(torch.cuda.current_stream(ob._rows.device))
+        ob._rows = None
+    done = set(dirty)
+    for k, ob in enumerate(obs):
+        if k not in done: buf[k].copy_(ob.histogram())
+    return buf
+
+
 def _prefetch(observers: Sequence[BaseTensorObserver]) -> None:
+    _fold_ranges([ob for ob in observers if getattr(ob, '_host_range', None) is None])
     pend = [(ob, ob.pending_range()) for ob in observers if getattr(ob, '_host_range', None) is None]
     pend = [(ob, r) for ob, r in pend if r is not None]
     if pend:
@@ -1056,7 +1094,7 @@
             if ob._quant_cfg.policy.has_property(P.PER_TENSOR):
                 groups.setdefault(ob.search_key(), []).append(ob)
     for key, obs in groups.items():
-        hists = torch.stack([ob.histogram() for ob in obs])
+        hists = _stacked_histograms(obs)
         if key[0] == 'kl':
             if any(ob._quant_cfg.policy.has_property(P.ASYMMETRICAL) for ob in obs): continue
             losses = CUDA.KLLosses(hists, key[2]).cpu().numpy()
```

Measured after the change: 3796 samples/s. Within noise of the previous version (-0.1%).
